# whwu95/MVFNet

Measured on AMD Instinct MI355X. Metric: clips/sec (fwd+bwd) MVFNet-R50 8x8 224^2, higher is better.
Workload: dtype bf16; 1 GPU; MVFNet-ResNet50 8x8, 32 clips/GPU of 8x3x224x224, bf16, train step: fwd (batch-stat BN) + loss + bwd + clip + SGD-nesterov; all through the HIP C ABI (stem + 16 bottlenecks + MVF + TSN head); clips_per_gpu=32, frames_per_clip=8, parallelism=dp1: replicas, one flat gradient all-reduce per step

## Files before the change

### include/mvfnet_hip.h

```cpp
#ifndef MVFNET_HIP_H
#define MVFNET_HIP_H

#include <stddef.h>
#include <stdint.h>

#ifdef __cplusplus
extern "C" {
#endif

#define MVF_ABI_VERSION 2

enum { MVF_OK = 0, MVF_EINVAL = -1, MVF_ESHAPE = -2, MVF_EWS = -3, MVF_EHIP = -4, MVF_EUNSUPPORTED = -5 };
enum { MVF_F32 = 0, MVF_BF16 = 1 };
enum { MVF_NCHW = 0, MVF_NHWC = 1 };
enum { MVF_VIEW_T = 1, MVF_VIEW_H = 2, MVF_VIEW_W = 4 };

int mvf_abi_version(void);
const char* mvf_last_error(void);

typedef struct {
    int32_t nt, c, h, w;
    int32_t n_segment;
    int32_t cs;
    int32_t mode;
// ... 6 lines not shown
                  const float* bn_scale, const float* bn_shift, void* stream);

int mvf_fwd_infer_slice(const mvf_desc_t* d, const void* x, void* out_slice,
                        const float* w_t, const float* w_h, const float* w_w,
                        const float* bn_scale, const float* bn_shift, void* stream);

size_t mvf_fwd_train_workspace_bytes(const mvf_desc_t* d);
int mvf_fwd_train(const mvf_desc_t* d, const void* x, void* out,
                  const float* w_t, const float* w_h, const float* w_w,
                  const float* gamma, const float* beta, float eps, float momentum,
                  float* running_mean, float* running_var, float* save_mean, float* save_invstd,
                  void* ws, size_t ws_bytes, void* stream);

size_t mvf_bwd_workspace_bytes(const mvf_desc_t* d);
int mvf_bwd(const mvf_desc_t* d, const void* g, const void* x,
            const float* w_t, const float* w_h, const float* w_w,
            const float* gamma, const float* beta, const float* mean, const float* invstd, int training,
            void* dx, float* dw_t, float* dw_h, float* dw_w, float* dgamma, float* dbeta,
            void* ws, size_t ws_bytes, void* stream);


typedef struct {
    int32_t n, h, w;
    int32_t cin, cout;
    int32_t kh, kw, stride, pad;
    int32_t ho, wo;
    int32_t x_pix_stride;
    int32_t dtype;
    int32_t relu;
    int32_t split_c;
    int32_t x2_pix_stride;
    int32_t in_dil;
    int32_t res_c0;
    int32_t x_c0;
} mvf_conv_desc_t;

int mvf_conv2d_nhwc_fwd(const mvf_conv_desc_t* d, const void* x, const void* x2, const void* w_packed,
                        const float* bias, const void* residual, void* y, void* stream);
size_t mvf_conv2d_workspace_bytes(const mvf_conv_desc_t* d);
int mvf_conv2d_nhwc_fwd_ws(const mvf_conv_desc_t* d, const void* x, const void* x2, const void* w_packed,
                           const float* bias, const void* residual, void* y, void* ws, size_t ws_bytes, void* stream);
int mvf_conv2d_nhwc_fwd_mvf(const mvf_conv_desc_t* d, const void* x, const void* w_packed, const float* bias, const float* mvf_coef,
                            int cs, int n_segment, int act, void* y, void* ws, size_t ws_bytes, void* stream);
int mvf_conv2d_nhwc_fwd_bnapply(const mvf_conv_desc_t* d, const void* x, const void* x2, const void* w_packed, const float* bn_scale,
                                const float* bn_shift, const void* residual, const float* res_scale, const float* res_shift, void* out,
                                unsigned char* sign_bits, void* ws, size_t ws_bytes, void* stream);
int mvf_conv2d_nhwc_fwd_bnbwd_sums(const mvf_conv_desc_t* d, const void* x, const void* x2, const void* w_packed, const void* g,
                                   const unsigned char* sign_bits, const float* bn_mean, const float* bn_invstd, float* sums_part, void* ws,
                                   size_t ws_bytes, void* stream);
int mvf_conv2d_nhwc_fwd_bnbwd_apply(const mvf_conv_desc_t* d, const void* x, const void* x2, const void* w_packed, const void* g,
                                    const unsigned char* sign_bits, const float* bn_gamma, const float* bn_mean, const float* bn_invstd,
                                    const float* dgamma, const float* dbeta, void* dz, void* ws, size_t ws_bytes, void* stream);
int mvf_conv2d_nhwc_fwd_resmask(const mvf_conv_desc_t* d, const void* x, const void* x2, const void* w_packed,
                                const float* bias, const void* residual, const unsigned char* res_sign_bits, void* y,
                                void* ws, size_t ws_bytes, void* stream);
int mvf_conv2d_nhwc_fwd_resmask_gate(const mvf_conv_desc_t* d, const void* x, const void* x2, const void* w_packed, const float* bias,
                                     const void* residual, const unsigned char* res_sign_bits, const unsigned char* out_gate_bits, void* y,
                                     void* ws, size_t ws_bytes, void* stream);
int mvf_conv2d_nhwc_fwd_resmask_gate_colsums(const mvf_conv_desc_t* d, const void* x, const void* x2, const void* w_packed, const void* residual,
                                             const unsigned char* res_sign_bits, const unsigned char* out_gate_bits, void* y, float* sums_part, void* ws,
                                             size_t ws_bytes, void* stream);
int mvf_conv2d_nhwc_dgrad_bnsums(const mvf_conv_desc_t* d, const void* dz, const void* w_packed_dgrad, void* y, const void* bn_z,
                                 const float* bn_mean, const float* bn_invstd, const float* bn_scale, const float* bn_shift,
                                 float* sums_part, void* ws, size_t ws_bytes, void* stream);
int mvf_bn_bwd_finalize(const float* sums_part, int nblk, int c, float* dgamma, float* dbeta, void* stream);
int mvf_conv2d_stats_rows(const mvf_conv_desc_t* d);
int mvf_conv2d_nhwc_fwd_stats(const mvf_conv_desc_t* d, const void* x, const void* x2, const void* w_packed, void* y,
                              float* stats_part, const float* stats_shift, void* ws, size_t ws_bytes, void* stream);

enum {
    MVF_CONV_FAM_NONE = 0,
    MVF_CONV_FAM_REG = 1,
    MVF_CONV_FAM_X3 = 2,
    MVF_CONV_FAM_LDS_DMA = 3,
    MVF_CONV_FAM_T256_2B = 4,
    MVF_CONV_FAM_T256_P4 = 5,
    MVF_CONV_FAM_DBUF = 6,
    MVF_CONV_FAM_DBUF_PF2 = 7,
    MVF_CONV_FAM_STREAMK = 8,
    MVF_CONV_FAM_GENERIC = 9,
    MVF_CONV_FAM_MVF_LOADER = 10,
    MVF_CONV_FAM_STEM_DIRECT = 11,
    MVF_CONV_FAM_PW_SUMS = 12,
    MVF_CONV_FAM_C3X3_C64 = 13
};
typedef struct {
    int32_t family;
    int32_t epi_asked;
    int32_t epi_run;
    int32_t pointwise;
    int32_t buffers;
    int32_t tile_m, tile_n;
    int32_t dtype;
    int32_t k_chunks;
    int32_t half_k;
    int32_t launches;
} mvf_conv_launch_info_t;
int mvf_conv2d_last_launch(mvf_conv_launch_info_t* out);

int mvf_pack_conv_weight(const float* w_oihw, int cout, int cin, int kh, int kw, int kw_pad, int cin_pad,
                         const float* scale, void* w_packed, int dtype, void* stream);
int mvf_bn_fold(const float* gamma, const float* beta, const float* mean, const float* var, float eps, int c,
                float* scale, float* shift, void* stream);

int mvf_stem_prep(const float* x_nchw, int n, int c, int h, int w, int pad, int wp, void* out, int dtype, void* stream);

int mvf_frames_prep_u8(const unsigned char* frames_hwc, int n, int hs, int ws, const int* window, int h, int w,
                       const float* mean3, const float* std3, int to_rgb, int div_255, int pad, int wp, void* out_stem,
                       float* out_nchw, int dtype, void* stream);
int mvf_frames_resample_u8(const unsigned char* frames_hwc, int n, int hs, int ws, const int* rows, int h, int w,
                           const float* mean3, const float* std3, int to_rgb, int div_255, int pad, int wp, void* out_stem,
                           float* out_nchw, int dtype, void* stream);
int mvf_frames_resample_color_u8(const unsigned char* frames_hwc, int n, int hs, int ws, const int* rows, const float* color, int h, int w,
                                 const float* mean3, const float* std3, int to_rgb, int div_255, int pad, int wp, void* out_stem,
                                 float* out_nchw, int dtype, void* stream);
int mvf_frames_gather_resample_u8(const unsigned char* frames_hwc, int n_src, int hs, int ws, const int* src_index, int n_out, const int* rows,
                                  const float* color, int h, int w, const float* mean3, const float* std3, int to_rgb, int div_255, int pad,
                                  int wp, void* out_stem, float* out_nchw, int dtype, void* stream);
int mvf_frames_yuv420_gather_resample_u8(const unsigned char* frames, int n_src, int hs, int ws, int pitch, int layout, int standard, int order,
                                         const int* src_index, int n_out, const int* rows, const float* color, int h, int w, const float* mean3,
                                         const float* std3, int to_rgb, int div_255, int pad, int wp, void* out_stem, float* out_nchw, int dtype,
                                         void* stream);
int mvf_frames_addressed_resample_u8(const unsigned char* frames, long long frames_bytes, int format, int standard, int order,
                                     int n_out, const int* rows, const int* addr, const float* color, int h, int w,
                                     const float* mean3, const float* std3, int to_rgb, int div_255, int pad, int wp,
                                     void* out_stem, float* out_nchw, int dtype, void* stream);

int mvf_maxpool3x3s2_nhwc(const void* x, int n, int h, int w, int c, void* y, int dtype, void* stream);

int mvf_head_pool_fc(const void* feat, int clips, int t, int hw, int c, const float* fc_w, const float* fc_b,
                     int classes, float* pooled_ws, float* scores, int dtype, void* stream);
int mvf_average_clip(const float* scores, int clips, int classes, int kind, float* out, void* stream);
int mvf_average_clip_sigmoid(const float* scores, int clips, int classes, float* out, void* stream);

int mvf_conv2d_nhwc_dgrad_bnsums_split(const mvf_conv_desc_t* d, const void* x, const void* x2, const void* w_packed, const float* bias, void* y,
                                       const void* bn_z, const float* bn_mean, const float* bn_invstd, const float* bn_scale, const float* bn_shift,
                                       float* sums_part, void* ws, size_t ws_bytes, void* stream);
int mvf_bn_bwd_dzfree_prep(const void* w_packed_dgrad, int c, int k, const float* gamma, const float* mean, const float* invstd, const float* dgamma,
                           const float* dbeta, long m, void* w_out, float* bias_out, int dtype, void* stream);
int mvf_bn_bwd_dzfree_wgrad(float* dw, const void* w_packed, const float* gram, const float* a_mean, const float* gamma, const float* mean,
                            const float* invstd, const float* dgamma, const float* dbeta, long m, int c, int k, int dtype, void* stream);
int mvf_bn_bwd_dzfree_sums(const float* q, const void* w_packed, int c, int k, const float* mean, const float* invstd, const float* part_lo, int rows_lo,
                           int c_split, const float* part_hi, int rows_hi, float* dgamma, float* dbeta, int dtype, void* stream);
size_t mvf_bn_workspace_bytes(long m, int c);
int mvf_bn_train_stats(const void* z, long m, int c, const float* gamma, const float* beta, float eps, float momentum,
                       float* running_mean, float* running_var, float* save_mean, float* save_invstd, float* scale,
                       float* shift, void* ws, size_t ws_bytes, int dtype, void* stream);
int mvf_bn_train_finalize(const float* part, int nblk, long m, int c, const float* gamma, const float* beta, float eps,
                          float momentum, float* running_mean, float* running_var, float* save_mean, float* save_invstd,
                          float* scale, float* shift, void* stream);
int mvf_bn_train_stats_gram(const float* gram, const float* a_mean, const void* w_packed, long m, int c, int k, const float* gamma, const float* beta,
                            float eps, float momentum, float* running_mean, float* running_var, float* save_mean, float* save_invstd, float* scale,
                            float* shift, int dtype, void* stream);
int mvf_bn_apply_colmeans(const void* z, long m, int c, const float* scale, const float* shift, int act, void* out, float* mean_out, void* ws,
                          size_t ws_bytes, int dtype, void* stream);
int mvf_bn_apply(const void* z, long m, int c, const float* scale, const float* shift, const void* residual,
                 const float* rscale, const float* rshift, int act, void* out, int dtype, void* stream);
int mvf_bn_bwd_reduce(const void* g, int g_pitch, const void* z, const void* ymask, long m, int c, const float* mean,
                      const float* invstd, const float* scale, const float* shift, int mask_mode, void* gm_out,
                      float* dgamma, float* dbeta, void* ws, size_t ws_bytes, int dtype, void* stream);
int mvf_bn_bwd_apply(const void* g, int g_pitch, const void* z, long m, int c, const float* gamma, const float* mean,
                     const float* invstd, const float* scale, const float* shift, const float* dgamma,
                     const float* dbeta, int mask_mode, void* dz, int dtype, void* stream);
int mvf_bn_apply_bits(const void* z, long m, int c, const float* scale, const float* shift, const void* residual,
                      const float* rscale, const float* rshift, int relu, void* out, unsigned char* sign_bits, int dtype,
                      void* stream);
int mvf_bn_apply_bits_rowscale(const void* z, long m, int c, const float* scale, const float* shift, const void* residual, const float* rscale,
                               const float* rshift, const float* row_scale, int rows_per_image, int act, void* out, unsigned char* sign_bits, int dtype,
                               void* stream);
int mvf_gate_rowscale(const void* g, int g_pitch, const unsigned char* sign_bits, const float* row_scale, int rows_per_image, long m, int c, void* gm_out,
                      int dtype, void* stream);
int mvf_bn_bwd_apply_masked(const void* g, int g_pitch, const void* z, const void* ymask, long m, int c, const float* gamma,
                            const float* mean, const float* invstd, const float* scale, const float* shift,
                            const float* dgamma, const float* dbeta, int mask_mode, void* dz, int dtype, void* stream);
int mvf_bn_bwd_pair(const void* g, int g_pitch, const void* z_a, const void* z_b, const unsigned char* sign_bits, long m, int c,
                    const float* gamma_a, const float* mean_a, const float* invstd_a, float* dgamma_a, float* dbeta_a,
                    const float* gamma_b, const float* mean_b, const float* invstd_b, float* dgamma_b, float* dbeta_b,
                    void* dz_a, void* dz_b, void* ws, size_t ws_bytes, int dtype, void* stream);
int mvf_bn_bwd_wgrad_splits(long m, int c, int k, int nbn, int mask_mode);
size_t mvf_bn_bwd_wgrad_slab_bytes(long m, int c, int k, int nbn, int mask_mode);
int mvf_bn_bwd_apply_wgrad(const void* g, int g_pitch, const void* z, const void* ymask, long m, int c, const float* gamma, const float* mean,
                           const float* invstd, const float* scale, const float* shift, const float* dgamma, const float* dbeta, int mask_mode,
                           void* dz, const void* x, int x_pitch, int k, float* slabs, size_t slab_bytes, int dtype, void* stream);
int mvf_bn_bwd_pair_wgrad(const void* g, int g_pitch, const void* z_a, const void* z_b, const unsigned char* sign_bits, long m, int c,
                          const float* gamma_a, const float* mean_a, const float* invstd_a, float* dgamma_a, float* dbeta_a,
                          const float* gamma_b, const float* mean_b, const float* invstd_b, float* dgamma_b, float* dbeta_b,
                          void* dz_a, void* dz_b, const void* x_a, int xa_pitch, const void* x_b, int xb_pitch, int k,
                          float* slabs_a, float* slabs_b, size_t slab_bytes, void* ws, size_t ws_bytes, int dtype, void* stream);
int mvf_conv1x1_bwd_fused_splits(long m, int c, int k);
int mvf_conv1x1_bwd_fused(const void* a_in, int a_pitch, const void* w_packed, const void* g, int g_pitch, const unsigned char* sign_bits, long m, int c,
                          int k, const float* gamma, const float* mean, const float* invstd, const float* dgamma, const float* dbeta, const void* z_in,
                          const float* in_mean, const float* in_invstd, const float* in_scale, const float* in_shift, void* dx, float* sums_part,
                          int sums_rows, float* slabs, size_t slab_bytes, int dtype, void* stream);
int mvf_conv1x1_bnbwd_sums_pair(const void* a_in, int a_pitch, const void* w_a, const void* x_in, int x_pitch, const void* w_b, const void* g, int g_pitch,
                                const unsigned char* sign_bits, long m, int c, int k, const float* mean_a, const float* invstd_a, const float* mean_b,
                                const float* invstd_b, float* part_a, float* part_b, int rows, int dtype, void* stream);
int mvf_wgrad_slab_reduce(const float* slabs, int nsplit, int cout, int k, float* dw_oihw, void* stream);
int mvf_maxpool_bn_relu_fwd(const void* z, int n, int h, int w, int c, const float* scale, const float* shift, void* y,
                            unsigned char* argmax, int dtype, void* stream);
int mvf_maxpool_bn_relu_bwd(const unsigned char* argmax, const void* g, int n, int h, int w, int c, void* ga, int dtype,
                            void* stream);
int mvf_maxpool_bwd_sums_rows(int n, int h);
int mvf_maxpool_bn_relu_bwd_apply(const unsigned char* argmax, const void* g, int n, int h, int w, int c, const void* z, const float* gamma,
                                  const float* mean, const float* invstd, const float* scale, const float* shift, const float* dgamma,
                                  const float* dbeta, void* dz, int dtype, void* stream);
int mvf_maxpool_bn_relu_bwd_sums(const unsigned char* argmax, const void* g, int n, int h, int w, int c, void* ga, const void* z, const float* mean,
                                 const float* invstd, const float* scale, const float* shift, float* sums_part, int dtype, void* stream);
enum {
    MVF_BN_ENTRY_NONE = 0,
    MVF_BN_ENTRY_TRAIN_STATS = 1, MVF_BN_ENTRY_TRAIN_FINALIZE = 2,
    MVF_BN_ENTRY_APPLY = 3,
    MVF_BN_ENTRY_APPLY_COLMEANS = 4,
    MVF_BN_ENTRY_BWD_REDUCE = 5, MVF_BN_ENTRY_BWD_FINALIZE = 6,
    MVF_BN_ENTRY_BWD_APPLY = 7,
    MVF_BN_ENTRY_BWD_PAIR = 8, MVF_BN_ENTRY_BWD_PAIR_WGRAD = 9,
    MVF_BN_ENTRY_POOL_FWD = 10, MVF_BN_ENTRY_POOL_BWD = 11, MVF_BN_ENTRY_POOL_BWD_SUMS = 12, MVF_BN_ENTRY_POOL_BWD_APPLY = 13
};
enum {
    MVF_BN_FIN_NONE = 0,
    MVF_BN_FIN_ROW_MAJOR = 1,
    MVF_BN_FIN_CM_WORKGROUP = 2,
    MVF_BN_FIN_CM_WAVE = 3
};
enum {
    MVF_POOL_FORM_NONE = 0,
    MVF_POOL_FORM_ELEMENT = 1,
    MVF_POOL_FORM_ROWS = 2,
    MVF_POOL_FORM_BLOCK = 3,
    MVF_POOL_FORM_ROWS_SUMS = 4,
    MVF_POOL_FORM_ROWS_APPLY = 5
};
typedef struct {
    int32_t entry;
    int32_t dtype;
    int32_t vn;
    int32_t cqb, rows, gx, gy;
    int32_t mask_mode;
    int32_t specialised;
    int32_t finalize;
    int32_t part_rows;
    int32_t pool;
    int32_t launches;
} mvf_bn_launch_info_t;
int mvf_bn_last_launch(mvf_bn_launch_info_t* out);
int mvf_head_train_fwd(const void* feat, int clips, int t, int hw, int c, const float* fc_w, const float* fc_b, int classes,
                       const long long* labels, const float* drop_mask ,
                       float* pooled, float* scores, float* dscores, float* loss_part, float* loss, int dtype, void* stream);
int mvf_ce_loss(const float* scores, const long long* labels, int clips, int classes, float* dscores, float* loss_part, float* loss,
                void* stream);
int mvf_head_train_bwd(const float* dscores, const float* pooled, const float* fc_w, const float* drop_mask, int clips, int t,
                       int hw, int c, int classes, float* dfc_w, float* dfc_b, float* dpool_ws , void* dfeat, int dtype,
                       void* stream);
int mvf_stem_blend(const void* xp, int clips, int t, int hp, int wp, int pad, const int* rows, const float* wts, void* out, int dtype, void* stream);
int mvf_soft_targets(const long long* labels, const int* rows, const float* wts, int clips, int classes, float eps, float* targets, void* stream);
int mvf_ce_loss_soft(const float* scores, const float* targets, int clips, int classes, float* dscores, float* loss_part, float* loss, void* stream);
int mvf_head_train_fwd_soft(const void* feat, int clips, int t, int hw, int c, const float* fc_w, const float* fc_b, int classes,
                            const float* targets, const float* drop_mask ,
                            float* pooled, float* scores, float* dscores, float* loss_part, float* loss, int dtype, void* stream);
int mvf_bce_loss(const float* scores, const float* targets, int clips, int classes, const float* pos_weight ,
                 float target_threshold , int sum_classes, float* dscores , float* loss_part, float* loss, void* stream);
int mvf_head_train_fwd_bce(const void* feat, int clips, int t, int hw, int c, const float* fc_w, const float* fc_b, int classes,
                           const float* targets, const float* drop_mask ,
                           const float* pos_weight , float target_threshold , int sum_classes,
                           float* pooled, float* scores, float* dscores, float* loss_part, float* loss, int dtype, void* stream);
typedef struct mvf_focal_params {
    float gamma_pos, gamma_neg, margin, alpha, target_threshold;
    int sum_classes, reserved[2];
} mvf_focal_params_t;
int mvf_focal_loss(const float* scores, const float* targets, int clips, int classes, const float* class_weight ,
                   const mvf_focal_params_t* prm, float* dscores , float* loss_part, float* loss, void* stream);
int mvf_head_train_fwd_focal(const void* feat, int clips, int t, int hw, int c, const float* fc_w, const float* fc_b, int classes,
                             const float* targets, const float* drop_mask ,
                             const float* class_weight , const mvf_focal_params_t* prm,
                             float* pooled, float* scores, float* dscores, float* loss_part, float* loss, int dtype, void* stream);
int mvf_distill_loss(const float* scores, const float* teacher_scores, int clips, int classes, float temperature, float alpha,
                     float* dscores , float* loss_part , float* loss , float* terms ,
                     void* stream);
#define MVF_TRN_MAX_FRAMES 16
#define MVF_TRN_KSPLIT_MAX 8
typedef struct mvf_trn_scale {
    const float *w1, *b1, *w2, *b2;
    float *dw1, *db1, *dw2, *db2;
} mvf_trn_scale_t;
enum { MVF_TRN_ENTRY_NONE = 0, MVF_TRN_ENTRY_FWD = 1, MVF_TRN_ENTRY_BWD = 2 };
typedef struct mvf_trn_launch_info {
    int32_t entry;
    int32_t dtype;
    int32_t rows, n_scales;
    int32_t launches;
} mvf_trn_launch_info_t;
int mvf_trn_head_fwd(const void* feat, int clips, int t, int hw, int c, const float* fc_w, const float* fc_b, int fdim, const mvf_trn_scale_t* scales,
                     int n_scales, int hidden, int classes, const int* table, int rows, const float* drop_mask , float* pooled,
                     float* f, float* h, float* hpart , float* scores, int dtype, void* stream);
int mvf_trn_head_bwd(const float* dscores, const float* pooled, const float* f, const float* h, const float* fc_w, const mvf_trn_scale_t* scales, int n_scales,
                     int hidden, int classes, const int* table, int rows, const float* drop_mask , int clips, int t, int hw, int c,
                     int fdim, float* dfc_w, float* dfc_b, float* dh , float* df , float* dpool ,
                     void* dfeat, int dtype, void* stream);
int mvf_trn_head_last_launch(mvf_trn_launch_info_t* out);
int mvf_stem_erase(void* xp, int planes, int hp, int wp, int pad, const int* boxes, int max_boxes, const float* fill, const unsigned int* key, int dtype,
                   void* stream);
#define MVF_RANDAUG_WS_PER_FRAME (3 * 256 + 16)
int mvf_frames_randaug_u8(const unsigned char* frames_hwc, int n, int hs, int ws, int t, int order, const int* sizes, const int* table, int layers,
                          unsigned stats_layers, unsigned char* out, unsigned char* tmp, void* workspace, long long workspace_bytes, void* stream);
size_t mvf_conv2d_wgrad_workspace_bytes(const mvf_conv_desc_t* d);
int mvf_conv2d_nhwc_wgrad(const mvf_conv_desc_t* d, const void* dz, const void* x, const void* x2, int kw_real,
                          int cin_real, int kw_packed, int cin_packed, float* dw_oihw, void* ws, size_t ws_bytes,
                          void* stream);
int mvf_conv2d_nhwc_wgrad_wgs(const mvf_conv_desc_t* d, const void* dz, const void* x, const void* x2, int kw_real,
                              int cin_real, int kw_packed, int cin_packed, float* dw_oihw, void* ws, size_t ws_bytes, int wgs, void* stream);
enum {
    MVF_WGRAD_FAM_NONE = 0,
    MVF_WGRAD_FAM_F32_REG = 1,
    MVF_WGRAD_FAM_F32_DMA = 2,
    MVF_WGRAD_FAM_X3 = 3,
    MVF_WGRAD_FAM_BF16_WIDEN = 4,
    MVF_WGRAD_FAM_BF16_REG = 5,
    MVF_WGRAD_FAM_BF16_DMA2 = 6,
    MVF_WGRAD_FAM_BF16_PIPE = 7,
    MVF_WGRAD_FAM_T256_2B = 8,
    MVF_WGRAD_FAM_T256_P4 = 9,
    MVF_WGRAD_FAM_C3X3_C64 = 10,
    MVF_WGRAD_FAM_STEM = 11
};
typedef struct {
    int32_t family;
    int32_t stages;
    int32_t tile_co, tile_k;
    int32_t dtype;
    int32_t nsplit;
    int32_t rows_per_split;
    int32_t xcd_rr;
    int32_t split_operand;
    int32_t gram;
    int32_t wgs_target;
    int32_t launches;
} mvf_wgrad_launch_info_t;
int mvf_conv2d_wgrad_last_launch(mvf_wgrad_launch_info_t* out);
typedef struct {
    const float* w;
    void* out;
    int cout, cin, kh, kw, kw_pad, cin_pad;
    int kind, first_block;
} mvf_pack_job_t;
int mvf_pack_conv_weights_batched(const mvf_pack_job_t* jobs_dev, int njobs, int total_blocks, int dtype, void* stream);

int mvf_pack_conv_weight_dgrad(const float* w_oihw, int cout, int cin, int kh, int kw, void* w_packed, int dtype,
                               void* stream);
int mvf_nhwc_stencil(const mvf_desc_t* d, const void* x, int x_c, void* out, int out_c, const float* w_t,
                     const float* w_h, const float* w_w, const float* scale, const float* shift, int flip,
                     const void* addend, int addend_c, const unsigned char* addend_sign_bits, void* stream);
int mvf_nhwc_stencil_gate(const mvf_desc_t* d, const void* x, int x_c, void* out, int out_c, const float* w_t,
                          const float* w_h, const float* w_w, const float* scale, const float* shift, int flip,
                          const void* addend, int addend_c, const unsigned char* addend_sign_bits,
                          const unsigned char* out_gate_bits, void* stream);
int mvf_nhwc_stencil_gate_colsums(const mvf_desc_t* d, const void* x, int x_c, void* out, int out_c, const float* w_t, const float* w_h,
                                  const float* w_w, int flip, const void* addend, int addend_c, const unsigned char* addend_sign_bits,
                                  const unsigned char* out_gate_bits, float* sums_part, void* stream);
int mvf_nhwc_stencil_stats_rows(const mvf_desc_t* d, int x_c, int out_c);
int mvf_nhwc_stencil_tile_plan(const mvf_desc_t* d, int x_c, int out_c, int* rows_per_band, int* chan_per_wg);
int mvf_nhwc_stencil_stats(const mvf_desc_t* d, const void* x, int x_c, void* out, int out_c, const float* w_t, const float* w_h,
                           const float* w_w, float* stats_part, const float* stats_shift, void* stream);
size_t mvf_nhwc_tapgrad_workspace_bytes(const mvf_desc_t* d);
int mvf_nhwc_tapgrad(const mvf_desc_t* d, const void* x, int x_c, const void* dy, int dy_c, float* dw_t, float* dw_h,
                     float* dw_w, void* ws, size_t ws_bytes, void* stream);
enum {
    MVF_STENCIL_KERNEL_NONE = 0,
    MVF_STENCIL_KERNEL_WALK1 = 1,
    MVF_STENCIL_KERNEL_WALK4 = 2,
    MVF_STENCIL_KERNEL_CHUNKED = 3,
    MVF_STENCIL_KERNEL_LDS = 4
};
enum {
    MVF_STENCIL_FLIP = 1, MVF_STENCIL_HSWISH = 2, MVF_STENCIL_ADDEND = 4, MVF_STENCIL_ADDEND_BITS = 8, MVF_STENCIL_OUT_GATE = 16,
    MVF_STENCIL_STATS = 32,
    MVF_STENCIL_TAIL_COPY = 64
};
typedef struct {
    int32_t kernel;
    int32_t dtype;
    int32_t frames_per_chunk;
    int32_t rows_per_band, chan_per_wg;
    int32_t bands;
    int32_t pixels_per_wg;
    int32_t grid_x, grid_y;
    int32_t partial_rows;
    int32_t flags;
    int32_t launches;
} mvf_stencil_launch_info_t;
int mvf_nhwc_stencil_last_launch(mvf_stencil_launch_info_t* out);
enum {
    MVF_TAPGRAD_KERNEL_NONE = 0,
    MVF_TAPGRAD_KERNEL_ROWS = 1,
    MVF_TAPGRAD_KERNEL_BANDS = 2
};
typedef struct {
    int32_t kernel;
    int32_t dtype;
    int32_t nblk;
    int32_t rows_per_blk;
    int32_t cgp;
    int32_t grid_y;
    int32_t launches;
} mvf_tapgrad_launch_info_t;
int mvf_nhwc_tapgrad_last_launch(mvf_tapgrad_launch_info_t* out);
size_t mvf_sgd_workspace_bytes(long n);
int mvf_sgd_nesterov_step(float* params, const float* grads, float* momentum_buf, long n, float grad_scale, float max_norm,
                          float lr, float momentum, float weight_decay, int first_step, float* norm_out, void* ws,
                          size_t ws_bytes, void* stream);
typedef struct mvf_sgd_segment {
    long long first;
    float lr_mult, decay_mult;
} mvf_sgd_segment_t;
int mvf_sgd_step_segments(float* params, const float* grads, float* momentum_buf, long n, float grad_scale, float max_norm, float lr,
                          float momentum, float weight_decay, int first_step, int nesterov, const mvf_sgd_segment_t* segments, int nseg,
                          float* norm_out, void* ws, size_t ws_bytes, void* stream);
int mvf_grad_accumulate(float* acc, const float* g, long n, int first, void* stream);
int mvf_sgd_nesterov_step_ema(float* params, const float* grads, float* momentum_buf, long n, float grad_scale, float max_norm, float lr, float momentum,
                              float weight_decay, int first_step, float* ema, float ema_momentum, float* norm_out, void* ws, size_t ws_bytes, void* stream);
int mvf_sgd_step_segments_ema(float* params, const float* grads, float* momentum_buf, long n, float grad_scale, float max_norm, float lr, float momentum,
                              float weight_decay, int first_step, int nesterov, const mvf_sgd_segment_t* segments, int nseg, float* ema, float ema_momentum,
                              float* norm_out, void* ws, size_t ws_bytes, void* stream);
int mvf_ema_update(float* ema, const float* params, long n, float momentum, void* stream);
int mvf_ema_swap(float* a, float* b, long n, void* stream);
typedef struct mvf_stat_segment {
    float* ptr;
    long first;
} mvf_stat_segment_t;
int mvf_bn_stats_accumulate(const mvf_stat_segment_t* seg, int nseg, long n, double* acc, void* stream);
int mvf_bn_stats_finalize(const mvf_stat_segment_t* seg, int nseg, long n, const double* acc, long count, float* dst_flat_or_null, void* stream);
int mvf_bn_stats_exchange(const mvf_stat_segment_t* seg, int nseg, long n, float* flat, int mode, void* stream);
int mvf_sgd_step_guarded(float* params, const float* grads, float* momentum_buf, long n, float grad_scale, float max_norm, float lr, float momentum,
                         float weight_decay, int first_step, int nesterov, const mvf_sgd_segment_t* segments, int nseg, float* ema, float ema_momentum,
                         int* guard, float* norm_out, void* ws, size_t ws_bytes, void* stream);
int mvf_bn_stats_snapshot(const mvf_stat_segment_t* seg, int nseg, long n, float* flat, const long long* counters, long ncount, long long* counters_copy,
                          void* stream);
int mvf_bn_stats_restore(const mvf_stat_segment_t* seg, int nseg, long n, const float* flat, long long* counters, long ncount,
                         const long long* counters_copy, const int* guard, void* stream);
typedef struct mvf_adamw_hyper {
    double lr, beta1, beta2, eps, weight_decay;
    int decoupled;
} mvf_adamw_hyper_t;
size_t mvf_adamw_workspace_bytes(long n);
int mvf_adamw_step(float* params, const float* grads, float* exp_avg, float* exp_avg_sq, long n, float grad_scale, float max_norm,
                   const mvf_adamw_hyper_t* hyper, const mvf_sgd_segment_t* segments, int nseg, float* ema, float ema_momentum, int* guard,
                   long long* applied_steps, float* norm_out, void* ws, size_t ws_bytes, void* stream);
typedef struct mvf_lamb_hyper {
    double lr, beta1, beta2, eps, weight_decay;
    int trust_clip, always_adapt;
} mvf_lamb_hyper_t;
size_t mvf_lamb_workspace_bytes(long n, int nseg);
int mvf_lamb_step(float* params, const float* grads, float* exp_avg, float* exp_avg_sq, long n, float grad_scale, float max_norm,
                  const mvf_lamb_hyper_t* hyper, const mvf_sgd_segment_t* segments, int nseg, float* ema, float ema_momentum, int* guard,
                  long long* applied_steps, float* norm_out, float* ratio_out, void* ws, size_t ws_bytes, void* stream);
enum { MVF_METRICS_ROWS = 0, MVF_METRICS_BAD_LABEL = 1, MVF_METRICS_NAN_ROWS = 2, MVF_METRICS_HITS = 8, MVF_METRICS_MAX_K = 8, MVF_METRICS_CONFUSION = 16 };
size_t mvf_metrics_state_words(int classes, int with_confusion);
int mvf_metrics_update(const float* scores, int rows, int classes, const long long* labels, const int* ks, int nk, long long* state, int with_confusion,
                       int* rank_out, int* pred_out, void* stream);
enum { MVF_MULTILABEL_SLOTS = 0, MVF_MULTILABEL_NAN_ROWS = 1, MVF_MULTILABEL_OVERFLOW = 2, MVF_MULTILABEL_SEEN = 3, MVF_MULTILABEL_STATE_WORDS = 8 };
int mvf_multilabel_record(const float* scores, const unsigned char* labels, int rows, int classes, float* rec_scores, unsigned char* rec_labels, long capacity,
                          long long* state, void* stream);
int mvf_multilabel_ap(const float* rec_scores, const unsigned char* rec_labels, long capacity, int classes, const long long* state, int* tp, int* nn, double* ap,
                      long long* positives, void* stream);
int mvf_multilabel_sample_ap(const float* rec_scores, const unsigned char* rec_labels, long capacity, int classes, const long long* state, double* sample_ap,
                             int* sample_positives, void* stream);
int mvf_multilabel_prf(const float* rec_scores, const unsigned char* rec_labels, long capacity, int classes, const long long* state, float threshold,
                       const float* thresholds , long long* counts , void* stream);
int mvf_multilabel_best_f1(const float* rec_scores, const int* tp, const int* nn, const long long* positives, long capacity, int classes,
                           const long long* state, int* best_tp, int* best_n, float* best_threshold, void* stream);
typedef struct mvf_flat_stats {
    double sumsq;
    double absmax;
    long long n_nan;
    long long n_inf;
} mvf_flat_stats_t;
size_t mvf_flat_stats_workspace_bytes(long n, int nseg);
int mvf_flat_segment_stats(const float* x, const float* y_or_null, long n, const long long* first, int nseg, mvf_flat_stats_t* out, const int* guard_or_null,
                           long long* step_out_or_null, void* ws, size_t ws_bytes, void* stream);
int mvf_bn_stats_nonfinite(const mvf_stat_segment_t* seg, int nseg, long n, long long* counts, const int* guard_or_null, void* stream);

enum { MVF_PLAN_CALL = 0, MVF_PLAN_RECORD = 1, MVF_PLAN_WAIT = 2 };
typedef struct mvf_plan_op {
    int kind, n_int, n_flt, reserved;
    void* fn;
    long long word0, float0;
} mvf_plan_op_t;
int mvf_plan_run(const mvf_plan_op_t* ops, int n_ops, const unsigned long long* words, const float* floats, int* failed_op);

#ifdef __cplusplus
}
#endif
// ... 2 lines not shown
```

### mvfnet_amd/_lib.py

```python
import ctypes as C
import os

import torch

_HERE = os.path.dirname(os.path.abspath(__file__))
LIB_PATH = os.environ.get("MVF_LIB_PATH") or os.path.join(_HERE, "libmvfnet_hip.so")

MVF_F32, MVF_BF16 = 0, 1
MVF_NCHW, MVF_NHWC = 0, 1
VIEW_T, VIEW_H, VIEW_W = 1, 2, 4
MODE_BITS = {"T": 1, "TH": 3, "THW": 7}
METRICS_ROWS, METRICS_BAD_LABEL, METRICS_NAN_ROWS, METRICS_HITS, METRICS_MAX_K, METRICS_CONFUSION = 0, 1, 2, 8, 8, 16
MULTILABEL_SLOTS, MULTILABEL_NAN_ROWS, MULTILABEL_OVERFLOW, MULTILABEL_SEEN, MULTILABEL_STATE_WORDS = 0, 1, 2, 3, 8
ERRNAMES = {-1: "MVF_EINVAL", -2: "MVF_ESHAPE", -3: "MVF_EWS", -4: "MVF_EHIP", -5: "MVF_EUNSUPPORTED"}


class MvfDesc(C.Structure):
    _fields_ = [("nt", C.c_int32), ("c", C.c_int32), ("h", C.c_int32), ("w", C.c_int32), ("n_segment", C.c_int32),
                ("cs", C.c_int32), ("mode", C.c_int32), ("layout", C.c_int32), ("dtype", C.c_int32)]


class ConvDesc(C.Structure):
    _fields_ = [("n", C.c_int32), ("h", C.c_int32), ("w", C.c_int32), ("cin", C.c_int32), ("cout", C.c_int32),
                ("kh", C.c_int32), ("kw", C.c_int32), ("stride", C.c_int32), ("pad", C.c_int32),
# ... 71 lines not shown


class FocalParams(C.Structure):
    _fields_ = [("gamma_pos", C.c_float), ("gamma_neg", C.c_float), ("margin", C.c_float), ("alpha", C.c_float), ("target_threshold", C.c_float),
                ("sum_classes", C.c_int32), ("reserved", C.c_int32 * 2)]


TRN_MAX_FRAMES, TRN_KSPLIT_MAX = 16, 8


class TrnScale(C.Structure):
    _fields_ = [("w1", C.c_void_p), ("b1", C.c_void_p), ("w2", C.c_void_p), ("b2", C.c_void_p),
                ("dw1", C.c_void_p), ("db1", C.c_void_p), ("dw2", C.c_void_p), ("db2", C.c_void_p)]


class TrnLaunchInfo(C.Structure):
    _fields_ = [("entry", C.c_int32), ("dtype", C.c_int32), ("rows", C.c_int32), ("n_scales", C.c_int32), ("launches", C.c_int32)]


class LambHyper(C.Structure):
    _fields_ = [("lr", C.c_double), ("beta1", C.c_double), ("beta2", C.c_double), ("eps", C.c_double), ("weight_decay", C.c_double), ("trust_clip", C.c_int32),
                ("always_adapt", C.c_int32)]


class StatSegment(C.Structure):
    _fields_ = [("ptr", C.c_void_p), ("first", C.c_long)]


QUERIES = frozenset((
    "mvf_abi_version", "mvf_last_error",
    "mvf_fwd_train_workspace_bytes", "mvf_bwd_workspace_bytes", "mvf_conv2d_workspace_bytes", "mvf_conv2d_wgrad_workspace_bytes", "mvf_bn_workspace_bytes",
    "mvf_bn_bwd_wgrad_slab_bytes", "mvf_nhwc_tapgrad_workspace_bytes", "mvf_sgd_workspace_bytes", "mvf_adamw_workspace_bytes", "mvf_lamb_workspace_bytes",
    "mvf_flat_stats_workspace_bytes", "mvf_metrics_state_words",
    "mvf_conv2d_stats_rows", "mvf_nhwc_stencil_stats_rows", "mvf_maxpool_bwd_sums_rows",
    "mvf_bn_bwd_wgrad_splits", "mvf_conv1x1_bwd_fused_splits", "mvf_nhwc_stencil_tile_plan",
    "mvf_conv2d_last_launch", "mvf_conv2d_wgrad_last_launch", "mvf_bn_last_launch", "mvf_nhwc_stencil_last_launch", "mvf_nhwc_tapgrad_last_launch",
    "mvf_trn_head_last_launch",
))


def _load():
    if not os.path.exists(LIB_PATH):
        raise ImportError(
            "mvfnet_amd: %s not found. Build it with `python -m mvfnet_amd.build` (needs hipcc, "
            "--offload-arch=gfx950). There is no CPU or PyTorch fallback for the hot path." % LIB_PATH)
    lib = C.CDLL(LIB_PATH)
    vp, fp, sz, i32, f32 = C.c_void_p, C.c_void_p, C.c_size_t, C.c_int, C.c_float
    dp = C.POINTER(MvfDesc)
    lib.mvf_abi_version.restype = i32
    lib.mvf_abi_version.argtypes = []
    lib.mvf_last_error.restype = C.c_char_p
    lib.mvf_last_error.argtypes = []
    lib.mvf_fwd_infer.restype = i32
    lib.mvf_fwd_infer.argtypes = [dp, vp, vp, fp, fp, fp, fp, fp, vp]
    lib.mvf_fwd_train_workspace_bytes.restype = sz
    lib.mvf_fwd_train_workspace_bytes.argtypes = [dp]
    lib.mvf_fwd_train.restype = i32
    lib.mvf_fwd_train.argtypes = [dp, vp, vp, fp, fp, fp, fp, fp, f32, f32, fp, fp, fp, fp, vp, sz, vp]
    lib.mvf_bwd_workspace_bytes.restype = sz
    lib.mvf_bwd_workspace_bytes.argtypes = [dp]
    lib.mvf_bwd.restype = i32
    lib.mvf_bwd.argtypes = [dp, vp, vp, fp, fp, fp, fp, fp, fp, fp, i32, vp, fp, fp, fp, fp, fp, vp, sz, vp]
    lib.mvf_fwd_infer_slice.restype = i32
    lib.mvf_fwd_infer_slice.argtypes = [dp, vp, vp, fp, fp, fp, fp, fp, vp]
    cp = C.POINTER(ConvDesc)
    lib.mvf_conv2d_nhwc_fwd.restype = i32
    lib.mvf_conv2d_nhwc_fwd.argtypes = [cp, vp, vp, vp, fp, vp, vp, vp]
    lib.mvf_conv2d_workspace_bytes.restype = sz
    lib.mvf_conv2d_workspace_bytes.argtypes = [cp]
    lib.mvf_conv2d_nhwc_fwd_ws.restype = i32
    lib.mvf_conv2d_nhwc_fwd_ws.argtypes = [cp, vp, vp, vp, fp, vp, vp, vp, sz, vp]
    lib.mvf_conv2d_nhwc_dgrad_bnsums.restype = i32
    lib.mvf_conv2d_nhwc_dgrad_bnsums.argtypes = [cp, vp, vp, vp, vp, fp, fp, fp, fp, fp, vp, sz, vp]
    lib.mvf_bn_bwd_finalize.restype = i32
    lib.mvf_bn_bwd_finalize.argtypes = [fp, i32, i32, fp, fp, vp]
    lib.mvf_conv2d_nhwc_fwd_bnapply.restype = i32
    lib.mvf_conv2d_nhwc_fwd_bnapply.argtypes = [cp, vp, vp, vp, fp, fp, vp, fp, fp, vp, vp, vp, sz, vp]
    lib.mvf_conv2d_nhwc_fwd_bnbwd_sums.restype = i32
    lib.mvf_conv2d_nhwc_fwd_bnbwd_sums.argtypes = [cp, vp, vp, vp, vp, vp, fp, fp, fp, vp, sz, vp]
    lib.mvf_conv2d_nhwc_fwd_bnbwd_apply.restype = i32
    lib.mvf_conv2d_nhwc_fwd_bnbwd_apply.argtypes = [cp, vp, vp, vp, vp, vp, fp, fp, fp, fp, fp, vp, vp, sz, vp]
    lib.mvf_conv2d_nhwc_fwd_resmask.restype = i32
    lib.mvf_conv2d_nhwc_fwd_resmask.argtypes = [cp, vp, vp, vp, fp, vp, vp, vp, vp, sz, vp]
    i64_ = C.c_long
    lib.mvf_conv2d_nhwc_fwd_resmask_gate.restype = i32
    lib.mvf_conv2d_nhwc_fwd_resmask_gate.argtypes = [cp, vp, vp, vp, fp, vp, vp, vp, vp, vp, sz, vp]
    lib.mvf_conv2d_nhwc_fwd_resmask_gate_colsums.restype = i32
    lib.mvf_conv2d_nhwc_fwd_resmask_gate_colsums.argtypes = [cp, vp, vp, vp, vp, vp, vp, vp, fp, vp, sz, vp]
    lib.mvf_nhwc_stencil_gate_colsums.restype = i32
    lib.mvf_nhwc_stencil_gate_colsums.argtypes = [dp, vp, i32, vp, i32, fp, fp, fp, i32, vp, i32, vp, vp, fp, vp]
    lib.mvf_conv2d_nhwc_dgrad_bnsums_split.restype = i32
    lib.mvf_conv2d_nhwc_dgrad_bnsums_split.argtypes = [cp, vp, vp, vp, fp, vp, vp, fp, fp, fp, fp, fp, vp, sz, vp]
    lib.mvf_bn_bwd_dzfree_prep.restype = i32
    lib.mvf_bn_bwd_dzfree_prep.argtypes = [vp, i32, i32, fp, fp, fp, fp, fp, i64_, vp, fp, i32, vp]
    lib.mvf_bn_bwd_dzfree_wgrad.restype = i32
    lib.mvf_bn_bwd_dzfree_wgrad.argtypes = [fp, vp, fp, fp, fp, fp, fp, fp, fp, i64_, i32, i32, i32, vp]
    lib.mvf_bn_bwd_dzfree_sums.restype = i32
    lib.mvf_bn_bwd_dzfree_sums.argtypes = [fp, vp, i32, i32, fp, fp, fp, i32, i32, fp, i32, fp, fp, i32, vp]
    lib.mvf_nhwc_stencil_stats_rows.restype = i32
    lib.mvf_nhwc_stencil_stats_rows.argtypes = [dp, i32, i32]
    lib.mvf_nhwc_stencil_tile_plan.restype = i32
    lib.mvf_nhwc_stencil_tile_plan.argtypes = [dp, i32, i32, C.POINTER(C.c_int), C.POINTER(C.c_int)]
    lib.mvf_nhwc_stencil_stats.restype = i32
    lib.mvf_nhwc_stencil_stats.argtypes = [dp, vp, i32, vp, i32, fp, fp, fp, fp, fp, vp]
    lib.mvf_nhwc_stencil_gate.restype = i32
    lib.mvf_nhwc_stencil_gate.argtypes = [dp, vp, i32, vp, i32, fp, fp, fp, fp, fp, i32, vp, i32, vp, vp, vp]
    lib.mvf_conv2d_stats_rows.restype = i32
    lib.mvf_conv2d_stats_rows.argtypes = [cp]
    lib.mvf_conv2d_nhwc_fwd_stats.restype = i32
    lib.mvf_conv2d_nhwc_fwd_stats.argtypes = [cp, vp, vp, vp, vp, fp, fp, vp, sz, vp]
    lib.mvf_conv2d_last_launch.restype = i32
    lib.mvf_conv2d_last_launch.argtypes = [C.POINTER(ConvLaunchInfo)]
    lib.mvf_pack_conv_weight.restype = i32
    lib.mvf_pack_conv_weight.argtypes = [fp, i32, i32, i32, i32, i32, i32, fp, vp, i32, vp]
    lib.mvf_pack_conv_weights_batched.restype = i32
    lib.mvf_pack_conv_weights_batched.argtypes = [vp, i32, i32, i32, vp]
    lib.mvf_bn_fold.restype = i32
    lib.mvf_bn_fold.argtypes = [fp, fp, fp, fp, f32, i32, fp, fp, vp]
    lib.mvf_stem_prep.restype = i32
    lib.mvf_stem_prep.argtypes = [fp, i32, i32, i32, i32, i32, i32, vp, i32, vp]
    lib.mvf_frames_prep_u8.restype = i32
    lib.mvf_frames_prep_u8.argtypes = [vp, i32, i32, i32, vp, i32, i32, C.POINTER(C.c_float), C.POINTER(C.c_float),
                                       i32, i32, i32, i32, vp, vp, i32, vp]
    lib.mvf_frames_resample_u8.restype = i32
    lib.mvf_frames_resample_u8.argtypes = [vp, i32, i32, i32, vp, i32, i32, C.POINTER(C.c_float), C.POINTER(C.c_float),
                                           i32, i32, i32, i32, vp, vp, i32, vp]
    lib.mvf_frames_resample_color_u8.restype = i32
    lib.mvf_frames_resample_color_u8.argtypes = [vp, i32, i32, i32, vp, vp, i32, i32, C.POINTER(C.c_float), C.POINTER(C.c_float),
                                                 i32, i32, i32, i32, vp, vp, i32, vp]
    lib.mvf_frames_gather_resample_u8.restype = i32
    lib.mvf_frames_gather_resample_u8.argtypes = [vp, i32, i32, i32, vp, i32, vp, vp, i32, i32, C.POINTER(C.c_float), C.POINTER(C.c_float),
                                                  i32, i32, i32, i32, vp, vp, i32, vp]
    lib.mvf_frames_yuv420_gather_resample_u8.restype = i32
    lib.mvf_frames_yuv420_gather_resample_u8.argtypes = [vp, i32, i32, i32, i32, i32, i32, i32, vp, i32, vp, vp, i32, i32, C.POINTER(C.c_float),
                                                         C.POINTER(C.c_float), i32, i32, i32, i32, vp, vp, i32, vp]
    lib.mvf_frames_addressed_resample_u8.restype = i32
    lib.mvf_frames_addressed_resample_u8.argtypes = [vp, C.c_longlong, i32, i32, i32, i32, vp, vp, vp, i32, i32, C.POINTER(C.c_float), C.POINTER(C.c_float),
                                                     i32, i32, i32, i32, vp, vp, i32, vp]
    lib.mvf_maxpool3x3s2_nhwc.restype = i32
    lib.mvf_maxpool3x3s2_nhwc.argtypes = [vp, i32, i32, i32, i32, vp, i32, vp]
    lib.mvf_head_pool_fc.restype = i32
    lib.mvf_head_pool_fc.argtypes = [vp, i32, i32, i32, i32, fp, fp, i32, fp, fp, i32, vp]
    lib.mvf_average_clip.restype = i32
    lib.mvf_average_clip.argtypes = [fp, i32, i32, i32, fp, vp]
    i64, ll = C.c_long, C.c_void_p
    lib.mvf_bn_workspace_bytes.restype = sz
    lib.mvf_bn_workspace_bytes.argtypes = [i64, i32]
    lib.mvf_bn_train_stats.restype = i32
    lib.mvf_bn_train_stats.argtypes = [vp, i64, i32, fp, fp, f32, f32, fp, fp, fp, fp, fp, fp, vp, sz, i32, vp]
    lib.mvf_bn_train_finalize.restype = i32
    lib.mvf_bn_train_finalize.argtypes = [fp, i32, i64, i32, fp, fp, f32, f32, fp, fp, fp, fp, fp, fp, vp]
    lib.mvf_bn_train_stats_gram.restype = i32
    lib.mvf_bn_train_stats_gram.argtypes = [fp, fp, vp, i64, i32, i32, fp, fp, f32, f32, fp, fp, fp, fp, fp, fp, i32, vp]
    lib.mvf_bn_apply_colmeans.restype = i32
    lib.mvf_bn_apply_colmeans.argtypes = [vp, i64, i32, fp, fp, i32, vp, fp, vp, sz, i32, vp]
    lib.mvf_bn_apply.restype = i32
    lib.mvf_bn_apply.argtypes = [vp, i64, i32, fp, fp, vp, fp, fp, i32, vp, i32, vp]
    lib.mvf_bn_apply_bits.restype = i32
    lib.mvf_bn_apply_bits.argtypes = [vp, i64, i32, fp, fp, vp, fp, fp, i32, vp, vp, i32, vp]
    lib.mvf_bn_apply_bits_rowscale.restype = i32
    lib.mvf_bn_apply_bits_rowscale.argtypes = [vp, i64, i32, fp, fp, vp, fp, fp, fp, i32, i32, vp, vp, i32, vp]
    lib.mvf_gate_rowscale.restype = i32
    lib.mvf_gate_rowscale.argtypes = [vp, i32, vp, fp, i32, i64, i32, vp, i32, vp]
    lib.mvf_bn_bwd_apply_masked.restype = i32
    lib.mvf_bn_bwd_apply_masked.argtypes = [vp, i32, vp, vp, i64, i32, fp, fp, fp, fp, fp, fp, fp, i32, vp, i32, vp]
    lib.mvf_bn_bwd_reduce.restype = i32
    lib.mvf_bn_bwd_reduce.argtypes = [vp, i32, vp, vp, i64, i32, fp, fp, fp, fp, i32, vp, fp, fp, vp, sz, i32, vp]
    lib.mvf_bn_bwd_apply.restype = i32
    lib.mvf_bn_bwd_apply.argtypes = [vp, i32, vp, i64, i32, fp, fp, fp, fp, fp, fp, fp, i32, vp, i32, vp]
    lib.mvf_maxpool_bn_relu_fwd.restype = i32
    lib.mvf_maxpool_bn_relu_fwd.argtypes = [vp, i32, i32, i32, i32, fp, fp, vp, vp, i32, vp]
    lib.mvf_maxpool_bn_relu_bwd.restype = i32
    lib.mvf_maxpool_bn_relu_bwd.argtypes = [vp, vp, i32, i32, i32, i32, vp, i32, vp]
    lib.mvf_maxpool_bwd_sums_rows.restype = i32
    lib.mvf_maxpool_bwd_sums_rows.argtypes = [i32, i32]
    lib.mvf_maxpool_bn_relu_bwd_apply.restype = i32
    lib.mvf_maxpool_bn_relu_bwd_apply.argtypes = [vp, vp, i32, i32, i32, i32, vp, fp, fp, fp, fp, fp, fp, fp, vp, i32, vp]
    lib.mvf_maxpool_bn_relu_bwd_sums.restype = i32
    lib.mvf_maxpool_bn_relu_bwd_sums.argtypes = [vp, vp, i32, i32, i32, i32, vp, vp, fp, fp, fp, fp, fp, i32, vp]
    lib.mvf_bn_last_launch.restype = i32
    lib.mvf_bn_last_launch.argtypes = [C.POINTER(BnLaunchInfo)]
    lib.mvf_head_train_fwd.restype = i32
    lib.mvf_head_train_fwd.argtypes = [vp, i32, i32, i32, i32, fp, fp, i32, ll, fp, fp, fp, fp, fp, fp, i32, vp]
    lib.mvf_conv2d_nhwc_fwd_mvf.restype = i32
    lib.mvf_conv2d_nhwc_fwd_mvf.argtypes = [cp, vp, vp, fp, fp, i32, i32, i32, vp, vp, sz, vp]
    lib.mvf_bn_bwd_pair.restype = i32
    lib.mvf_bn_bwd_pair.argtypes = [vp, i32, vp, vp, vp, i64, i32, fp, fp, fp, fp, fp, fp, fp, fp, fp, fp, vp, vp, vp, sz, i32, vp]
    lib.mvf_bn_bwd_wgrad_splits.restype = i32
    lib.mvf_bn_bwd_wgrad_splits.argtypes = [i64, i32, i32, i32, i32]
    lib.mvf_bn_bwd_wgrad_slab_bytes.restype = sz
    lib.mvf_bn_bwd_wgrad_slab_bytes.argtypes = [i64, i32, i32, i32, i32]
    lib.mvf_bn_bwd_apply_wgrad.restype = i32
    lib.mvf_bn_bwd_apply_wgrad.argtypes = [vp, i32, vp, vp, i64, i32, fp, fp, fp, fp, fp, fp, fp, i32, vp, vp, i32, i32, fp, sz, i32, vp]
    lib.mvf_bn_bwd_pair_wgrad.restype = i32
    lib.mvf_bn_bwd_pair_wgrad.argtypes = [vp, i32, vp, vp, vp, i64, i32, fp, fp, fp, fp, fp, fp, fp, fp, fp, fp, vp, vp, vp, i32, vp, i32, i32,
                                          fp, fp, sz, vp, sz, i32, vp]
    lib.mvf_conv1x1_bwd_fused_splits.restype = i32
    lib.mvf_conv1x1_bwd_fused_splits.argtypes = [i64, i32, i32]
    lib.mvf_conv1x1_bwd_fused.restype = i32
    lib.mvf_conv1x1_bwd_fused.argtypes = [vp, i32, vp, vp, i32, vp, i64, i32, i32, fp, fp, fp, fp, fp, vp, fp, fp, fp, fp, vp, fp, i32, fp, sz, i32, vp]
    lib.mvf_conv1x1_bnbwd_sums_pair.restype = i32
    lib.mvf_conv1x1_bnbwd_sums_pair.argtypes = [vp, i32, vp, vp, i32, vp, vp, i32, vp, i64, i32, i32, fp, fp, fp, fp, fp, fp, i32, i32, vp]
    lib.mvf_wgrad_slab_reduce.restype = i32
    lib.mvf_wgrad_slab_reduce.argtypes = [fp, i32, i32, i32, fp, vp]
    lib.mvf_ce_loss.restype = i32
    lib.mvf_ce_loss.argtypes = [fp, ll, i32, i32, fp, fp, fp, vp]
    lib.mvf_stem_blend.restype = i32
    lib.mvf_stem_blend.argtypes = [vp, i32, i32, i32, i32, i32, vp, fp, vp, i32, vp]
    lib.mvf_stem_erase.restype = i32
    lib.mvf_stem_erase.argtypes = [vp, i32, i32, i32, i32, vp, i32, fp, vp, i32, vp]
    lib.mvf_frames_randaug_u8.restype = i32
    lib.mvf_frames_randaug_u8.argtypes = [vp, i32, i32, i32, i32, i32, vp, vp, i32, C.c_uint, vp, vp, vp, C.c_longlong, vp]
    lib.mvf_soft_targets.restype = i32
    lib.mvf_soft_targets.argtypes = [ll, vp, fp, i32, i32, f32, fp, vp]
    lib.mvf_ce_loss_soft.restype = i32
    lib.mvf_ce_loss_soft.argtypes = [fp, fp, i32, i32, fp, fp, fp, vp]
    lib.mvf_head_train_fwd_soft.restype = i32
    lib.mvf_head_train_fwd_soft.argtypes = [vp, i32, i32, i32, i32, fp, fp, i32, fp, fp, fp, fp, fp, fp, fp, i32, vp]
    lib.mvf_distill_loss.restype = i32
    lib.mvf_distill_loss.argtypes = [fp, fp, i32, i32, f32, f32, fp, fp, fp, fp, vp]
    lib.mvf_bce_loss.restype = i32
    lib.mvf_bce_loss.argtypes = [fp, fp, i32, i32, fp, f32, i32, fp, fp, fp, vp]
    lib.mvf_head_train_fwd_bce.restype = i32
    lib.mvf_head_train_fwd_bce.argtypes = [vp, i32, i32, i32, i32, fp, fp, i32, fp, fp, fp, f32, i32, fp, fp, fp, fp, fp, i32, vp]
    lib.mvf_focal_loss.restype = i32
    lib.mvf_focal_loss.argtypes = [fp, fp, i32, i32, fp, C.POINTER(FocalParams), fp, fp, fp, vp]
    lib.mvf_head_train_fwd_focal.restype = i32
    lib.mvf_head_train_fwd_focal.argtypes = [vp, i32, i32, i32, i32, fp, fp, i32, fp, fp, fp, C.POINTER(FocalParams), fp, fp, fp, fp, fp, i32, vp]
    lib.mvf_trn_head_fwd.restype = i32
    lib.mvf_trn_head_fwd.argtypes = [vp, i32, i32, i32, i32, fp, fp, i32, C.POINTER(TrnScale), i32, i32, i32, vp, i32, fp, fp, fp, fp, fp, fp, i32, vp]
    lib.mvf_trn_head_bwd.restype = i32
    lib.mvf_trn_head_bwd.argtypes = [fp, fp, fp, fp, fp, C.POINTER(TrnScale), i32, i32, i32, vp, i32, fp, i32, i32, i32, i32, i32, fp, fp, fp, fp, fp, vp, i32, vp]
    lib.mvf_trn_head_last_launch.restype = i32
    lib.mvf_trn_head_last_launch.argtypes = [C.POINTER(TrnLaunchInfo)]
    lib.mvf_average_clip_sigmoid.restype = i32
    lib.mvf_average_clip_sigmoid.argtypes = [fp, i32, i32, fp, vp]
    lib.mvf_multilabel_record.restype = i32
    lib.mvf_multilabel_record.argtypes = [fp, vp, i32, i32, fp, vp, C.c_long, ll, vp]
    lib.mvf_multilabel_ap.restype = i32
    lib.mvf_multilabel_ap.argtypes = [fp, vp, C.c_long, i32, ll, vp, vp, vp, ll, vp]
    lib.mvf_multilabel_sample_ap.restype = i32
    lib.mvf_multilabel_sample_ap.argtypes = [fp, vp, C.c_long, i32, ll, vp, vp, vp]
    lib.mvf_multilabel_prf.restype = i32
    lib.mvf_multilabel_prf.argtypes = [fp, vp, C.c_long, i32, ll, f32, fp, ll, vp]
    lib.mvf_multilabel_best_f1.restype = i32
    lib.mvf_multilabel_best_f1.argtypes = [fp, vp, vp, ll, C.c_long, i32, ll, vp, vp, fp, vp]
    lib.mvf_head_train_bwd.restype = i32
    lib.mvf_head_train_bwd.argtypes = [fp, fp, fp, fp, i32, i32, i32, i32, i32, fp, fp, fp, vp, i32, vp]
    lib.mvf_conv2d_wgrad_workspace_bytes.restype = sz
    lib.mvf_conv2d_wgrad_workspace_bytes.argtypes = [cp]
    lib.mvf_conv2d_nhwc_wgrad.restype = i32
    lib.mvf_conv2d_nhwc_wgrad.argtypes = [cp, vp, vp, vp, i32, i32, i32, i32, fp, vp, sz, vp]
    lib.mvf_conv2d_nhwc_wgrad_wgs.restype = i32
    lib.mvf_conv2d_nhwc_wgrad_wgs.argtypes = [cp, vp, vp, vp, i32, i32, i32, i32, fp, vp, sz, i32, vp]
    lib.mvf_conv2d_wgrad_last_launch.restype = i32
    lib.mvf_conv2d_wgrad_last_launch.argtypes = [C.POINTER(WgradLaunchInfo)]
    lib.mvf_pack_conv_weight_dgrad.restype = i32
    lib.mvf_pack_conv_weight_dgrad.argtypes = [fp, i32, i32, i32, i32, vp, i32, vp]
    lib.mvf_nhwc_stencil.restype = i32
    lib.mvf_nhwc_stencil.argtypes = [dp, vp, i32, vp, i32, fp, fp, fp, fp, fp, i32, vp, i32, vp, vp]
    lib.mvf_nhwc_tapgrad_workspace_bytes.restype = sz
    lib.mvf_nhwc_tapgrad_workspace_bytes.argtypes = [dp]
    lib.mvf_nhwc_tapgrad.restype = i32
    lib.mvf_nhwc_tapgrad.argtypes = [dp, vp, i32, vp, i32, fp, fp, fp, vp, sz, vp]
    lib.mvf_nhwc_stencil_last_launch.restype = i32
    lib.mvf_nhwc_stencil_last_launch.argtypes = [C.POINTER(StencilLaunchInfo)]
    lib.mvf_nhwc_tapgrad_last_launch.restype = i32
    lib.mvf_nhwc_tapgrad_last_launch.argtypes = [C.POINTER(TapgradLaunchInfo)]
    lib.mvf_sgd_workspace_bytes.restype = sz
    lib.mvf_sgd_workspace_bytes.argtypes = [i64]
    lib.mvf_sgd_nesterov_step.restype = i32
    lib.mvf_sgd_nesterov_step.argtypes = [fp, fp, fp, i64, f32, f32, f32, f32, f32, i32, fp, vp, sz, vp]
    lib.mvf_sgd_step_segments.restype = i32
    lib.mvf_sgd_step_segments.argtypes = [fp, fp, fp, i64, f32, f32, f32, f32, f32, i32, i32, vp, i32, fp, vp, sz, vp]
    lib.mvf_grad_accumulate.restype = i32
    lib.mvf_grad_accumulate.argtypes = [fp, fp, i64, i32, vp]
    lib.mvf_sgd_nesterov_step_ema.restype = i32
    lib.mvf_sgd_nesterov_step_ema.argtypes = [fp, fp, fp, i64, f32, f32, f32, f32, f32, i32, fp, f32, fp, vp, sz, vp]
    lib.mvf_sgd_step_segments_ema.restype = i32
    lib.mvf_sgd_step_segments_ema.argtypes = [fp, fp, fp, i64, f32, f32, f32, f32, f32, i32, i32, vp, i32, fp, f32, fp, vp, sz, vp]
    lib.mvf_ema_update.restype = i32
    lib.mvf_ema_update.argtypes = [fp, fp, i64, f32, vp]
    lib.mvf_ema_swap.restype = i32
    lib.mvf_ema_swap.argtypes = [fp, fp, i64, vp]
    lib.mvf_bn_stats_accumulate.restype = i32
    lib.mvf_bn_stats_accumulate.argtypes = [vp, i32, i64, vp, vp]
    lib.mvf_bn_stats_finalize.restype = i32
    lib.mvf_bn_stats_finalize.argtypes = [vp, i32, i64, vp, i64, fp, vp]
    lib.mvf_bn_stats_exchange.restype = i32
    lib.mvf_bn_stats_exchange.argtypes = [vp, i32, i64, fp, i32, vp]
    lib.mvf_sgd_step_guarded.restype = i32
    lib.mvf_sgd_step_guarded.argtypes = [fp, fp, fp, i64, f32, f32, f32, f32, f32, i32, i32, vp, i32, fp, f32, vp, fp, vp, sz, vp]
    lib.mvf_bn_stats_snapshot.restype = i32
    lib.mvf_bn_stats_snapshot.argtypes = [vp, i32, i64, fp, vp, i64, vp, vp]
    lib.mvf_bn_stats_restore.restype = i32
    lib.mvf_bn_stats_restore.argtypes = [vp, i32, i64, fp, vp, i64, vp, vp, vp]
    lib.mvf_adamw_workspace_bytes.restype = sz
    lib.mvf_adamw_workspace_bytes.argtypes = [i64]
    lib.mvf_adamw_step.restype = i32
    lib.mvf_adamw_step.argtypes = [fp, fp, fp, fp, i64, f32, f32, C.POINTER(AdamwHyper), vp, i32, fp, f32, vp, vp, fp, vp, sz, vp]
    lib.mvf_lamb_workspace_bytes.restype = sz
    lib.mvf_lamb_workspace_bytes.argtypes = [i64, i32]
    lib.mvf_lamb_step.restype = i32
    lib.mvf_lamb_step.argtypes = [fp, fp, fp, fp, i64, f32, f32, C.POINTER(LambHyper), vp, i32, fp, f32, vp, vp, fp, fp, vp, sz, vp]
    lib.mvf_metrics_state_words.restype = sz
    lib.mvf_metrics_state_words.argtypes = [i32, i32]
    lib.mvf_metrics_update.restype = i32
    lib.mvf_metrics_update.argtypes = [fp, i32, i32, ll, vp, i32, ll, i32, vp, vp, vp]
    lib.mvf_flat_stats_workspace_bytes.restype = sz
    lib.mvf_flat_stats_workspace_bytes.argtypes = [i64, i32]
    lib.mvf_flat_segment_stats.restype = i32
    lib.mvf_flat_segment_stats.argtypes = [fp, fp, i64, vp, i32, vp, vp, vp, vp, sz, vp]
    lib.mvf_bn_stats_nonfinite.restype = i32
    lib.mvf_bn_stats_nonfinite.argtypes = [vp, i32, i64, vp, vp, vp]
    lib.mvf_plan_run.restype = i32
    lib.mvf_plan_run.argtypes = [C.POINTER(PlanOp), i32, C.POINTER(C.c_ulonglong), C.POINTER(C.c_float), C.POINTER(C.c_int)]
    missing = [n for n in declared_symbols() if hasattr(lib, n) and getattr(lib, n).argtypes is None]
    if missing:
        raise ImportError("mvfnet_amd._lib: no argtypes declared for %s" % missing)
    return lib


def check(rc, what=""):
    if rc != 0:
        msg = lib.mvf_last_error().decode("utf-8", "replace")
        raise RuntimeError("%s failed: %s (%s)" % (what or "libmvfnet_hip", ERRNAMES.get(rc, rc), msg))


def declared_symbols():
    import re
    hdr = os.path.join(os.path.dirname(_HERE), "include", "mvfnet_hip.h")
    txt = open(hdr).read()
    txt = re.sub(r"/\*.*?\*/", "", txt, flags=re.S)
    return sorted(set(re.findall(r"\b((?:mvf|mvfnet)_[a-z0-9_]+)\s*\(", txt)))


lib = _load()
```

### mvfnet_amd/csrc/bn_dzfree.hip

```cpp
#include "common.h"

namespace {

typedef float f32x16 __attribute__((ext_vector_type(16)));
typedef short bf16x8 __attribute__((ext_vector_type(8)));

struct PrepArgs {
    const uint16_t* wd;
    const float *gamma, *mean, *invstd, *dgamma, *dbeta;
    uint16_t* bd;
    float* bias;
    int C, K;
    float inv_m;
    int g_wgs, s_wgs;
};

__device__ __forceinline__ float bf16lo(unsigned u) { return __uint_as_float(u << 16); }
__device__ __forceinline__ float bf16hi(unsigned u) { return __uint_as_float(u & 0xffff0000u); }

__global__ __launch_bounds__(256) void dzfree_prep_kernel(PrepArgs p) {
    extern __shared__ __attribute__((aligned(16))) float coef[];
    const int C = p.C, K = p.K, tid = threadIdx.x;
    float* ca = coef;
    float* ce = coef + C;
// ... 98 lines not shown
    const int kb = K / 32, blk = blockIdx.x * 4 + wave;
    if (blk >= (C / 32) * kb) return;
    const int c0 = (blk / kb) * 32, k0 = (blk % kb) * 32;
    const int row = lane & 31, half = lane >> 5;
    const uint16_t* pw = w + (long)(c0 + row) * K + half * 8;
    const float* pg = gram + (long)(k0 + row) * K + half * 8;
    f32x16 acc;
#pragma unroll
    for (int r = 0; r < 16; ++r) acc[r] = 0.f;
    constexpr int U = 4;
    for (int j = 0; j < K; j += 16 * U) {
        uint4 vw[U];
        float4 g0[U], g1[U];
#pragma unroll
        for (int u = 0; u < U; ++u) {
            vw[u] = *reinterpret_cast<const uint4*>(pw + j + 16 * u);
            g0[u] = *reinterpret_cast<const float4*>(pg + j + 16 * u);
            g1[u] = *reinterpret_cast<const float4*>(pg + j + 16 * u + 4);
        }
#pragma unroll
        for (int u = 0; u < U; ++u) {
            uint4 hi, lo;
            hi.x = pack_bf16x2(g0[u].x, g0[u].y); hi.y = pack_bf16x2(g0[u].z, g0[u].w);
            hi.z = pack_bf16x2(g1[u].x, g1[u].y); hi.w = pack_bf16x2(g1[u].z, g1[u].w);
            lo.x = pack_bf16x2(g0[u].x - bf16lo(hi.x), g0[u].y - bf16hi(hi.x)); lo.y = pack_bf16x2(g0[u].z - bf16lo(hi.y), g0[u].w - bf16hi(hi.y));
            lo.z = pack_bf16x2(g1[u].x - bf16lo(hi.z), g1[u].y - bf16hi(hi.z)); lo.w = pack_bf16x2(g1[u].z - bf16lo(hi.w), g1[u].w - bf16hi(hi.w));
            bf16x8 fw, fh, fl;
            __builtin_memcpy(&fw, &vw[u], 16);
            __builtin_memcpy(&fh, &hi, 16);
            __builtin_memcpy(&fl, &lo, 16);
            acc = __builtin_amdgcn_mfma_f32_32x32x16_bf16(fw, fh, acc, 0, 0, 0);
            acc = __builtin_amdgcn_mfma_f32_32x32x16_bf16(fw, fl, acc, 0, 0, 0);
        }
    }
    const float inv_m = 1.0f / m_f;
    const int k = k0 + row;
    const float sa = a_mean[k] * m_f;
#pragma unroll
    for (int r = 0; r < 16; ++r) {
        const int c = c0 + 8 * (r >> 2) + 4 * half + (r & 3);
        const float rs = invstd[c], a = gamma[c] * rs, d0 = dbeta[c] * inv_m, kx = rs * dgamma[c] * inv_m;
        const long i = (long)c * K + k;
        dw[i] = a * (dw[i] - d0 * sa - kx * (acc[r] - mean[c] * sa));
    }
}

__global__ __launch_bounds__(256) void dzfree_sums_kernel(const float* q, const uint16_t* w, int C, int K, const float* mean,
                                                          const float* invstd, const float* part_lo, int rows_lo, int c_split, const float* part_hi, int rows_hi,
                                                          float* dgamma, float* dbeta) {
    const int lane = threadIdx.x & 63, c = blockIdx.x * 4 + (threadIdx.x >> 6);
    if (c >= C) return;
    const bool lo = c < c_split;
    const int rows = lo ? rows_lo : rows_hi;
    const float2* p = reinterpret_cast<const float2*>(lo ? part_lo : part_hi) + (long)c * rows;
    float s1 = 0.f, dot = 0.f;
    for (int r = lane; r < rows; r += 64) s1 += p[r].x;
    const uint16_t* pw = w + (long)c * K;
    const float* pq = q + (long)c * K;
    for (int k = lane * 4; k < K; k += 256) {
        const uint2 wv = *reinterpret_cast<const uint2*>(pw + k);
        const float4 qv = *reinterpret_cast<const float4*>(pq + k);
        dot += bf16lo(wv.x) * qv.x + bf16hi(wv.x) * qv.y + bf16lo(wv.y) * qv.z + bf16hi(wv.y) * qv.w;
    }
#pragma unroll
    for (int o = 32; o > 0; o >>= 1) {
        s1 += __shfl_xor(s1, o, 64);
        dot += __shfl_xor(dot, o, 64);
    }
    if (lane == 0) {
        dbeta[c] = s1;
        dgamma[c] = invstd[c] * (dot - mean[c] * s1);
    }
}

struct GramStatsArgs {
    const float* gram; const float* a_mean; const uint16_t* w; const float* gamma; const float* beta;
    float* running_mean; float* running_var; float* save_mean; float* save_invstd; float* scale; float* shift;
    int C, K; float inv_m, eps, momentum, unbias;
};
__global__ __launch_bounds__(256) void gram_stats_kernel(GramStatsArgs p) {
    const int lane = threadIdx.x & 63, wave = threadIdx.x >> 6, K = p.K;
    const int blk = blockIdx.x * 4 + wave;
    if (blk >= p.C / 32) return;
    const int c0 = blk * 32, row = lane & 31, half = lane >> 5;
    const uint16_t* pw = p.w + (long)(c0 + row) * K + half * 8;
    float qacc[16], macc[16];
#pragma unroll
    for (int r = 0; r < 16; ++r) qacc[r] = macc[r] = 0.f;
    for (int kb = 0; kb < K / 32; ++kb) {
        const int k = kb * 32 + row;
        const float* pg = p.gram + (long)k * K + half * 8;
        const float* pa = p.a_mean + half * 8;
        const float ak = p.a_mean[k];
        f32x16 acc;
#pragma unroll
        for (int r = 0; r < 16; ++r) acc[r] = 0.f;
        for (int j = 0; j < K; j += 16) {
            const uint4 vw = *reinterpret_cast<const uint4*>(pw + j);
            const float4 g0 = *reinterpret_cast<const float4*>(pg + j), g1 = *reinterpret_cast<const float4*>(pg + j + 4);
            const float4 a0 = *reinterpret_cast<const float4*>(pa + j), a1 = *reinterpret_cast<const float4*>(pa + j + 4);
            float gc[8] = {g0.x * p.inv_m - ak * a0.x, g0.y * p.inv_m - ak * a0.y, g0.z * p.inv_m - ak * a0.z, g0.w * p.inv_m - ak * a0.w,
                           g1.x * p.inv_m - ak * a1.x, g1.y * p.inv_m - ak * a1.y, g1.z * p.inv_m - ak * a1.z, g1.w * p.inv_m - ak * a1.w};
            unsigned hi[4], mid[4], lo[4];
#pragma unroll
            for (int q = 0; q < 4; ++q) {
                const float x0 = gc[2 * q], x1 = gc[2 * q + 1];
                hi[q] = pack_bf16x2(x0, x1);
                const float r0 = x0 - bf16lo(hi[q]), r1 = x1 - bf16hi(hi[q]);
                mid[q] = pack_bf16x2(r0, r1);
                lo[q] = pack_bf16x2(r0 - bf16lo(mid[q]), r1 - bf16hi(mid[q]));
            }
            bf16x8 fw, fh, fm, fl;
            __builtin_memcpy(&fw, &vw, 16);
            __builtin_memcpy(&fh, hi, 16);
            __builtin_memcpy(&fm, mid, 16);
            __builtin_memcpy(&fl, lo, 16);
            acc = __builtin_amdgcn_mfma_f32_32x32x16_bf16(fw, fh, acc, 0, 0, 0);
            acc = __builtin_amdgcn_mfma_f32_32x32x16_bf16(fw, fm, acc, 0, 0, 0);
            acc = __builtin_amdgcn_mfma_f32_32x32x16_bf16(fw, fl, acc, 0, 0, 0);
        }
#pragma unroll
        for (int r = 0; r < 16; ++r) {
            const int c = c0 + 8 * (r >> 2) + 4 * half + (r & 3);
            const float wv = __uint_as_float((unsigned)p.w[(long)c * K + k] << 16);
            qacc[r] += acc[r] * wv;
            macc[r] += wv * ak;
        }
    }
#pragma unroll
    for (int r = 0; r < 16; ++r) {
#pragma unroll
        for (int o = 1; o < 32; o <<= 1) {
            qacc[r] += __shfl_xor(qacc[r], o, 64);
            macc[r] += __shfl_xor(macc[r], o, 64);
        }
    }
    if (row == 0) {
#pragma unroll
        for (int r = 0; r < 16; ++r) {
            const int c = c0 + 8 * (r >> 2) + 4 * half + (r & 3);
            const float mean = macc[r], var = fmaxf(qacc[r], 0.f);
            const float invstd = 1.0f / sqrtf(var + p.eps);
            p.save_mean[c] = mean;
            p.save_invstd[c] = invstd;
            const float s = p.gamma[c] * invstd;
            p.scale[c] = s;
            p.shift[c] = p.beta[c] - mean * s;
            if (p.running_mean) p.running_mean[c] = (1.f - p.momentum) * p.running_mean[c] + p.momentum * mean;
            if (p.running_var) p.running_var[c] = (1.f - p.momentum) * p.running_var[c] + p.momentum * (var * p.unbias);
        }
    }
}

constexpr long GRAM_F64_MAX_ROWS = 16;
__global__ __launch_bounds__(256) void gram_stats_f64_kernel(GramStatsArgs p, double inv_m, double unbias) {
    const int lane = threadIdx.x & 63, c = blockIdx.x * 4 + (threadIdx.x >> 6), K = p.K;
    if (c >= p.C) return;
    const uint16_t* pw = p.w + (long)c * K;
    double q = 0.0, mu = 0.0;
    for (int k = lane; k < K; k += 64) {
        const double wk = (double)__uint_as_float((unsigned)pw[k] << 16), ak = (double)p.a_mean[k];
        const float* pg = p.gram + (long)k * K;
        double t = 0.0;
        for (int j = 0; j < K; ++j) t += (double)__uint_as_float((unsigned)pw[j] << 16) * ((double)pg[j] * inv_m - ak * (double)p.a_mean[j]);
        q += wk * t;
        mu += wk * ak;
    }
#pragma unroll
    for (int o = 32; o > 0; o >>= 1) {
        q += __shfl_xor(q, o, 64);
        mu += __shfl_xor(mu, o, 64);
    }
    if (lane == 0) {
        const double var = q > 0.0 ? q : 0.0;
        const float mean = (float)mu, invstd = (float)(1.0 / sqrt(var + (double)p.eps));
        p.save_mean[c] = mean;
        p.save_invstd[c] = invstd;
        const float s = p.gamma[c] * invstd;
        p.scale[c] = s;
        p.shift[c] = p.beta[c] - mean * s;
        if (p.running_mean) p.running_mean[c] = (1.f - p.momentum) * p.running_mean[c] + p.momentum * mean;
        if (p.running_var) p.running_var[c] = (1.f - p.momentum) * p.running_var[c] + p.momentum * (float)(var * unbias);
    }
}

}

extern "C" {

int mvf_bn_train_stats_gram(const float* gram, const float* a_mean, const void* w_packed, long m, int c, int k, const float* gamma, const float* beta, float eps,
                            float momentum, float* running_mean, float* running_var, float* save_mean, float* save_invstd, float* scale, float* shift,
                            int dtype, void* stream) {
    MVF_REQUIRE(gram && a_mean && w_packed && gamma && beta && save_mean && save_invstd && scale && shift && m > 0, MVF_EINVAL, "bn_train_stats_gram: NULL argument");
    MVF_REQUIRE(dtype == MVF_BF16, MVF_EUNSUPPORTED, "bn_train_stats_gram: bf16 storage only");
    MVF_REQUIRE(c > 0 && k > 0 && c % 32 == 0 && k % 32 == 0, MVF_ESHAPE, "bn_train_stats_gram: c=%d and k=%d must be multiples of 32", c, k);
    MVF_REQUIRE(((uintptr_t)gram | (uintptr_t)a_mean | (uintptr_t)w_packed) % 16 == 0, MVF_EINVAL, "bn_train_stats_gram: operands must be 16-byte aligned");
    GramStatsArgs p = {gram, a_mean, (const uint16_t*)w_packed, gamma, beta, running_mean, running_var, save_mean, save_invstd, scale, shift,
                       c, k, 1.0f / (float)m, eps, momentum, (float)((double)m / (double)(m > 1 ? m - 1 : 1))};
    if (m <= GRAM_F64_MAX_ROWS)
        hipLaunchKernelGGL(gram_stats_f64_kernel, dim3((c + 3) / 4), dim3(256), 0, (hipStream_t)stream, p, 1.0 / (double)m, (double)m / (double)(m > 1 ? m - 1 : 1));
    else
        hipLaunchKernelGGL(gram_stats_kernel, dim3((c / 32 + 3) / 4), dim3(256), 0, (hipStream_t)stream, p);
    MVF_LAUNCH_CHECK();
    return MVF_OK;
}

int mvf_bn_bwd_dzfree_sums(const float* q, const void* w_packed, int c, int k, const float* mean, const float* invstd,
                           const float* part_lo, int rows_lo, int c_split, const float* part_hi, int rows_hi, float* dgamma, float* dbeta, int dtype, void* stream) {
    MVF_REQUIRE(q && w_packed && mean && invstd && dgamma && dbeta, MVF_EINVAL, "bn_bwd_dzfree_sums: NULL argument");
    MVF_REQUIRE(dtype == MVF_BF16, MVF_EUNSUPPORTED, "bn_bwd_dzfree_sums: bf16 storage only");
    MVF_REQUIRE(c > 0 && k > 0 && k % 4 == 0 && c_split >= 0 && c_split <= c, MVF_ESHAPE, "bn_bwd_dzfree_sums: c=%d, k=%d (a multiple of 4), 0 <= c_split=%d <= c", c, k, c_split);
    MVF_REQUIRE((c_split == 0 || (part_lo && rows_lo > 0)) && (c_split == c || (part_hi && rows_hi > 0)), MVF_EINVAL, "bn_bwd_dzfree_sums: a channel range without partial sums");
    MVF_REQUIRE(((uintptr_t)q % 16 == 0) && ((uintptr_t)w_packed % 8 == 0), MVF_EINVAL, "bn_bwd_dzfree_sums: q must be 16-byte, w_packed 8-byte aligned");
    hipLaunchKernelGGL(dzfree_sums_kernel, dim3((c + 3) / 4), dim3(256), 0, (hipStream_t)stream, q, (const uint16_t*)w_packed, c, k, mean, invstd, part_lo, rows_lo,
                       c_split, part_hi, rows_hi, dgamma, dbeta);
    MVF_LAUNCH_CHECK();
    return MVF_OK;
}

int mvf_bn_bwd_dzfree_prep(const void* w_packed_dgrad, int c, int k, const float* gamma, const float* mean, const float* invstd, const float* dgamma,
                           const float* dbeta, long m, void* w_out, float* bias_out, int dtype, void* stream) {
    MVF_REQUIRE(w_packed_dgrad && gamma && mean && invstd && dgamma && dbeta && w_out && bias_out && m > 0, MVF_EINVAL, "bn_bwd_dzfree_prep: NULL argument");
    MVF_REQUIRE(dtype == MVF_BF16, MVF_EUNSUPPORTED, "bn_bwd_dzfree_prep: bf16 storage only");
    MVF_REQUIRE(c > 0 && k > 0 && c % 64 == 0 && k % 32 == 0 && c <= 4096, MVF_ESHAPE, "bn_bwd_dzfree_prep: c=%d must be a multiple of 64 (<= 4096), k=%d a multiple of 32", c, k);
    MVF_REQUIRE(((uintptr_t)w_packed_dgrad | (uintptr_t)w_out) % 16 == 0, MVF_EINVAL, "bn_bwd_dzfree_prep: operands must be 16-byte aligned");
    PrepArgs p = {};
    p.wd = (const uint16_t*)w_packed_dgrad; p.gamma = gamma; p.mean = mean; p.invstd = invstd; p.dgamma = dgamma; p.dbeta = dbeta;
    p.bd = (uint16_t*)w_out; p.bias = bias_out; p.C = c; p.K = k; p.inv_m = 1.0f / (float)m;
    MVF_REQUIRE(c % 256 == 0, MVF_ESHAPE, "bn_bwd_dzfree_prep: c=%d must be a multiple of 256 (four waves x 64-channel trips)", c);
    const int kb = k / 32;
    p.g_wgs = kb * kb;
    p.s_wgs = (int)(((long)k * (c / 8) + 255) / 256);
    const int b_wgs = (k + 3) / 4;
    const size_t lds = (size_t)3 * c * sizeof(float) + 4 * 16 * 64 * sizeof(float);
    hipLaunchKernelGGL(dzfree_prep_kernel, dim3(p.g_wgs + p.s_wgs + b_wgs), dim3(256), lds, (hipStream_t)stream, p);
    MVF_LAUNCH_CHECK();
    return MVF_OK;
}

int mvf_bn_bwd_dzfree_wgrad(float* dw, const void* w_packed, const float* gram, const float* a_mean, const float* gamma, const float* mean,
                            const float* invstd, const float* dgamma, const float* dbeta, long m, int c, int k, int dtype, void* stream) {
    MVF_REQUIRE(dw && w_packed && gram && a_mean && gamma && mean && invstd && dgamma && dbeta && m > 0, MVF_EINVAL, "bn_bwd_dzfree_wgrad: NULL argument");
    MVF_REQUIRE(dtype == MVF_BF16, MVF_EUNSUPPORTED, "bn_bwd_dzfree_wgrad: bf16 storage only");
    MVF_REQUIRE(c > 0 && c % 32 == 0 && k > 0 && k % 64 == 0, MVF_ESHAPE, "bn_bwd_dzfree_wgrad: c=%d must be a multiple of 32, k=%d of 64", c, k);
    MVF_REQUIRE(((uintptr_t)w_packed | (uintptr_t)gram) % 16 == 0, MVF_EINVAL, "bn_bwd_dzfree_wgrad: w_packed / gram must be 16-byte aligned");
    const int blocks = (c / 32) * (k / 32);
    hipLaunchKernelGGL(dzfree_wgrad_fix_kernel, dim3((blocks + 3) / 4), dim3(256), 0, (hipStream_t)stream, dw, (const uint16_t*)w_packed, gram, a_mean, gamma, mean,
                       invstd, dgamma, dbeta, c, k, (float)m);
    MVF_LAUNCH_CHECK();
    return MVF_OK;
}

}
```

### mvfnet_amd/csrc/wgrad_nhwc.hip

```cpp
#include <algorithm>

#include <stdlib.h>

#include "common.h"

namespace {

constexpr int kThreads = 256;
constexpr int BMR = 32;
typedef float f32x16 __attribute__((ext_vector_type(16)));

struct WgArgs {
    const void* dz;
    const void* x;
    const void* x2;
    float* part;
    int N, H, W, Cin, Cout, KH, KW, stride, pad, Ho, Wo, xps, split_c, x2ps;
    int M, K, rows_per_split, tiles_k;
    int tiles, nsplit;
    unsigned fd_hw_mul, fd_hw_shr, fd_w_mul, fd_w_shr;
    int xcd_rr;
    int abl;
};

// ... 362 lines not shown
        __syncthreads();
    }
    if (c < nchunks) compute(0);
    float* out = a.part + (long)wg_split * a.Cout * a.K;
#pragma unroll
    for (int j = 0; j < TN; ++j) {
        const int col = k0 + (wn * TN + j) * 32 + lc;
        if (col >= a.K) continue;
#pragma unroll
        for (int i = 0; i < TM; ++i)
#pragma unroll
            for (int r = 0; r < 16; ++r) {
                const int row = co0 + (wm * TM + i) * 32 + (r & 3) + 8 * (r >> 2) + 4 * lr;
                if (row < a.Cout) out[(long)row * a.K + col] = acc[i][j][r];
            }
    }
}

template <int N>
__device__ __forceinline__ void wg_wait_vmcnt() {
    static_assert(N >= 0 && N < 64, "vmcnt is a 6-bit field");
    asm volatile("s_waitcnt vmcnt(%0)" ::"n"(N) : "memory");
}
template <int TM, int TN, int NS>
__global__ __launch_bounds__(256) void wgrad_bf16_pipe_kernel(WgArgs a) {
    constexpr int kThreads = 256;
    constexpr int BCO = 2 * TM * 32, BK = 2 * TN * 32;
    constexpr int PA = BCO * 2, PB = BK * 2;
    constexpr int UA = BCO / 8, UB = BK / 8;
    constexpr int NA = BMR16 * UA / kThreads, NB = BMR16 * UB / kThreads;
    constexpr int IPC = NA + NB;
    static_assert(NS >= 3 && (NS - 2) * IPC < 64, "ring depth");
    extern __shared__ __attribute__((aligned(16))) char smem16[];
    char* Ds = smem16;
    char* Xs = smem16 + NS * BMR16 * PA;
    int wg_tile, wg_split;
    if (!wg_map(a.tiles, a.nsplit, wg_tile, wg_split, a.xcd_rr)) return;
    const int tile_k = wg_tile % a.tiles_k, tile_co = wg_tile / a.tiles_k;
    const int co0 = tile_co * BCO, k0 = tile_k * BK;
    const int tid = threadIdx.x, lane = tid & 63, wave = tid >> 6;
    const int wm = wave >> 1, wn = wave & 1;
    const int ra0 = tid / UA, rb0 = tid / UB;
    const int qa = (tid % UA) ^ swz16<UA>(ra0);
    const int qb = (tid % UB) ^ swz16<UB>(rb0);
    const bool co_ok = co0 + qa * 8 < a.Cout;
    const int kcol = k0 + qb * 8;
    const bool k_ok = kcol < a.K;
    const int tap = k_ok ? kcol / a.Cin : 0;
    const int ci = k_ok ? kcol - tap * a.Cin : 0;
    const int kh = tap / a.KW, kw = tap - kh * a.KW;
    const bf16_t* dzp = reinterpret_cast<const bf16_t*>(a.dz);
    const int m_begin = wg_split * a.rows_per_split;
    const int m_end = min(a.M, m_begin + a.rows_per_split);
    const int nchunks = (m_end - m_begin + BMR16 - 1) / BMR16;
    constexpr unsigned kOOB = 0x80000000u;
    const int hw_o = a.Ho * a.Wo;
    const i32x4 gs_dz = rsrc_words(dzp + (long)m_begin * a.Cout, (unsigned)min((long)(m_end - m_begin) * a.Cout * 2, 0x7ffffff0L));
    const bool x2u = a.split_c > 0 && (k0 % a.Cin) < a.split_c;
    const int ps = x2u ? a.x2ps : a.xps;
    const i32x4 gs_x = rsrc_words(x2u ? a.x2 : a.x, (unsigned)min((long)a.N * a.H * a.W * ps * 2, 0x7ffffff0L));
    const unsigned lds_d0 = (unsigned)__builtin_amdgcn_readfirstlane((int)(unsigned)(size_t)(__attribute__((address_space(3))) char*)Ds + (wave * 64 / UA) * PA);
    const unsigned lds_x0 = (unsigned)__builtin_amdgcn_readfirstlane((int)(unsigned)(size_t)(__attribute__((address_space(3))) char*)Xs + (wave * 64 / UB) * PB);
    const unsigned dz_col = (unsigned)(qa * 8 + co0) * 2u;
    const unsigned x_tap = (unsigned)((kh * a.W + kw) * ps + ci) * 2u;
    auto dma_chunk = [&](int c, int buf) {
        const int mc = m_begin + c * BMR16;
#pragma unroll
        for (int i = 0; i < NA; ++i) {
            const int r = c * BMR16 + ra0 + (kThreads / UA) * i;
            const unsigned off = co_ok ? (unsigned)(r * a.Cout) * 2u + dz_col : kOOB;
            glds16(gs_dz, lds_d0 + (unsigned)((buf * BMR16 + (kThreads / UA) * i) * PA), off);
        }
#pragma unroll
        for (int i = 0; i < NB; ++i) {
            const int m = mc + rb0 + (kThreads / UB) * i;
            const int img = wg_fd_div(m, a.fd_hw_mul, a.fd_hw_shr), rem = m - img * hw_o;
            const int oh = wg_fd_div(rem, a.fd_w_mul, a.fd_w_shr), ow = rem - oh * a.Wo;
            const int ih0 = oh * a.stride - a.pad, iw0 = ow * a.stride - a.pad;
            const bool ok = m < m_end && k_ok && (unsigned)(ih0 + kh) < (unsigned)a.H && (unsigned)(iw0 + kw) < (unsigned)a.W;
            const unsigned off = ok ? (unsigned)(((img * a.H + ih0) * a.W + iw0) * ps) * 2u + x_tap : kOOB;
            glds16(gs_x, lds_x0 + (unsigned)((buf * BMR16 + (kThreads / UB) * i) * PB), off);
        }
    };
    const int tg = lane >> 4, ti = lane & 15;
    const int trow = (ti >> 2) + 8 * (tg >> 1);
    const int tunit = 2 * (tg & 1) + ((ti & 3) >> 1), thalf = ti & 1;
    int offA[TM], offB[TN];
#pragma unroll
    for (int i = 0; i < TM; ++i) offA[i] = trow * PA + ((((wm * TM + i) * 4 + tunit) ^ swz16<UA>(trow)) * 16) + thalf * 8;
#pragma unroll
    for (int j = 0; j < TN; ++j) offB[j] = trow * PB + ((((wn * TN + j) * 4 + tunit) ^ swz16<UB>(trow)) * 16) + thalf * 8;
    auto gather = [&](const char* p, int pitch) {
        typedef short v4s __attribute__((ext_vector_type(4)));
        typedef __attribute__((address_space(3))) v4s* lds_v4s;
        const v4s lo = __builtin_amdgcn_ds_read_tr16_b64_v4i16((lds_v4s)(p));
        const v4s hi = __builtin_amdgcn_ds_read_tr16_b64_v4i16((lds_v4s)(p + 4 * pitch));
        bf16x8_t v;
        v[0] = lo[0]; v[1] = lo[1]; v[2] = lo[2]; v[3] = lo[3];
        v[4] = hi[0]; v[5] = hi[1]; v[6] = hi[2]; v[7] = hi[3];
        return v;
    };
    f32x16 acc[TM][TN];
#pragma unroll
    for (int i = 0; i < TM; ++i)
#pragma unroll
        for (int j = 0; j < TN; ++j)
#pragma unroll
            for (int r = 0; r < 16; ++r) acc[i][j][r] = 0.f;
    auto compute = [&](int buf) {
#pragma unroll
        for (int ks = 0; ks < BMR16 / 16; ++ks) {
            const int r0 = buf * BMR16 + ks * 16;
            bf16x8_t fa[TM], fb[TN];
#pragma unroll
            for (int i = 0; i < TM; ++i) fa[i] = gather(Ds + r0 * PA + offA[i], PA);
#pragma unroll
            for (int j = 0; j < TN; ++j) fb[j] = gather(Xs + r0 * PB + offB[j], PB);
#pragma unroll
            for (int i = 0; i < TM; ++i)
#pragma unroll
                for (int j = 0; j < TN; ++j) acc[i][j] = __builtin_amdgcn_mfma_f32_32x32x16_bf16(fa[i], fb[j], acc[i][j], 0, 0, 0);
        }
    };
#pragma unroll
    for (int s_ = 0; s_ < NS - 1; ++s_) dma_chunk(s_, s_);
    for (int cc = 0; cc < nchunks; cc += NS) {
#pragma unroll
        for (int s_ = 0; s_ < NS; ++s_) {
            if (cc + s_ < nchunks) {
                wg_wait_vmcnt<(NS - 2) * IPC>();
                __builtin_amdgcn_s_barrier();
                dma_chunk(cc + s_ + NS - 1, (s_ + NS - 1) % NS);
                compute(s_);
            }
        }
    }
    asm volatile("s_waitcnt vmcnt(0)" ::: "memory");
    float* outp = a.part + (long)wg_split * a.Cout * a.K;
    const int lr = lane >> 5, lc = lane & 31;
#pragma unroll
    for (int j = 0; j < TN; ++j) {
        const int col = k0 + (wn * TN + j) * 32 + lc;
        if (col >= a.K) continue;
#pragma unroll
        for (int i = 0; i < TM; ++i)
#pragma unroll
            for (int r = 0; r < 16; ++r) {
                const int row = co0 + (wm * TM + i) * 32 + (r & 3) + 8 * (r >> 2) + 4 * lr;
                if (row < a.Cout) outp[(long)row * a.K + col] = acc[i][j][r];
            }
    }
}

constexpr int BMRX = 32;
template <int TM, int TN>
__global__ __launch_bounds__(256, 3) void wgrad_x3_kernel(WgArgs a) {
    constexpr int kThreads = 256;
    constexpr int BCO = 2 * TM * 32, BK = 2 * TN * 32;
    constexpr int PA = BCO * 2, PB = BK * 2;
    constexpr int UA = BCO / 8, UB = BK / 8;
    constexpr int QA = BCO / 4, QB = BK / 4;
    constexpr int NA = BMRX * QA / kThreads, NB = BMRX * QB / kThreads;
    __shared__ __attribute__((aligned(16))) char Ds[3 * BMRX * PA];
    __shared__ __attribute__((aligned(16))) char Xs[3 * BMRX * PB];
    int wg_tile, wg_split;
    if (!wg_map(a.tiles, a.nsplit, wg_tile, wg_split, a.xcd_rr)) return;
    const int tile_k = wg_tile % a.tiles_k, tile_co = wg_tile / a.tiles_k;
    const int co0 = tile_co * BCO, k0 = tile_k * BK;
    const int tid = threadIdx.x, lane = tid & 63, wave = tid >> 6;
    const int wm = wave >> 1, wn = wave & 1;
    const int qa = tid % QA, ra0 = tid / QA, qb = tid % QB, rb0 = tid / QB;
    const int co = co0 + qa * 4;
    const bool co_ok = co < a.Cout;
    const int kcol = k0 + qb * 4;
    const bool k_ok = kcol < a.K;
    const int tap = k_ok ? kcol / a.Cin : 0;
    const int ci = k_ok ? kcol - tap * a.Cin : 0;
    const int kh = tap / a.KW, kw = tap - kh * a.KW;
    const bool from2 = a.split_c > 0 && ci < a.split_c;
    const float* xb = reinterpret_cast<const float*>(from2 ? a.x2 : a.x);
    const float* dzp = reinterpret_cast<const float*>(a.dz);
    const int ps = from2 ? a.x2ps : a.xps;

    const int m_begin = wg_split * a.rows_per_split;
    const int m_end = min(a.M, m_begin + a.rows_per_split);
    const int nchunks = (m_end - m_begin + BMRX - 1) / BMRX;

    typedef unsigned u32x4 __attribute__((ext_vector_type(4)));
    constexpr unsigned kOOB = 0x80000000u;
    const int hw_o = a.Ho * a.Wo;
    const __amdgpu_buffer_rsrc_t rs_dz = __builtin_amdgcn_make_buffer_rsrc(
        (void*)(dzp + (long)m_begin * a.Cout), 0, (unsigned)min((long)(m_end - m_begin) * a.Cout * 4, 0x7ffffff0L), 0x00020000);
    uint4 sd[NA], sx[NB];
    unsigned okx = 0u;
    auto load_chunk = [&](int c) {
#pragma unroll
        for (int i = 0; i < NA; ++i) {
            const int r = c * BMRX + ra0 + (kThreads / QA) * i;
            const unsigned off = co_ok ? (unsigned)(r * a.Cout + co) * 4u : kOOB;
            const u32x4 v = __builtin_amdgcn_raw_buffer_load_b128(rs_dz, off, 0, 0);
            sd[i] = make_uint4(v.x, v.y, v.z, v.w);
        }
        okx = 0u;
#pragma unroll
        for (int i = 0; i < NB; ++i) {
            const int m = m_begin + c * BMRX + rb0 + (kThreads / QB) * i;
            const int img = wg_fd_div(m, a.fd_hw_mul, a.fd_hw_shr), rem = m - img * hw_o;
            const int oh = wg_fd_div(rem, a.fd_w_mul, a.fd_w_shr), ow = rem - oh * a.Wo;
            const int ih = oh * a.stride - a.pad + kh, iw = ow * a.stride - a.pad + kw;
            const bool ok = m < m_end && k_ok && (unsigned)ih < (unsigned)a.H && (unsigned)iw < (unsigned)a.W;
            const long off = ok ? ((long)((img * a.H + ih) * a.W + iw) * ps + ci) : 0L;
            sx[i] = *reinterpret_cast<const uint4*>(xb + off);
            okx |= ok ? (1u << i) : 0u;
        }
    };
    auto split3 = [&](const uint4& v, uint2 (&pl)[3]) {
        float r[4] = {__uint_as_float(v.x), __uint_as_float(v.y), __uint_as_float(v.z), __uint_as_float(v.w)};
#pragma unroll
        for (int p = 0; p < 3; ++p) {
            const unsigned lo2 = pack_bf16x2(r[0], r[1]), hi2 = pack_bf16x2(r[2], r[3]);
            pl[p] = make_uint2(lo2, hi2);
            if (p < 2) {
                auto sub1 = [](float x, float y) { float d; asm("v_sub_f32 %0, %1, %2" : "=v"(d) : "v"(x), "v"(y)); return d; };
                r[0] = sub1(r[0], __uint_as_float(lo2 << 16)); r[1] = sub1(r[1], __uint_as_float(lo2 & 0xffff0000u));
                r[2] = sub1(r[2], __uint_as_float(hi2 << 16)); r[3] = sub1(r[3], __uint_as_float(hi2 & 0xffff0000u));
            }
        }
    };
    auto store_chunk = [&]() {
#pragma unroll
        for (int i = 0; i < NA; ++i) {
            const int row = ra0 + (kThreads / QA) * i;
            uint2 pl[3];
            split3(sd[i], pl);
            char* d = Ds + row * PA + ((((qa >> 1) ^ swz16<UA>(row)) << 4) | ((qa & 1) << 3));
#pragma unroll
            for (int p = 0; p < 3; ++p) *reinterpret_cast<uint2*>(d + p * BMRX * PA) = pl[p];
        }
#pragma unroll
        for (int i = 0; i < NB; ++i) {
            const int row = rb0 + (kThreads / QB) * i;
            const bool ok = (okx >> i) & 1u;
            const uint4 v = sx[i];
            uint2 pl[3];
            split3(make_uint4(ok ? v.x : 0u, ok ? v.y : 0u, ok ? v.z : 0u, ok ? v.w : 0u), pl);
            char* d = Xs + row * PB + ((((qb >> 1) ^ swz16<UB>(row)) << 4) | ((qb & 1) << 3));
#pragma unroll
            for (int p = 0; p < 3; ++p) *reinterpret_cast<uint2*>(d + p * BMRX * PB) = pl[p];
        }
    };
    const int tg = lane >> 4, ti = lane & 15;
    const int trow = (ti >> 2) + 8 * (tg >> 1);
    const int tunit = 2 * (tg & 1) + ((ti & 3) >> 1), thalf = ti & 1;
    int offA[TM], offB[TN];
#pragma unroll
    for (int i = 0; i < TM; ++i) offA[i] = trow * PA + ((((wm * TM + i) * 4 + tunit) ^ swz16<UA>(trow)) * 16) + thalf * 8;
#pragma unroll
    for (int j = 0; j < TN; ++j) offB[j] = trow * PB + ((((wn * TN + j) * 4 + tunit) ^ swz16<UB>(trow)) * 16) + thalf * 8;
    auto gather = [&](const char* p, int pitch) {
        typedef short v4s __attribute__((ext_vector_type(4)));
        typedef __attribute__((address_space(3))) v4s* lds_v4s;
        const v4s lo = __builtin_amdgcn_ds_read_tr16_b64_v4i16((lds_v4s)(p));
        const v4s hi = __builtin_amdgcn_ds_read_tr16_b64_v4i16((lds_v4s)(p + 4 * pitch));
        bf16x8_t v;
        v[0] = lo[0]; v[1] = lo[1]; v[2] = lo[2]; v[3] = lo[3];
        v[4] = hi[0]; v[5] = hi[1]; v[6] = hi[2]; v[7] = hi[3];
        return v;
    };

    f32x16 acc[TM][TN];
#pragma unroll
    for (int i = 0; i < TM; ++i)
#pragma unroll
        for (int j = 0; j < TN; ++j)
#pragma unroll
            for (int r = 0; r < 16; ++r) acc[i][j][r] = 0.f;

    auto compute = [&]() {
#pragma unroll
        for (int ks = 0; ks < BMRX / 16; ++ks) {
            bf16x8_t fa[3][TM], fb[3][TN];
#pragma unroll
            for (int p = 0; p < 3; ++p) {
#pragma unroll
                for (int i = 0; i < TM; ++i) fa[p][i] = gather(Ds + (p * BMRX + ks * 16) * PA + offA[i], PA);
#pragma unroll
                for (int j = 0; j < TN; ++j) fb[p][j] = gather(Xs + (p * BMRX + ks * 16) * PB + offB[j], PB);
            }
            constexpr int PA_[6] = {0, 2, 1, 0, 1, 0}, PB_[6] = {2, 0, 1, 1, 0, 0};
#pragma unroll
            for (int t = 0; t < 6; ++t)
#pragma unroll
                for (int i = 0; i < TM; ++i)
#pragma unroll
                    for (int j = 0; j < TN; ++j)
                        acc[i][j] = __builtin_amdgcn_mfma_f32_32x32x16_bf16(fa[PA_[t]][i], fb[PB_[t]][j], acc[i][j], 0, 0, 0);
        }
    };
    load_chunk(0);
    for (int c = 0; c < nchunks; ++c) {
        store_chunk();
        __syncthreads();
        load_chunk(c + 1);
        compute();
        __syncthreads();
    }
// ... 166 lines not shown
        asm volatile("s_waitcnt lgkmcnt(0)" ::: "memory");
        MVF_PIN2(acc[0][0], acc[0][1]); MVF_PIN2(acc[1][0], acc[1][1]);
        MVF_WG_PRIO(1);
#pragma unroll
        for (int ks = 0; ks < 4; ++ks) {
            acc[0][0] = __builtin_amdgcn_mfma_f32_32x32x16_bf16(fd0[ks], fx[0][ks], acc[0][0], 0, 0, 0);
            __builtin_amdgcn_sched_barrier(0); x_step(4 * ks + 0, c + 2); __builtin_amdgcn_sched_barrier(0);
            acc[0][1] = __builtin_amdgcn_mfma_f32_32x32x16_bf16(fd0[ks], fx[1][ks], acc[0][1], 0, 0, 0);
            __builtin_amdgcn_sched_barrier(0); x_step(4 * ks + 1, c + 2); __builtin_amdgcn_sched_barrier(0);
            acc[1][0] = __builtin_amdgcn_mfma_f32_32x32x16_bf16(d1[ks], fx[0][ks], acc[1][0], 0, 0, 0);
            __builtin_amdgcn_sched_barrier(0); x_step(4 * ks + 2, c + 2); __builtin_amdgcn_sched_barrier(0);
            acc[1][1] = __builtin_amdgcn_mfma_f32_32x32x16_bf16(d1[ks], fx[1][ks], acc[1][1], 0, 0, 0);
            __builtin_amdgcn_sched_barrier(0); x_step(4 * ks + 3, c + 2); __builtin_amdgcn_sched_barrier(0);
        }
        MVF_WG_PRIO(0);
        MVF_PIN2(acc[0][0], acc[0][1]); MVF_PIN2(acc[1][0], acc[1][1]);
        __builtin_amdgcn_s_barrier();
    };
    auto phase_y = [&](int c, int buf, bf16x8_t (&d1)[4], bf16x8_t (&d1n)[4]) {
        fetch_x(buf, 2, fx[0]);
        fetch_x(buf, 3, fx[1]);
        __builtin_amdgcn_sched_barrier(0);
        fetch_dz(buf ^ 1, 1, d1n);
        __builtin_amdgcn_sched_barrier(0);
        stage_dz(1, buf, c + 2);
        stage_x(0, buf);
        asm volatile("s_waitcnt vmcnt(6) lgkmcnt(8)" ::: "memory");
        __builtin_amdgcn_s_barrier();
        asm volatile("s_waitcnt lgkmcnt(0)" ::: "memory");
        MVF_PIN2(acc[0][2], acc[0][3]); MVF_PIN2(acc[1][2], acc[1][3]);
        MVF_WG_PRIO(1);
#pragma unroll
        for (int ks = 0; ks < 4; ++ks) {
            acc[0][2] = __builtin_amdgcn_mfma_f32_32x32x16_bf16(fd0[ks], fx[0][ks], acc[0][2], 0, 0, 0);
            acc[0][3] = __builtin_amdgcn_mfma_f32_32x32x16_bf16(fd0[ks], fx[1][ks], acc[0][3], 0, 0, 0);
            acc[1][2] = __builtin_amdgcn_mfma_f32_32x32x16_bf16(d1[ks], fx[0][ks], acc[1][2], 0, 0, 0);
            acc[1][3] = __builtin_amdgcn_mfma_f32_32x32x16_bf16(d1[ks], fx[1][ks], acc[1][3], 0, 0, 0);
        }
        MVF_WG_PRIO(0);
        MVF_PIN2(acc[0][2], acc[0][3]); MVF_PIN2(acc[1][2], acc[1][3]);
        __builtin_amdgcn_s_barrier();
    };
#ifdef MVF_WGRAD_ABLATE
    const int nloop = (a.abl & 1) ? 0 : nchunks;
#else
    const int nloop = nchunks;
#endif
    for (int c = 0; c < nloop; c += 2) {
        phase_x(c, 0, fd1a);
        phase_y(c, 0, fd1a, fd1b);
        if (c + 1 < nchunks) {
            phase_x(c + 1, 1, fd1b);
            phase_y(c + 1, 1, fd1b, fd1a);
        }
    }
    if (grp == 0) __builtin_amdgcn_s_barrier();
    asm volatile("s_waitcnt vmcnt(0)" ::: "memory");
#undef MVF_PIN2
#ifdef MVF_WGRAD_ABLATE
    if (a.abl & 2) {
        if (acc[0][0][0] == 123.456f) a.part[0] = acc[1][3][5];
        return;
    }
#endif
    float* outp = a.part + (long)wg_split * a.Cout * a.K;
    const int lr = lane >> 5, lc = lane & 31;
#pragma unroll
    for (int j = 0; j < 4; ++j) {
        const int col = k0 + (j >> 1) * 128 + wn * 64 + (j & 1) * 32 + lc;
        if (col >= a.K) continue;
#pragma unroll
        for (int i = 0; i < 2; ++i)
#pragma unroll
            for (int r = 0; r < 16; ++r) {
                const int row = co0 + i * 128 + wm * 32 + (r & 3) + 8 * (r >> 2) + 4 * lr;
                if (row < a.Cout) outp[(long)row * a.K + col] = acc[i][j][r];
            }
    }
}

template <int TM, int TN>
int launch_wgrad_bf16(const WgArgs& a, int tiles, int nsplit, hipStream_t st, int& fam, int& stages) {
    constexpr int BCO = 2 * TM * 32, BK = 2 * TN * 32;
    const size_t lds = (size_t)2 * BMR16 * (BCO * 2 + BK * 2);
    static const int dma_env = mvf_policy_int("wgrad_dma", 1);
    const bool dma = dma_env && (a.split_c == 0 || (dma_env != 3 && a.split_c % BK == 0 && a.Cin % BK == 0)) &&
                     (long)a.N * a.H * a.W * std::max(a.xps, a.x2ps) * 2 < 0x7ffffff0L && (dma_env == 2 || (a.K >= 128 && a.Cin >= 32));
    static const int stages_env = mvf_policy_int("wgrad_stages", 3);
    if (dma && stages_env >= 3) {
        const size_t lds_p = (size_t)(stages_env >= 4 ? 4 : 3) * BMR16 * (BCO * 2 + BK * 2);
        auto k3 = wgrad_bf16_pipe_kernel<TM, TN, 3>;
        auto k4 = wgrad_bf16_pipe_kernel<TM, TN, 4>;
        static bool attr_p = false;
        if (!attr_p) {
            MVF_HIP_OK(hipFuncSetAttribute((const void*)k3, hipFuncAttributeMaxDynamicSharedMemorySize, (int)(3 * BMR16 * (BCO * 2 + BK * 2))));
            MVF_HIP_OK(hipFuncSetAttribute((const void*)k4, hipFuncAttributeMaxDynamicSharedMemorySize, (int)(4 * BMR16 * (BCO * 2 + BK * 2))));
            attr_p = true;
        }
        if (stages_env >= 4) hipLaunchKernelGGL(k4, dim3(nsplit * tiles), dim3(kThreads), lds_p, st, a);
        else hipLaunchKernelGGL(k3, dim3(nsplit * tiles), dim3(kThreads), lds_p, st, a);
        MVF_LAUNCH_CHECK();
        fam = MVF_WGRAD_FAM_BF16_PIPE; stages = stages_env >= 4 ? 4 : 3;
        return MVF_OK;
    }
    if (dma) {
        auto kd = wgrad_bf16_kernel<TM, TN, true>;
        static bool attr_d = false;
        if (!attr_d) {
            MVF_HIP_OK(hipFuncSetAttribute((const void*)kd, hipFuncAttributeMaxDynamicSharedMemorySize, (int)lds));
            attr_d = true;
        }
        hipLaunchKernelGGL(kd, dim3(nsplit * tiles), dim3(kThreads), lds, st, a);
        MVF_LAUNCH_CHECK();
        fam = MVF_WGRAD_FAM_BF16_DMA2; stages = 2;
        return MVF_OK;
    }
    auto kern = wgrad_bf16_kernel<TM, TN>;
    static bool attr_done = false;
    if (!attr_done) {
        MVF_HIP_OK(hipFuncSetAttribute((const void*)kern, hipFuncAttributeMaxDynamicSharedMemorySize, (int)lds));
        attr_done = true;
    }
    hipLaunchKernelGGL(kern, dim3(nsplit * tiles), dim3(kThreads), lds, st, a);
    MVF_LAUNCH_CHECK();
    fam = MVF_WGRAD_FAM_BF16_REG; stages = 0;
    return MVF_OK;
}

int launch_wgrad_bf16_big(const WgArgs& a, int tiles, int nsplit, hipStream_t st, int& fam, int& stages) {
    stages = 2;
    constexpr size_t lds = (size_t)2 * BMR16 * (256 * 2 + 256 * 2);
    auto kd = wgrad_bf16_kernel<2, 4, true, 4>;
    auto kp = wgrad_bf16_p4_kernel;
    static bool attr_d = false;
    if (!attr_d) {
        MVF_HIP_OK(hipFuncSetAttribute((const void*)kd, hipFuncAttributeMaxDynamicSharedMemorySize, (int)lds));
        MVF_HIP_OK(hipFuncSetAttribute((const void*)kp, hipFuncAttributeMaxDynamicSharedMemorySize, (int)lds));
        attr_d = true;
    }
    static const int p4_on = mvf_policy_int("wgrad_p4", 1);
    if (p4_on && a.Cin % 64 == 0) {
        hipLaunchKernelGGL(kp, dim3(nsplit * tiles), dim3(512), lds, st, a);
        MVF_LAUNCH_CHECK();
        fam = MVF_WGRAD_FAM_T256_P4;
        return MVF_OK;
    }
    hipLaunchKernelGGL(kd, dim3(nsplit * tiles), dim3(512), lds, st, a);
    MVF_LAUNCH_CHECK();
    fam = MVF_WGRAD_FAM_T256_2B;
    return MVF_OK;
}

__global__ __launch_bounds__(256) void wgrad_reduce1_kernel(const float* part, int nsplit, int cout, int cin, int kh, int kw, int kwp, int cinp,
                                    float* dw) {
    __shared__ float red[4][64];
    const long K = (long)kh * kwp * cinp;
    const long total = (long)cout * K;
    const int e = threadIdx.x & 63, sl = threadIdx.x >> 6;
    const long i = (long)blockIdx.x * 64 + e;
    float s0 = 0.f, s1 = 0.f, s2 = 0.f, s3 = 0.f;
    if (i < total) {
        int k = sl;
        for (; k + 12 < nsplit; k += 16) {
            s0 += part[(long)k * total + i];
            s1 += part[(long)(k + 4) * total + i];
            s2 += part[(long)(k + 8) * total + i];
            s3 += part[(long)(k + 12) * total + i];
        }
        for (; k < nsplit; k += 4) s0 += part[(long)k * total + i];
    }
    red[sl][e] = (s0 + s1) + (s2 + s3);
    __syncthreads();
    if (sl == 0 && i < total) {
        long t = i;
        const int ci = (int)(t % cinp); t /= cinp;
        const int x = (int)(t % kwp); t /= kwp;
        const int y = (int)(t % kh);
        const int co = (int)(t / kh);
        if (ci < cin && x < kw) dw[(((long)co * cin + ci) * kh + y) * kw + x] = (red[0][e] + red[1][e]) + (red[2][e] + red[3][e]);
    }
}
int launch_wgrad_reduce(const float* part, int nsplit, int cout, int cin, int kh, int kw, int kwp, int cinp, float* dw, hipStream_t st) {
    const long total = (long)cout * kh * kwp * cinp;
    hipLaunchKernelGGL(wgrad_reduce1_kernel, dim3((int)((total + 63) / 64)), dim3(256), 0, st, part, nsplit, cout, cin, kh, kw, kwp, cinp, dw);
    MVF_LAUNCH_CHECK();
    return MVF_OK;
}

template <typename ET>
__global__ void pack_dgrad_weight_kernel(const float* w, int cout, int cin, int kh, int kw, ET* out) {
    const long total = (long)cin * kh * kw * cout;
    for (long i = (long)blockIdx.x * blockDim.x + threadIdx.x; i < total; i += (long)gridDim.x * blockDim.x) {
        long t = i;
        const int co = (int)(t % cout); t /= cout;
        const int x = (int)(t % kw); t /= kw;
        const int y = (int)(t % kh);
        const int ci = (int)(t / kh);
        stf(out + i, w[(((long)co * cin + ci) * kh + (kh - 1 - y)) * kw + (kw - 1 - x)]);
    }
}

constexpr int kPackT = 32, kPackTapsMax = 9;
template <typename ET>
__global__ __launch_bounds__(256) void pack_batched_kernel(const mvf_pack_job_t* jobs, int njobs) {
    __shared__ float tile[kPackT * (kPackT * kPackTapsMax + 1)];
    int lo = 0, hi = njobs - 1;
    while (lo < hi) {
        const int mid = (lo + hi + 1) >> 1;
        if (jobs[mid].first_block <= (int)blockIdx.x) lo = mid; else hi = mid - 1;
    }
    const mvf_pack_job_t j = jobs[lo];
    const float* w = j.w;
    ET* out = reinterpret_cast<ET*>(j.out);
    if (j.kind >= 2) {
        const int taps = j.kh * j.kw, run = kPackT * taps, pitch = run + 1;
        const int b = (int)blockIdx.x - j.first_block, tiles_ci = j.cin / kPackT;
        const int co0 = (b / tiles_ci) * kPackT, ci0 = (b % tiles_ci) * kPackT;
        for (int e = threadIdx.x; e < kPackT * run; e += 256) {
            const int r = e / run, q = e - r * run;
            tile[r * pitch + q] = w[((long)(co0 + r) * j.cin + ci0) * taps + q];
        }
        __syncthreads();
        const int l = threadIdx.x & 31, g = threadIdx.x >> 5;
        if (j.kind == 2) {
            for (int p = g; p < kPackT * taps; p += 8) {
                const int r = p / taps, t = p - r * taps;
                stf(out + ((long)(co0 + r) * taps + t) * j.cin + ci0 + l, tile[r * pitch + l * taps + t]);
            }
        } else {
            for (int p = g; p < kPackT * taps; p += 8) {
                const int c = p / taps, t = p - c * taps;
                stf(out + ((long)(ci0 + c) * taps + t) * j.cout + co0 + l, tile[l * pitch + c * taps + (taps - 1 - t)]);
            }
        }
        return;
    }
    const long base = (long)((int)blockIdx.x - j.first_block) * 2048;
    const long total = j.kind == 0 ? (long)j.cout * j.kh * j.kw_pad * j.cin_pad : (long)j.cin * j.kh * j.kw * j.cout;
#pragma unroll
    for (int u = 0; u < 8; ++u) {
        const long i = base + u * 256 + threadIdx.x;
        if (i >= total) break;
        long t = i;
        float v = 0.f;
        if (j.kind == 0) {
            const int ci = (int)(t % j.cin_pad); t /= j.cin_pad;
            const int x = (int)(t % j.kw_pad); t /= j.kw_pad;
            const int yk = (int)(t % j.kh);
            const int co = (int)(t / j.kh);
            if (ci < j.cin && x < j.kw) v = w[(((long)co * j.cin + ci) * j.kh + yk) * j.kw + x];
        } else {
            const int co = (int)(t % j.cout); t /= j.cout;
            const int x = (int)(t % j.kw); t /= j.kw;
            const int y = (int)(t % j.kh);
            const int ci = (int)(t / j.kh);
            v = w[(((long)co * j.cin + ci) * j.kh + (j.kh - 1 - y)) * j.kw + (j.kw - 1 - x)];
        }
        stf(out + i, v);
    }
}

int plan_split(int M, int tiles, int target_override = 0, int* target_used = nullptr) {
    static const int target_env = std::max(64, mvf_policy_int("wgrad_wgs", 1024));
    const int target = target_override > 0 ? target_override : target_env;
    if (target_used) *target_used = target;
    int want = std::max(1, target / std::max(tiles, 1));
    int rows = std::max((M + want - 1) / want, 256);
    rows = (rows + 63) / 64 * 64;
    return rows;
}

struct WgTile { int bco, bk; };
WgTile pick_tile(int cout, int K) {
    if (cout <= 64) return {64, 128};
    if (K <= 64) return {128, 64};
    return {128, 128};
}

}

namespace mvf_internal {
int wgrad_slab_reduce_launch(const float* part, int nsplit, int cout, int k, float* dw_oihw, hipStream_t st) {
    return launch_wgrad_reduce(part, nsplit, cout, k, 1, 1, 1, k, dw_oihw, st);
}
}

extern "C" {

static bool wg_big_shape(const mvf_conv_desc_t* d) {
    static const int big_env = mvf_policy_int("wgrad_big", 1);
    const long K = (long)d->kh * d->kw * d->cin;
    if (big_env >= 2 && (d->kh != 1 || d->kw != 1)) return false;
    if (big_env >= 3 && d->cout < 512) return false;
    return big_env && d->dtype == MVF_BF16 && d->cout % 256 == 0 && K % 256 == 0 && d->cin % 8 == 0 && d->x_pix_stride % 4 == 0 &&
           (d->split_c == 0 || (d->split_c % 256 == 0 && d->cin % 256 == 0));
}
static int wg_big_rows(const mvf_conv_desc_t* d, int wgs_override = 0, int* target_used = nullptr) {
    const int M = d->n * d->ho * d->wo, K = d->kh * d->kw * d->cin;
    static const int big_wgs = std::max(32, mvf_policy_int("wgrad_big_wgs", 128));
    return plan_split(M, (d->cout / 256) * (K / 256), wgs_override > 0 ? wgs_override : big_wgs, target_used);
}

static bool wg_direct3x3(const mvf_conv_desc_t* d) {
    return d->dtype == MVF_BF16 && d->cin == 64 && d->cout == 64 && d->kh == 3 && d->kw == 3 && d->stride == 1 && d->pad == 1 && d->split_c == 0 &&
           d->ho == d->h && d->wo == d->w && mvf_internal::wgrad3x3_c64_ok(d->n, d->h, d->w, d->x_pix_stride);
}

static bool wg_direct_stem(const mvf_conv_desc_t* d) {
    return d->dtype == MVF_BF16 && d->cin == 32 && d->cout == 64 && d->kh == 7 && d->kw == 1 && d->stride == 2 && d->pad == 0 && d->split_c == 0 &&
           d->x_pix_stride == 4 && mvf_internal::wgrad_stem_ok(d->n, d->h, d->w, d->ho, d->wo);
}

size_t mvf_conv2d_wgrad_workspace_bytes(const mvf_conv_desc_t* d) {
    if (!d || d->cout <= 0 || d->cin <= 0) return 0;
    const int M = d->n * d->ho * d->wo, K = d->kh * d->kw * d->cin;
    const WgTile t = pick_tile(d->cout, K);
    const int tiles = ((d->cout + t.bco - 1) / t.bco) * ((K + t.bk - 1) / t.bk);
    const int rows = plan_split(M, tiles);
    int nsplit = (M + rows - 1) / rows;
    if (wg_big_shape(d)) nsplit = std::max(nsplit, (M + wg_big_rows(d) - 1) / wg_big_rows(d));
    if (wg_direct3x3(d)) nsplit = std::max(nsplit, mvf_internal::wgrad3x3_c64_wgs(d->n, d->h));
    if (wg_direct_stem(d)) nsplit = std::max(nsplit, mvf_internal::wgrad_stem_wgs(d->n, d->ho));
    return align_up((size_t)nsplit * d->cout * K * sizeof(float), 256);
}

}
static int wgrad_impl(const mvf_conv_desc_t* d, const void* dz, const void* x, const void* x2, int kw_real, int cin_real,
                      int kw_packed, int cin_packed, float* dw_oihw, void* ws, size_t ws_bytes, void* stream, int wgs_target) {
    t_last_wgrad = mvf_wgrad_launch_info_t{};
    MVF_REQUIRE(d && dz && x && dw_oihw, MVF_EINVAL, "wgrad: NULL argument");
    MVF_REQUIRE(d->dtype == MVF_F32 || d->dtype == MVF_BF16, MVF_EINVAL, "wgrad: bad dtype");
    MVF_REQUIRE(d->cin % 4 == 0 && d->cout % 4 == 0 && d->x_pix_stride > 0, MVF_ESHAPE, "wgrad: cin/cout must be multiples of 4");
    MVF_REQUIRE(kw_packed * cin_packed == d->kw * d->cin && kw_real <= kw_packed && cin_real <= cin_packed, MVF_EINVAL, "wgrad: packed extents inconsistent");
    MVF_REQUIRE(ws && ws_bytes >= mvf_conv2d_wgrad_workspace_bytes(d), MVF_EWS, "wgrad: workspace too small");
    if (d->split_c) MVF_REQUIRE(x2 && d->kh == 1 && d->kw == 1 && d->split_c % 4 == 0, MVF_EINVAL, "wgrad: bad split_c");
    hipStream_t st0 = (hipStream_t)stream;
    if (wg_direct3x3(d) && kw_real == 3 && cin_real == 64 && kw_packed == 3 && cin_packed == 64 && ((uintptr_t)dz | (uintptr_t)x) % 16 == 0) {
        Wgrad3x3C64Args w = {dz, x, (float*)ws, d->n, d->h, d->w, d->x_pix_stride, mvf_internal::wgrad3x3_c64_wgs(d->n, d->h)};
        const int rc = mvf_internal::wgrad3x3_c64_launch(w, st0);
        if (rc != MVF_OK) return rc;
        t_last_wgrad = mvf_wgrad_launch_info_t{MVF_WGRAD_FAM_C3X3_C64, 0, 64, 576, MVF_BF16, w.nwg, 0, 0, 0, 0, 0, 1};
        const int rr = launch_wgrad_reduce((const float*)ws, w.nwg, 64, 64, 3, 3, 3, 64, dw_oihw, st0);
        if (rr == MVF_OK) t_last_wgrad.launches = 2;
        return rr;
    }
    if (wg_direct_stem(d) && kw_real == 7 && cin_real == 3 && kw_packed == 8 && cin_packed == 4 && ((uintptr_t)dz | (uintptr_t)x) % 16 == 0) {
        WgradStemArgs w = {dz, x, (float*)ws, d->n, d->h, d->w, d->ho, d->wo, mvf_internal::wgrad_stem_wgs(d->n, d->ho)};
        const int rc = mvf_internal::wgrad_stem_launch(w, st0);
        if (rc != MVF_OK) return rc;
        t_last_wgrad = mvf_wgrad_launch_info_t{MVF_WGRAD_FAM_STEM, 0, 64, 224, MVF_BF16, w.nwg, 0, 0, 0, 0, 0, 1};
        const int rr = launch_wgrad_reduce((const float*)ws, w.nwg, 64, 3, 7, 7, 8, 4, dw_oihw, st0);
        if (rr == MVF_OK) t_last_wgrad.launches = 2;
        return rr;
    }
    WgArgs a = {};
    a.dz = dz; a.x = x; a.x2 = x2; a.part = (float*)ws;
    a.N = d->n; a.H = d->h; a.W = d->w; a.Cin = d->cin; a.Cout = d->cout; a.KH = d->kh; a.KW = d->kw;
    a.stride = d->stride; a.pad = d->pad; a.Ho = d->ho; a.Wo = d->wo; a.xps = d->x_pix_stride;
    a.split_c = d->split_c; a.x2ps = d->x2_pix_stride;
    a.M = d->n * d->ho * d->wo; a.K = d->kh * d->kw * d->cin;
    WgTile t = pick_tile(d->cout, a.K);
    static const int gram_env = std::max(8, mvf_policy_int("gram_wgs", 32));
    const bool gram = wgs_target <= 0 && dz == x && !x2 && d->kh == 1 && d->kw == 1 && d->cin == d->cout;
    const int gram_wgs = wgs_target > 0 ? wgs_target : gram ? gram_env : 0;
    bool big = wg_big_shape(d) && wgs_target <= 0 && ((uintptr_t)dz | (uintptr_t)x | (uintptr_t)(x2 ? x2 : x)) % 16 == 0 &&
               (long)a.N * a.H * a.W * std::max(a.xps, a.x2ps) * 2 < 0x7ffffff0L;
    if (big) {
        const int rows = wg_big_rows(d, gram_wgs);
        big = rows >= 4 * 64 && ((long)rows + 6 * 64) * d->cout * 2 < 0x7ffffff0L;
        if (big) t = WgTile{256, 256};
    }
    a.tiles_k = (a.K + t.bk - 1) / t.bk;
    const int tiles = ((d->cout + t.bco - 1) / t.bco) * a.tiles_k;
    static const int x3_env = (mvf_policy_int("f32_x3", 1) != 0) && (mvf_policy_int("wgrad_x3", 1) != 0);
    bool x3 = d->dtype == MVF_F32 && x3_env && d->cin % 4 == 0 && d->cout % 4 == 0 && d->x_pix_stride % 4 == 0 && d->split_c % 4 == 0 &&
              (d->x2_pix_stride % 4 == 0 || !d->split_c) && ((uintptr_t)dz | (uintptr_t)x | (uintptr_t)(x2 ? x2 : x)) % 16 == 0;
    static const bool wgs_forced = mvf_policy_has("wgrad_wgs");
    const int bf16_wgs = (d->dtype == MVF_BF16 && !wgs_forced) ? 256 : 0;
    int target_used = 0;
    a.rows_per_split = big ? wg_big_rows(d, gram_wgs, &target_used) : plan_split(a.M, tiles, gram_wgs ? gram_wgs : (x3 && !wgs_forced ? 768 : bf16_wgs), &target_used);
    if (wgs_target > 0) {
        const long fit = std::max<long>(1, (long)(mvf_conv2d_wgrad_workspace_bytes(d) / ((size_t)d->cout * a.K * sizeof(float))));
        if ((a.M + a.rows_per_split - 1) / a.rows_per_split > fit) a.rows_per_split = std::max(a.rows_per_split, (int)(((a.M + fit - 1) / fit + 63) / 64 * 64));
    }
    x3 = x3 && ((long)a.rows_per_split + 64) * d->cout * 4 < 0x7ffffff0L;
    if (d->dtype == MVF_F32 && !x3 && !wgs_forced && !gram_wgs) a.rows_per_split = plan_split(a.M, tiles, 0, &target_used);
    const int nsplit = (a.M + a.rows_per_split - 1) / a.rows_per_split;
    MVF_REQUIRE(ws_bytes >= (size_t)nsplit * d->cout * a.K * sizeof(float), MVF_EWS, "wgrad: workspace too small for %d slabs", nsplit);
    a.tiles = tiles;
    a.nsplit = nsplit;
    a.xcd_rr = nsplit % 8 == 0;
#ifdef MVF_WGRAD_ABLATE
    a.abl = mvf_policy_int("wgrad_abl", 0);
#endif
    wg_fd_make((unsigned)(a.Ho * a.Wo), a.fd_hw_mul, a.fd_hw_shr);
    wg_fd_make((unsigned)a.Wo, a.fd_w_mul, a.fd_w_shr);
    hipStream_t st = (hipStream_t)stream;
    static const int dma32_env = mvf_policy_int("wgrad_dma_f32", 1);
    const bool dma32 = d->dtype == MVF_F32 && dma32_env && d->cin % 4 == 0 && d->cout % 4 == 0 && d->x_pix_stride % 4 == 0 &&
                       (a.split_c == 0 || (a.split_c % t.bk == 0 && a.Cin % t.bk == 0)) &&
                       ((uintptr_t)dz | (uintptr_t)x | (uintptr_t)(x2 ? x2 : x)) % 16 == 0 &&
                       (long)a.N * a.H * a.W * std::max(a.xps, a.x2ps) * 4 < 0x7ffffff0L && ((long)a.rows_per_split + 64) * d->cout * 4 < 0x7ffffff0L;
    int fam = MVF_WGRAD_FAM_NONE, stages = 0;
    if (x3) {
        fam = MVF_WGRAD_FAM_X3;
        if (t.bco == 64) hipLaunchKernelGGL((wgrad_x3_kernel<1, 2>), dim3(nsplit * tiles), dim3(256), 0, st, a);
        else if (t.bk == 64) hipLaunchKernelGGL((wgrad_x3_kernel<2, 1>), dim3(nsplit * tiles), dim3(256), 0, st, a);
        else hipLaunchKernelGGL((wgrad_x3_kernel<2, 2>), dim3(nsplit * tiles), dim3(256), 0, st, a);
    } else if (dma32) {
        fam = MVF_WGRAD_FAM_F32_DMA; stages = 2;
        if (t.bco == 64) hipLaunchKernelGGL((wgrad_kernel<float, 1, 2, true>), dim3(nsplit * tiles), dim3(kThreads), 0, st, a);
        else if (t.bk == 64) hipLaunchKernelGGL((wgrad_kernel<float, 2, 1, true>), dim3(nsplit * tiles), dim3(kThreads), 0, st, a);
        else hipLaunchKernelGGL((wgrad_kernel<float, 2, 2, true>), dim3(nsplit * tiles), dim3(kThreads), 0, st, a);
    } else if (d->dtype == MVF_F32) {
        fam = MVF_WGRAD_FAM_F32_REG;
        if (t.bco == 64) hipLaunchKernelGGL((wgrad_kernel<float, 1, 2>), dim3(nsplit * tiles), dim3(kThreads), 0, st, a);
        else if (t.bk == 64) hipLaunchKernelGGL((wgrad_kernel<float, 2, 1>), dim3(nsplit * tiles), dim3(kThreads), 0, st, a);
        else hipLaunchKernelGGL((wgrad_kernel<float, 2, 2>), dim3(nsplit * tiles), dim3(kThreads), 0, st, a);
    } else if (d->cin % 8 == 0 && d->cout % 8 == 0 && d->x_pix_stride % 4 == 0 && (d->split_c % 8) == 0 &&
               ((uintptr_t)dz | (uintptr_t)x | (uintptr_t)(x2 ? x2 : x)) % 16 == 0 &&
               ((long)a.rows_per_split + 6 * 64) * d->cout * 2 < 0x7ffffff0L) {
        int rc;
        if (big) rc = launch_wgrad_bf16_big(a, tiles, nsplit, st, fam, stages);
        else if (t.bco == 64) rc = launch_wgrad_bf16<1, 2>(a, tiles, nsplit, st, fam, stages);
        else if (t.bk == 64) rc = launch_wgrad_bf16<2, 1>(a, tiles, nsplit, st, fam, stages);
        else rc = launch_wgrad_bf16<2, 2>(a, tiles, nsplit, st, fam, stages);
        if (rc) return rc;
    } else {
        fam = MVF_WGRAD_FAM_BF16_WIDEN;
        if (t.bco == 64) hipLaunchKernelGGL((wgrad_kernel<bf16_t, 1, 2>), dim3(nsplit * tiles), dim3(kThreads), 0, st, a);
        else if (t.bk == 64) hipLaunchKernelGGL((wgrad_kernel<bf16_t, 2, 1>), dim3(nsplit * tiles), dim3(kThreads), 0, st, a);
        else hipLaunchKernelGGL((wgrad_kernel<bf16_t, 2, 2>), dim3(nsplit * tiles), dim3(kThreads), 0, st, a);
    }
    MVF_LAUNCH_CHECK();
    t_last_wgrad = mvf_wgrad_launch_info_t{fam, stages, t.bco, t.bk, d->dtype, nsplit, a.rows_per_split, a.xcd_rr, a.split_c > 0 ? 1 : 0, gram ? 1 : 0, target_used, 1};
    const int kh_p = d->kh * d->kw * d->cin / (kw_packed * cin_packed);
    const int rr = launch_wgrad_reduce(a.part, nsplit, d->cout, cin_real, kh_p, kw_real, kw_packed, cin_packed, dw_oihw, st);
    if (rr == MVF_OK) t_last_wgrad.launches = 2;
    return rr;
}
extern "C" {

int mvf_conv2d_nhwc_wgrad(const mvf_conv_desc_t* d, const void* dz, const void* x, const void* x2, int kw_real, int cin_real,
                          int kw_packed, int cin_packed, float* dw_oihw, void* ws, size_t ws_bytes, void* stream) {
    return wgrad_impl(d, dz, x, x2, kw_real, cin_real, kw_packed, cin_packed, dw_oihw, ws, ws_bytes, stream, 0);
}

int mvf_conv2d_nhwc_wgrad_wgs(const mvf_conv_desc_t* d, const void* dz, const void* x, const void* x2, int kw_real, int cin_real,
                              int kw_packed, int cin_packed, float* dw_oihw, void* ws, size_t ws_bytes, int wgs, void* stream) {
    t_last_wgrad = mvf_wgrad_launch_info_t{};
    MVF_REQUIRE(wgs >= 8 && wgs <= 4096, MVF_EINVAL, "wgrad_wgs: wgs=%d outside 8 .. 4096", wgs);
    return wgrad_impl(d, dz, x, x2, kw_real, cin_real, kw_packed, cin_packed, dw_oihw, ws, ws_bytes, stream, wgs);
}

int mvf_conv2d_wgrad_last_launch(mvf_wgrad_launch_info_t* out) {
    MVF_REQUIRE(out, MVF_EINVAL, "conv2d_wgrad_last_launch: NULL argument");
    *out = t_last_wgrad;
    return MVF_OK;
}

int mvf_pack_conv_weights_batched(const mvf_pack_job_t* jobs_dev, int njobs, int total_blocks, int dtype, void* stream) {
    MVF_REQUIRE(jobs_dev && njobs > 0 && total_blocks > 0 && (dtype == MVF_F32 || dtype == MVF_BF16), MVF_EINVAL, "pack_conv_weights_batched: bad argument");
    if (dtype == MVF_F32)
        hipLaunchKernelGGL(pack_batched_kernel<float>, dim3(total_blocks), dim3(256), 0, (hipStream_t)stream, jobs_dev, njobs);
    else
        hipLaunchKernelGGL(pack_batched_kernel<bf16_t>, dim3(total_blocks), dim3(256), 0, (hipStream_t)stream, jobs_dev, njobs);
    MVF_LAUNCH_CHECK();
    return MVF_OK;
}

int mvf_pack_conv_weight_dgrad(const float* w_oihw, int cout, int cin, int kh, int kw, void* w_packed, int dtype, void* stream) {
    MVF_REQUIRE(w_oihw && w_packed && cout > 0 && cin > 0 && kh > 0 && kw > 0, MVF_EINVAL, "pack_conv_weight_dgrad: bad argument");
    const long total = (long)cout * cin * kh * kw;
    const int blocks = (int)std::min<long>((total + 255) / 256, 4096);
    if (dtype == MVF_F32)
        hipLaunchKernelGGL(pack_dgrad_weight_kernel<float>, dim3(blocks), dim3(256), 0, (hipStream_t)stream, w_oihw, cout, cin, kh, kw, (float*)w_packed);
    else
        hipLaunchKernelGGL(pack_dgrad_weight_kernel<bf16_t>, dim3(blocks), dim3(256), 0, (hipStream_t)stream, w_oihw, cout, cin, kh, kw, (bf16_t*)w_packed);
    MVF_LAUNCH_CHECK();
    return MVF_OK;
}

}
```

### mvfnet_amd/train_engine.py

```python
import ctypes as C
import os

import torch

from . import _lib
from ._lib import ConvDesc, MvfDesc, check
from .heads import loss_calls

F32 = _lib.MVF_F32

_ConvDescT, _MvfDescT = ConvDesc, MvfDesc
_DESC_CACHE = {}


def ConvDesc(*a):
    d = _DESC_CACHE.get(a)
    if d is None:
        d = _DESC_CACHE[a] = _ConvDescT(*a)
    return d


def MvfDesc(*a):
    k = ("mvf",) + a
    d = _DESC_CACHE.get(k)
# ... 306 lines not shown
            check(self.eng.lib.mvf_bn_bwd_finalize(_p(part), 2 * ns, self.cout, _p(bn.dgamma), _p(bn.dbeta), _st()), "mvf_bn_bwd_finalize")
        elif not sums_done:
            part = self.eng.buf((id(self), "bwpart"), (rows, self.cout, 2), torch.float32)
            self.launch_bwd_sums(d, a_in, g, bits, bn, part, ws)
            check(self.eng.lib.mvf_bn_bwd_finalize(_p(part), rows, self.cout, _p(bn.dgamma), _p(bn.dbeta), _st()), "mvf_bn_bwd_finalize")
        dx = self.eng.buf((id(self), "dx"), (m, self.cin))
        spart = self.eng.buf((id(self), "bnsums_fused"), (self.cin, 2 * ns, 2), torch.float32) if bn_in is not None else None
        slabs = self.eng.buf((id(self), "wslab"), (ns * self.cout * self.cin,), torch.float32)
        self.launch_bwd_fused(m, a_in, g, bits, bn, bn_in, z_in, dx, spart, ns, slabs, pitch)
        if bn_in is not None:
            check(self.eng.lib.mvf_bn_bwd_finalize(_p(spart), 2 * ns, self.cin, _p(bn_in.dgamma), _p(bn_in.dbeta), _st()), "bn bwd finalize")
        self.slab_reduce(slabs, ns, self.eng)
        return dx

    def launch_bwd_sums1(self, m, a_in, a_pitch, g, bits, bn, part, ns):
        check(self.eng.lib.mvf_conv1x1_bnbwd_sums_pair(_p(a_in), a_pitch, _p(self.wp), None, 0, None, _p(g), self.cout, _p(bits), m, self.cout, self.cin, _p(bn.mean),
                                              _p(bn.invstd), None, None, _p(part), None, 2 * ns, self.eng.dt, _st()), "bn backward sums (one branch)")

    def launch_bwd_fused(self, m, a_in, g, bits, bn, bn_in, z_in, dx, spart, ns, slabs, a_pitch=None):
        i = bn_in
        check(self.eng.lib.mvf_conv1x1_bwd_fused(_p(a_in), a_pitch or self.cin, _p(self.wp), _p(g), self.cout, _p(bits), m, self.cout, self.cin, _p(bn.gamma), _p(bn.mean),
                                        _p(bn.invstd), _p(bn.dgamma), _p(bn.dbeta), _p(z_in) if i is not None else None, _p(i.mean) if i else None,
                                        _p(i.invstd) if i else None, _p(i.scale) if i else None, _p(i.shift) if i else None,
                                        _p(dx), _p(spart), 2 * ns, _p(slabs), slabs.numel() * 4, self.eng.dt, _st()), "conv1x1 backward fused")

    def launch_bwd_sums(self, d, a_in, g, bits, bn, part, ws):
        check(self.eng.lib.mvf_conv2d_nhwc_fwd_bnbwd_sums(C.byref(d), _p(a_in), None, _p(self.wp), _p(g), _p(bits), _p(bn.mean), _p(bn.invstd), _p(part),
                                                 _p(ws), ws.numel(), _st()), "conv + bn backward sums")

    def launch_bwd_apply(self, d, a_in, g, bits, bn, dz, ws):
        check(self.eng.lib.mvf_conv2d_nhwc_fwd_bnbwd_apply(C.byref(d), _p(a_in), None, _p(self.wp), _p(g), _p(bits), _p(bn.gamma), _p(bn.mean), _p(bn.invstd),
                                                  _p(bn.dgamma), _p(bn.dbeta), _p(dz), _p(ws), ws.numel(), _st()), "conv + bn backward apply")

    def launch_fwd_apply(self, d, x, bn, residual, rbn, out, bits, ws):
        check(self.eng.lib.mvf_conv2d_nhwc_fwd_bnapply(C.byref(d), _p(x), None, _p(self.wp), _p(bn.scale), _p(bn.shift), _p(residual),
                                              _p(rbn.scale if rbn else None), _p(rbn.shift if rbn else None), _p(out), _p(bits),
                                              _p(ws), ws.numel(), _st()), "conv fwd + bn apply")

    def launch_fwd(self, d, x, x2, z, ws, part, shift):
        if part is None:
            check(self.eng.lib.mvf_conv2d_nhwc_fwd_ws(C.byref(d), _p(x), _p(x2), _p(self.wp), None, None, _p(z), _p(ws), ws.numel(), _st()), "conv fwd")
        else:
            check(self.eng.lib.mvf_conv2d_nhwc_fwd_stats(C.byref(d), _p(x), _p(x2), _p(self.wp), _p(z), _p(part), _p(shift), _p(ws), ws.numel(), _st()),
                  "conv fwd+stats")

    def wgrad(self, dz, x, n, h, w, ho, wo, eng, x_pitch=None, x2=None, split_c=0, on_main=False):
        d = self.desc(n, h, w, ho, wo, x_pitch or self.cin, split_c)
        kwr, cinr, kwp, cinp = (self.kw, self.cin, 8, 4) if self.stem else (self.kw, self.cin, self.kw, self.cin)
        nbytes = self.eng.lib.mvf_conv2d_wgrad_workspace_bytes(C.byref(d))
        side = None if on_main else eng.side_stream()
        if side is None:
            ws = eng.workspace(nbytes)
            check(self.eng.lib.mvf_conv2d_nhwc_wgrad(C.byref(d), _p(dz), _p(x), _p(x2), kwr, cinr, kwp, cinp, _p(self.dw), _p(ws), ws.numel(), _st()), "conv wgrad")
            return
        ws = eng.workspace(nbytes, side=True)

        def launch():
            check(self.eng.lib.mvf_conv2d_nhwc_wgrad(C.byref(d), _p(dz), _p(x), _p(x2), kwr, cinr, kwp, cinp, _p(self.dw), _p(ws), ws.numel(), _st()), "conv wgrad")
        eng.on_side(launch)

    def fuses_wgrad(self, eng, m, c, mask_mode, nbn=1):
        return (eng.tdtype == torch.bfloat16 and self.kh == 1 and self.kw == 1 and self.stride == 1 and not self.stem and c == self.cout and
                self.eng.lib.mvf_bn_bwd_wgrad_splits(m, c, self.cin, nbn, mask_mode) > 0)

    def slab_reduce(self, slabs, ns, eng):
        def launch():
            check(self.eng.lib.mvf_wgrad_slab_reduce(_p(slabs), ns, self.cout, self.cin, _p(self.dw), _st()), "wgrad slab reduce")
        if eng.side_stream() is None:
            launch()
        else:
            eng.on_side(launch)

    def dgrad_bnsums(self, dz, n, ho, wo, h, w, bn, z):
        d = ConvDesc(n, ho, wo, self.cout, self.cin, self.kh, self.kw, 1, self.kh - 1 - self.pad, h, w, self.cout, self.eng.dt, 0, 0, 0,
                     self.stride if self.stride > 1 else 0, 0)
        dx = self.eng.buf((id(self), "dx"), (n * h * w, self.cin))
        ws = _conv_ws(dz.device)
        rows = _stats_rows(d)
        part = self.eng.buf((id(self), "bnsums"), (rows, self.cin, 2), torch.float32)
        self.launch_dgrad_bnsums(d, dz, dx, z, bn, part, ws)
        check(self.eng.lib.mvf_bn_bwd_finalize(_p(part), rows, self.cin, _p(bn.dgamma), _p(bn.dbeta), _st()), "bn bwd finalize")
        return dx

    def launch_dgrad_bnsums(self, d, dz, dx, z, bn, part, ws):
        check(self.eng.lib.mvf_conv2d_nhwc_dgrad_bnsums(C.byref(d), _p(dz), _p(self.wd), _p(dx), _p(z), _p(bn.mean), _p(bn.invstd), _p(bn.scale), _p(bn.shift),
                                               _p(part), _p(ws), ws.numel(), _st()), "conv dgrad+bn sums")

    def dgrad(self, dz, n, ho, wo, h, w, residual=None, res_c0=0, res_bits=None, out_gate=None, gsum=None):
        d = ConvDesc(n, ho, wo, self.cout, self.cin, self.kh, self.kw, 1, self.kh - 1 - self.pad, h, w, self.cout, self.eng.dt, 0, 0, 0,
                     self.stride if self.stride > 1 else 0, res_c0)
        dx = self.eng.buf((id(self), "dx"), (n * h * w, self.cin))
        ws = _conv_ws(dz.device)
        if out_gate is not None and gsum is not None:
            bn = gsum["bn"]
            rows = _stats_rows(d)
            part = self.eng.buf((id(bn), "gsum_conv"), (self.cin, rows, 2), torch.float32)
            check(self.eng.lib.mvf_conv2d_nhwc_fwd_resmask_gate_colsums(C.byref(d), _p(dz), None, _p(self.wd), _p(residual), _p(res_bits), _p(out_gate), _p(dx), _p(part), _p(ws),
                                                               ws.numel(), _st()), "conv dgrad (gated output + column sums)")
            bn._s1 = [None, 0, res_c0, part, rows]
        elif out_gate is not None:
            check(self.eng.lib.mvf_conv2d_nhwc_fwd_resmask_gate(C.byref(d), _p(dz), None, _p(self.wd), None, _p(residual), _p(res_bits), _p(out_gate), _p(dx), _p(ws),
                                                       ws.numel(), _st()), "conv dgrad (gated output)")
        else:
            check(self.eng.lib.mvf_conv2d_nhwc_fwd_resmask(C.byref(d), _p(dz), None, _p(self.wd), None, _p(residual), _p(res_bits), _p(dx), _p(ws), ws.numel(),
                                                  _st()), "conv dgrad")
        return dx

    def dzfree_ok(self, m):
        return (self.eng.tdtype == torch.bfloat16 and self.kh == 1 and self.kw == 1 and self.stride == 1 and not self.stem and
                self.cout % 256 == 0 and self.cin % 64 == 0 and self.cout <= 4096 and m * (self.cout + self.cin) * 2 < 0x7ffffff0)

    def dzfree_dgrad(self, gm, a_in, bn, n, h, w, bn_in, z_in, frozen_zero=None):
        eng = self.eng
        c, k, m = self.cout, self.cin, n * h * w
        bd = eng.buf((id(self), "dzfree_w"), (k, c + k))
        bias = eng.buf((id(self), "dzfree_b"), (k,), torch.float32)
        sg, sb = (frozen_zero, frozen_zero) if frozen_zero is not None else (bn.dgamma, bn.dbeta)
        check(self.eng.lib.mvf_bn_bwd_dzfree_prep(_p(self.wd), c, k, _p(bn.gamma), _p(bn.mean), _p(bn.invstd), _p(sg), _p(sb), m, _p(bd), _p(bias), eng.dt, _st()),
              "bn backward without dz: operands")
        d = ConvDesc(n, h, w, c + k, k, 1, 1, 1, 0, h, w, k, eng.dt, 0, c, c, 0, 0, c)
        dx = eng.buf((id(self), "dx"), (m, k))
        ws = _conv_ws(gm.device)
        rows = _stats_rows(d)
        part = eng.buf((id(self), "bnsums"), (rows, k, 2), torch.float32)
        self.launch_dzfree_dgrad(d, a_in, gm, bd, bias, dx, z_in, bn_in, part, ws)
        check(self.eng.lib.mvf_bn_bwd_finalize(_p(part), rows, k, _p(bn_in.dgamma), _p(bn_in.dbeta), _st()), "bn bwd finalize")
        return dx

    def launch_dzfree_dgrad(self, d, a_in, gm, bd, bias, dx, z_in, bn_in, part, ws):
        check(self.eng.lib.mvf_conv2d_nhwc_dgrad_bnsums_split(C.byref(d), _p(a_in), _p(gm), _p(bd), _p(bias), _p(dx), _p(z_in), _p(bn_in.mean), _p(bn_in.invstd),
                                                     _p(bn_in.scale), _p(bn_in.shift), _p(part), _p(ws), ws.numel(), _st()), "conv dgrad on [gm | a] + bn sums")

    def dzfree_q_sums(self, gm, a_in, bn, n, h, w, eng):
        c, k = self.cout, self.cin
        d = self.desc(n, h, w, h, w, k, 0)
        ws = eng.workspace(self.eng.lib.mvf_conv2d_wgrad_workspace_bytes(C.byref(d)))
        self.launch_q(d, gm, a_in, ws, eng.dzfree_q_wgs)
        lo, rows_lo, c_split, hi, rows_hi = bn._s1
        assert c_split == 0 or lo is not None, "the MVF slice's column sums are missing"
        check(self.eng.lib.mvf_bn_bwd_dzfree_sums(_p(self.dw), _p(self.wp), c, k, _p(bn.mean), _p(bn.invstd), _p(lo), rows_lo, c_split, _p(hi), rows_hi, _p(bn.dgamma),
                                         _p(bn.dbeta), eng.dt, _st()), "bn backward sums from the weight-gradient GEMM")
        bn._s1 = None

    def launch_q(self, d, gm, a_in, ws, wgs):
        check(self.eng.lib.mvf_conv2d_nhwc_wgrad_wgs(C.byref(d), _p(gm), _p(a_in), None, self.kw, self.cin, self.kw, self.cin, _p(self.dw), _p(ws), ws.numel(), wgs, _st()),
              "conv wgrad (launch stream)")

    def gram_ok(self):
        return (self.eng.tdtype == torch.bfloat16 and self.kh == 1 and self.kw == 1 and self.stride == 1 and not self.stem and
                self.cin % 32 == 0 and self.cout % 32 == 0)

    def gram_stats(self, a_in, bn, n, h, w, eng, means_done=False):
        c, k, m = self.cout, self.cin, n * h * w
        gram = eng.buf((id(self), "gram"), (k, k), torch.float32)
        amean = eng.buf((id(self), "amean"), (4, k), torch.float32)
        d = ConvDesc(n, h, w, k, k, 1, 1, 1, 0, h, w, k, eng.dt, 0, 0, 0, 0)
        ws = eng.workspace(max(self.eng.lib.mvf_conv2d_wgrad_workspace_bytes(C.byref(d)), self.eng.lib.mvf_bn_workspace_bytes(m, k), (eng.gram_stats_wgs + 8) * k * k * 4))
        if k not in eng._ones:
            eng._ones[k] = (torch.ones(k, device=a_in.device), torch.zeros(k, device=a_in.device))
        one, zero = eng._ones[k]
        self.launch_gram(d, a_in, gram, ws, eng.gram_stats_wgs)
        if not means_done:
            check(self.eng.lib.mvf_bn_train_stats(_p(a_in), m, k, _p(one), _p(zero), C.c_float(1e-5), C.c_float(0.1), None, None, _p(amean[0]), _p(amean[1]),
                                         _p(amean[2]), _p(amean[3]), _p(ws), ws.numel(), eng.dt, _st()), "column means")
        check(self.eng.lib.mvf_bn_train_stats_gram(_p(gram), _p(amean[0]), _p(self.wp), m, c, k, _p(bn.gamma), _p(bn.beta), C.c_float(bn.eps), C.c_float(bn.momentum),
                                          _p(bn.mod.running_mean), _p(bn.mod.running_var), _p(bn.mean), _p(bn.invstd), _p(bn.scale), _p(bn.shift), eng.dt,
                                          _st()), "bn statistics from the Gram matrix")
        bn._count()

    def launch_gram(self, d, a_in, gram, ws, wgs):
        k = self.cin
        check(self.eng.lib.mvf_conv2d_nhwc_wgrad_wgs(C.byref(d), _p(a_in), _p(a_in), None, 1, k, 1, k, _p(gram), _p(ws), ws.numel(), wgs, _st()), "gram (launch stream)")

    def dzfree_wgrad(self, gm, a_in, bn, n, h, w, eng, frozen_zero=None, q_done=False, gram_done=False):
        c, k, m = self.cout, self.cin, n * h * w
        if not q_done:
            self.wgrad(gm, a_in, n, h, w, h, w, eng)
        gram = eng.buf((id(self), "gram"), (k, k), torch.float32)
        amean = eng.buf((id(self), "amean"), (4, k), torch.float32)
        d = ConvDesc(n, h, w, k, k, 1, 1, 1, 0, h, w, k, eng.dt, 0, 0, 0, 0)
        nbytes = max(self.eng.lib.mvf_conv2d_wgrad_workspace_bytes(C.byref(d)), self.eng.lib.mvf_bn_workspace_bytes(m, k))
        if k not in eng._ones:
            eng._ones[k] = (torch.ones(k, device=gm.device), torch.zeros(k, device=gm.device))
        one, zero = eng._ones[k]
        sg, sb = (frozen_zero, frozen_zero) if frozen_zero is not None else (bn.dgamma, bn.dbeta)
        side = eng.side_stream()
        ws = eng.workspace(nbytes, side=side is not None)

        def launch():
            if not gram_done:
                check(self.eng.lib.mvf_conv2d_nhwc_wgrad(C.byref(d), _p(a_in), _p(a_in), None, 1, k, 1, k, _p(gram), _p(ws), ws.numel(), _st()), "gram")
                check(self.eng.lib.mvf_bn_train_stats(_p(a_in), m, k, _p(one), _p(zero), C.c_float(1e-5), C.c_float(0.1), None, None, _p(amean[0]), _p(amean[1]),
                                             _p(amean[2]), _p(amean[3]), _p(ws), ws.numel(), eng.dt, _st()), "column means")
            check(self.eng.lib.mvf_bn_bwd_dzfree_wgrad(_p(self.dw), _p(self.wp), _p(gram), _p(amean[0]), _p(bn.gamma), _p(bn.mean), _p(bn.invstd), _p(sg), _p(sb),
                                              m, c, k, eng.dt, _st()), "weight gradient without dz: correction")
        if side is None:
            launch()
        else:
            eng.on_side(launch)


class _TMvf(object):
    def __init__(self, mvf, eng):
        self.eng = eng
        self.cs, self.T = mvf.num_shift_channel, mvf.n_segment
        self.mode = _lib.MODE_BITS[mvf.mode]
        self.share, self.use_hs = mvf.share, mvf.use_hs
        cs = self.cs
        self.wt = mvf.shift_conv.weight
        self.wh = mvf.shift_conv.weight if mvf.share else (mvf.h_conv.weight if self.mode & 2 else None)
        self.ww = mvf.shift_conv.weight if mvf.share else (mvf.w_conv.weight if self.mode & 4 else None)
        self.dwt = eng.grad_of(mvf.shift_conv.weight)
        self.dwh = None if mvf.share or not (self.mode & 2) else eng.grad_of(mvf.h_conv.weight)
        self.dww = None if mvf.share or not (self.mode & 4) else eng.grad_of(mvf.w_conv.weight)
        self.bn = _BN(mvf.bn, eng, "mvf.bn") if self.use_hs else None
        dev = mvf.shift_conv.weight.device
        self.tmp_h = torch.empty(cs, 3, device=dev) if self.dwh is None else None
        self.tmp_w = torch.empty(cs, 3, device=dev) if self.dww is None else None

    def desc(self, nt, h, w, c):
        return MvfDesc(nt, c, h, w, self.T, self.cs, self.mode, _lib.MVF_NHWC, self.eng.dt)

    def forward(self, x, nt, h, w, c, eng):
        m = nt * h * w
        d = self.desc(nt, h, w, c)
        y = self.eng.buf((id(self), "y"), (m, self.cs))
        if self.use_hs and eng.fuse_mvf_stats and eng.fuse_stats and not self.bn.frozen and self.cs % 4 == 0:
            rows = self.eng.lib.mvf_nhwc_stencil_stats_rows(C.byref(d), c, self.cs)
            part = self.eng.buf((id(self), "part"), (self.cs, rows, 2), torch.float32)
            self.launch_stencil_stats(d, x, c, y, part)
            self.bn.finalize(part, rows, m)
            return y, self.bn.apply(y, m, 2)
        self.launch_stencil(d, x, c, y, self.cs, 0, None, 0, None)
        if not self.use_hs:
            return y, y
        self.bn.stats(y, m, eng)
        return y, self.bn.apply(y, m, 2)

    def launch_stencil_stats(self, d, x, c, y, part):
        check(self.eng.lib.mvf_nhwc_stencil_stats(C.byref(d), _p(x), c, _p(y), self.cs, _p(self.wt), _p(self.wh), _p(self.ww), _p(part), _p(self.bn.mod.running_mean),
                                         _st()), "mvf stencil + statistics")

    def backward(self, dxp, x, y, nt, h, w, c, eng, addend=None, addend_bits=None, out_gate=None, gsum=None):
        m = nt * h * w
        d = self.desc(nt, h, w, c)
        if self.use_hs:
            dy = self.bn.backward(dxp, c, y, m, eng, 3)
        else:
            dy = dxp[:, : self.cs].contiguous()
        nbytes = self.eng.lib.mvf_nhwc_tapgrad_workspace_bytes(C.byref(d))
        dwh = self.dwh if self.dwh is not None else self.tmp_h
        dww = self.dww if self.dww is not None else self.tmp_w
        side = eng.side_stream() if (self.use_hs and not self.share) else None
        if side is None:
            ws = eng.workspace(nbytes)
            check(self.eng.lib.mvf_nhwc_tapgrad(C.byref(d), _p(x), c, _p(dy), self.cs, _p(self.dwt), _p(dwh), _p(dww), _p(ws), ws.numel(), _st()), "mvf tapgrad")
            if self.share:
                self.dwt.view(self.cs, 3).add_(dwh.view(self.cs, 3) if self.mode & 2 else 0).add_(dww.view(self.cs, 3) if self.mode & 4 else 0)
        else:
            ws = eng.workspace(nbytes, side=True)

            def launch():
                check(self.eng.lib.mvf_nhwc_tapgrad(C.byref(d), _p(x), c, _p(dy), self.cs, _p(self.dwt), _p(dwh), _p(dww), _p(ws), ws.numel(), _st()), "mvf tapgrad")
            eng.on_side(launch)
        self.launch_stencil(d, dy, self.cs, dxp, c, 1, addend, c if addend is not None else 0, addend_bits, out_gate, gsum)

    def launch_stencil(self, d, src, src_c, dst, dst_c, flip, addend, addend_c, addend_bits, out_gate=None, gsum=None):
        if out_gate is not None and gsum is not None:
            bn = gsum["bn"]
            rows = self.eng.lib.mvf_nhwc_stencil_stats_rows(C.byref(d), src_c, dst_c)
            part = self.eng.buf((id(bn), "gsum_mvf"), (self.cs, rows, 2), torch.float32)
            check(self.eng.lib.mvf_nhwc_stencil_gate_colsums(C.byref(d), _p(src), src_c, _p(dst), dst_c, _p(self.wt), _p(self.wh), _p(self.ww), flip, _p(addend), addend_c,
                                                    _p(addend_bits), _p(out_gate), _p(part), _st()), "mvf stencil (gated output + column sums)")
            bn._s1[0], bn._s1[1] = part, rows
            return
        if out_gate is not None:
            check(self.eng.lib.mvf_nhwc_stencil_gate(C.byref(d), _p(src), src_c, _p(dst), dst_c, _p(self.wt), _p(self.wh), _p(self.ww), None, None, flip,
                                            _p(addend), addend_c, _p(addend_bits), _p(out_gate), _st()), "mvf stencil (gated output)")
            return
        check(self.eng.lib.mvf_nhwc_stencil(C.byref(d), _p(src), src_c, _p(dst), dst_c, _p(self.wt), _p(self.wh), _p(self.ww), None, None, flip,
                                   _p(addend), addend_c, _p(addend_bits), _st()), "mvf stencil")


class _TBlock(object):
    def __init__(self, blk, eng):
        from .modules.MVF import MVF
        c1 = blk.conv1
        self.mvf = None
        if isinstance(c1, MVF):
            if c1.num_shift_channel:
                self.mvf = _TMvf(c1, eng)
            c1 = c1.net
        self.c1, self.b1 = _TConv(c1, eng), _BN(blk.bn1, eng, "bn1")
        self.c2, self.b2 = _TConv(blk.conv2, eng), _BN(blk.bn2, eng, "bn2")
        self.c3, self.b3 = _TConv(blk.conv3, eng), _BN(blk.bn3, eng, "bn3")
        self.cd = self.bd = None
        if blk.downsample is not None:
            self.cd, self.bd = _TConv(blk.downsample[0], eng), _BN(blk.downsample[1], eng, "down")
        self.split_ok = self.mvf is not None and self.mvf.cs % (32 if eng.tdtype == torch.float32 else 64) == 0

    def convs(self):
        return [c for c in (self.c1, self.c2, self.c3, self.cd) if c is not None]

    def fuse_apply(self, eng):
        if self.drop is not None:
            return False
        f = eng.fuse_bn3_apply
        return f == 2 or (f == 1 and self.c3.cin <= 128)

    def z3_free(self, eng, m2=None):
        m2 = m2 or (1 << 16)
        if self.cd is not None:
            return self.z3_free_ds(eng, m2)
        if not (eng.z3_free and self.fuse_apply(eng) and eng.fuse_stats and not self.b3.frozen):
            return False
        if self.q_z3_free(eng, m2):
            return True
        if (eng.fuse_bnwg & 8) and eng.tdtype == torch.bfloat16 and eng.lib.mvf_bn_bwd_wgrad_splits(m2, self.c3.cout, self.c3.cin, 1, 4) > 0:
            return False
        return eng.z3_free == 2 or self.c3.cin <= 64

    def z3_free_ds(self, eng, m2=1 << 16):
        if not (eng.z3_free_ds and eng.z3_free and eng.fuse_c3_bwd and eng.fuse_bn_bwd_sums and eng.fuse_stats and self.fuse_apply(eng) and eng.tdtype == torch.bfloat16):
            return False
        if self.b3.frozen or self.bd.frozen or self.cd.stride != 1 or self.cd.kh != 1 or self.cd.kw != 1 or self.cd.cin != self.c3.cin or self.cd.cout != self.c3.cout:
            return False
        return eng.lib.mvf_conv1x1_bwd_fused_splits(m2, self.c3.cout, self.c3.cin) > 0

    above = None
    drop = None

    def q_policy(self, eng, m2):
        return eng.dzfree_q == 2 or (eng.dzfree_q == 1 and eng.dzfree_q_mink <= self.c3.cin <= eng.dzfree_q_maxk and m2 * self.c3.cout * 4 >= 160e6)

    def _dzfree_base(self, eng, m2):
        if not eng.dzfree or self.cd is not None or not eng.fuse_bn_bwd_sums or not self.c3.dzfree_ok(m2 or (1 << 16)):
            return False
        return eng.dzfree == 2 or self.c3.cin >= 256

    def gram_fwd(self, eng, m2):
        if not (eng.gram_stats and eng.tdtype == torch.bfloat16 and self.cd is None and self.c3.gram_ok() and self.fuse_apply(eng) and eng.fuse_stats and
                not self.b3.frozen and eng.z3_free):
            return False
        return self.z3_free(eng, m2)

    def q_z3_free(self, eng, m2):
        return bool(eng.gram_stats and self.c3.gram_ok() and eng.gate_producer and self.above is not None and
                    not self.b3.frozen and self.fuse_apply(eng) and self._dzfree_base(eng, m2) and self.q_policy(eng, m2))

    def dzfree(self, eng, m2=None):
        if self.drop is not None or self.cd is not None or (self.z3_free(eng, m2) and not self.q_z3_free(eng, m2 or (1 << 16))):
            return False
        return self._dzfree_base(eng, m2)

    def wants_gated_gradient(self, eng):
        s = self.saved
        if s is None or not eng.gate_producer or not self.dzfree(eng, s["out"].shape[0]):
            return None
        q = self.q_policy(eng, s["out"].shape[0])
        sums = "s1" if (q and not self.b3.frozen) else False
        if s["z3"] is None and sums != "s1":
            return None
        return dict(bits=s["bits"], z3=s["z3"], bn=self.b3, sums=sums)

    def launch_sums_pair(self, a2, x, x_pitch, g, bits, m, eng):
        c3, cd = self.c3, self.cd
        ns = eng.lib.mvf_conv1x1_bwd_fused_splits(m, c3.cout, c3.cin)
        pa = eng.buf((id(c3), "bwpart_pair"), (c3.cout, 2 * ns, 2), torch.float32)
        pb = eng.buf((id(cd), "bwpart_pair"), (c3.cout, 2 * ns, 2), torch.float32)
        check(eng.lib.mvf_conv1x1_bnbwd_sums_pair(_p(a2), c3.cin, _p(c3.wp), _p(x), x_pitch, _p(cd.wp), _p(g), c3.cout, _p(bits), m, c3.cout, c3.cin, _p(self.b3.mean),
                                              _p(self.b3.invstd), _p(self.bd.mean), _p(self.bd.invstd), _p(pa), _p(pb), 2 * ns, eng.dt, _st()), "bn backward sums (pair)")
        check(eng.lib.mvf_bn_bwd_finalize(_p(pa), 2 * ns, c3.cout, _p(self.b3.dgamma), _p(self.b3.dbeta), _st()), "mvf_bn_bwd_finalize")
        check(eng.lib.mvf_bn_bwd_finalize(_p(pb), 2 * ns, c3.cout, _p(self.bd.dgamma), _p(self.bd.dbeta), _st()), "mvf_bn_bwd_finalize")

    def forward(self, x, nt, h, w, c, eng):
        m = nt * h * w
        s = dict(x=x, h=h, w=w, c=c)
        if self.drop is not None and (self.drop.numel() != nt or self.drop.dtype != torch.float32):
            raise ValueError("drop path: a float32 scale per image is expected (%d images, got %d %s)" % (nt, self.drop.numel(), self.drop.dtype))
        side = eng.side_stream() if (self.cd is not None and eng.overlap_downsample and eng.fuse_stats) else None
        if side is not None:
            eng._wait(side, eng.main_stream())
            with _on_stream(side):
                zd, _, _ = self.cd.forward(x, nt, h, w, bn=self.bd)
        if self.mvf is not None:
            s["y"], o = self.mvf.forward(x, nt, h, w, c, eng)
            if self.split_ok:
                s["o"] = o
                z1, _, _ = self.c1.forward(x, nt, h, w, c, x2=o, split_c=self.mvf.cs, bn=self.b1)
            else:
                xin = x.clone()
                xin[:, : self.mvf.cs] = o
                s["xin"] = xin
                z1, _, _ = self.c1.forward(xin, nt, h, w, c, bn=self.b1)
        else:
            z1, _, _ = self.c1.forward(x, nt, h, w, c, bn=self.b1)
        a1 = self.b1.apply(z1, m, 1)
        z2, ho, wo = self.c2.forward(a1, nt, h, w, bn=self.b2)
        m2 = nt * ho * wo
        gram = self.gram_fwd(eng, m2)
        cs = gram and eng.gram_colsums and self.b2.c % 8 == 0
        if cs:
            amean = eng.buf((id(self.c3), "amean"), (4, self.c3.cin), torch.float32)
            a2 = self.b2.apply_colmeans(z2, m2, 1, amean[0])
        else:
            a2 = self.b2.apply(z2, m2, 1)
        if gram:
            self.c3.gram_stats(a2, self.b3, nt, ho, wo, eng, means_done=cs)
            z3 = None
        else:
            z3, _, _ = self.c3.forward(a2, nt, ho, wo, bn=self.b3, store=not self.z3_free(eng, m2))
        if self.cd is not None:
            if side is not None:
                eng._wait(eng.main_stream(), side)
            else:
                zd, _, _ = self.cd.forward(x, nt, h, w, bn=self.bd)
            if self.drop is not None:
                out, bits = self.b3.apply_rowscale(z3, m2, 1, zd, self.drop, ho * wo, rbn=self.bd)
            elif self.fuse_apply(eng):
                out, bits = self.c3.forward_apply(a2, nt, ho, wo, self.b3, zd, self.bd)
            else:
                out, bits = self.b3.apply(z3, m2, 1, residual=zd, rbn=self.bd, bits=True)
            s["zd"] = zd
        elif self.drop is not None:
            out, bits = self.b3.apply_rowscale(z3, m2, 1, x, self.drop, ho * wo)
        elif self.fuse_apply(eng):
            out, bits = self.c3.forward_apply(a2, nt, ho, wo, self.b3, x)
        else:
            out, bits = self.b3.apply(z3, m2, 1, residual=x, bits=True)
        s.update(z1=z1, a1=a1, z2=z2, a2=a2, z3=z3, out=out, bits=bits, ho=ho, wo=wo, gram=gram, drop=self.drop)
        self.saved = s
        return out, ho, wo, self.c3.cout

    def backward(self, g, nt, eng, g_gated=False, gate=None, sums_done=False):
        out_gate = gate["bits"] if gate is not None else None
        gsum = gate if (gate is not None and gate["sums"]) else None
        s = self.saved
        h, w, c, ho, wo = s["h"], s["w"], s["c"], s["ho"], s["wo"]
        m, m2 = nt * h * w, nt * ho * wo
        bits = s["bits"]
        self.gated_out = self.sums_out = False
        if g_gated:
            assert self.dzfree(eng, m2), "a gated gradient was produced for a block that does not take it"
        dzd = resid_ds = None
        w3_done = wd_done = False
        q_first = s["z3"] is None and g_gated and sums_done == "s1"
        if s["drop"] is not None:
            assert not g_gated and s["z3"] is not None
            gm = self.b3.gate_rowscale(g, self.c3.cout, bits, m2, s["drop"], ho * wo)
            dz3 = self.b3.backward(gm, self.c3.cout, s["z3"], m2, eng, 0)
            del gm
        elif self.cd is not None and s["z3"] is None:
            pair = bool(eng.pair_ds_sums & 1)
            if pair:
                self.launch_sums_pair(s["a2"], s["x"], c, g, bits, m2, eng)
            da2 = self.c3.bwd_fused(s["a2"], g, bits, nt, ho, wo, self.b3, self.b2, s["z2"], sums_done=pair)
            resid_ds = self.cd.bwd_fused(s["x"], g, bits, nt, h, w, self.bd, a_pitch=c, sums_done=pair)
            dz3, w3_done, wd_done = None, True, True
        elif self.cd is not None and eng.pair_bn_bwd and not (self.b3.frozen or self.bd.frozen):
            if (eng.fuse_bnwg & 2) and self.c3.fuses_wgrad(eng, m2, self.c3.cout, 4, 2):
                both = self.cd.stride == 1 and self.cd.cin == self.c3.cin and self.cd.kh == 1 and self.c3.cin == 64
                dz3, dzd = _BN.backward_pair_wgrad(self.b3, self.bd, g, self.c3.cout, s["z3"], s["zd"], m2, eng, bits, self.c3, s["a2"], self.c3.cin,
                                                   self.cd, s["x"] if both else None, c)
                w3_done, wd_done = True, both
            else:
                dz3, dzd = _BN.backward_pair(self.b3, self.bd, g, self.c3.cout, s["z3"], s["zd"], m2, eng, bits)
        elif s["z3"] is None and not q_first and eng.fuse_c3_bwd and eng.fuse_bn_bwd_sums and self.c3.bwd_fused_ok(m2):
            da2 = self.c3.bwd_fused(s["a2"], g, bits, nt, ho, wo, self.b3, self.b2, s["z2"])
            dz3, w3_done = None, True
        elif s["z3"] is None and not q_first:
            dz3 = self.c3.bwd_recompute(s["a2"], g, bits, nt, ho, wo, self.b3)
        elif self.dzfree(eng, m2):
            b3 = self.b3
            q_done = False
            if g_gated:
                gm = g
                if sums_done == "s1":
                    self.c3.dzfree_q_sums(gm, s["a2"], b3, nt, ho, wo, eng)
                    q_done = True
                elif not sums_done:
                    b3._reduce(gm, self.c3.cout, s["z3"], m2, eng, 0, None, None)
            else:
                assert s["z3"] is not None
                gm = eng.buf((id(b3), "gm"), s["z3"].shape, s["z3"].dtype)
                b3._reduce(g, self.c3.cout, s["z3"], m2, eng, 4, bits, gm)
            fz = b3._zero if b3.frozen else None
            da2 = self.c3.dzfree_dgrad(gm, s["a2"], b3, nt, ho, wo, self.b2, s["z2"], frozen_zero=fz)
            self.c3.dzfree_wgrad(gm, s["a2"], b3, nt, ho, wo, eng, frozen_zero=fz, q_done=q_done, gram_done=bool(s.get("gram")))
            dz3, w3_done = None, True
            del gm
        elif (eng.fuse_bnwg & 1) and self.c3.fuses_wgrad(eng, m2, self.c3.cout, 4):
            dz3 = self.b3.backward_wgrad(g, self.c3.cout, s["z3"], m2, eng, 4, bits, self.c3, s["a2"], self.c3.cin)
            w3_done = True
        else:
            dz3 = self.b3.backward(g, self.c3.cout, s["z3"], m2, eng, 4, ymask=bits)
        eng.issue_marked()
        fuse = eng.fuse_bn_bwd_sums
        if dz3 is None:
            pass
        elif fuse:
            da2 = self.c3.dgrad_bnsums(dz3, nt, ho, wo, ho, wo, self.b2, s["z2"])
        else:
            da2 = self.c3.dgrad(dz3, nt, ho, wo, ho, wo)
        if not w3_done:
            self.c3.wgrad(dz3, s["a2"], nt, ho, wo, ho, wo, eng)
        del dz3
        dz2 = self.b2.backward(da2, self.c2.cout, s["z2"], m2, eng, 2, sums_done=fuse)
        del da2
        fuse1 = fuse and (self.c2.stride == 1 or eng.fuse_bn_bwd_strided)
        if fuse1:
            da1 = self.c2.dgrad_bnsums(dz2, nt, ho, wo, h, w, self.b1, s["z1"])
        else:
            da1 = self.c2.dgrad(dz2, nt, ho, wo, h, w)
        self.c2.wgrad(dz2, s["a1"], nt, h, w, ho, wo, eng)
        del dz2
        w1_done = (eng.fuse_bnwg & 4) and self.mvf is None and self.c1.fuses_wgrad(eng, m, self.c1.cout, 2)
        if w1_done:
            dz1 = self.b1.backward_wgrad(da1, self.c1.cout, s["z1"], m, eng, 2, None, self.c1, s["x"], c, sums_done=fuse1)
        else:
            dz1 = self.b1.backward(da1, self.c1.cout, s["z1"], m, eng, 2, sums_done=fuse1)
        del da1
        resid, rbits = (g, None) if g_gated else (g, bits)
        if resid_ds is not None:
            resid, rbits = resid_ds, None
        elif self.cd is not None:
            if dzd is None:
                dzd = self.bd.backward(g, self.cd.cout, s["zd"], m2, eng, 4, ymask=bits)
            resid, rbits = self.cd.dgrad(dzd, nt, ho, wo, h, w), None
            if not wd_done:
                self.cd.wgrad(dzd, s["x"], nt, h, w, ho, wo, eng, x_pitch=c)
            del dzd
        if self.mvf is None:
            dx = self.c1.dgrad(dz1, nt, h, w, h, w, residual=resid, res_bits=rbits, out_gate=out_gate, gsum=gsum)
            self.gated_out, self.sums_out = out_gate is not None, (gsum["sums"] if gsum is not None else False)
            if not w1_done:
                self.c1.wgrad(dz1, s["x"], nt, h, w, h, w, eng, x_pitch=c)
        else:
            fuse = self.mvf.cs % 4 == 0
            og = out_gate if fuse else None
            gs = gsum if fuse else None
            dxp = self.c1.dgrad(dz1, nt, h, w, h, w, residual=resid if fuse else None, res_c0=self.mvf.cs, res_bits=rbits if fuse else None, out_gate=og, gsum=gs)
            self.gated_out, self.sums_out = og is not None, (gs["sums"] if gs is not None else False)
            if self.split_ok:
                self.c1.wgrad(dz1, s["x"], nt, h, w, h, w, eng, x_pitch=c, x2=s["o"], split_c=self.mvf.cs)
            else:
                self.c1.wgrad(dz1, s["xin"], nt, h, w, h, w, eng, x_pitch=c)
            self.mvf.backward(dxp, s["x"], s["y"], nt, h, w, c, eng, addend=resid if fuse else None, addend_bits=rbits if fuse else None, out_gate=og, gsum=gs)
            if not fuse:
                if rbits is not None:
                    resid = resid * (s["out"] > 0).to(resid.dtype)
                dx = eng.add(dxp, resid, key=id(self))
            else:
                dx = dxp
        if eng.keep_io:
            self.io = dict(x=s["x"], out=s["out"], g=g, dx=dx, h=h, w=w, c=c, ho=ho, wo=wo, g_gated=g_gated, dx_gated=self.gated_out)
        self.saved = None
        eng.flush_side(late=True)
        return dx


class _StatTable(object):

    def __init__(self, eng, bns):
        self.eng = eng
        names = {id(m_): n_ for n_, m_ in eng.model.named_modules()}
        segs, self.keys, self.slices, first = [], [], [], 0
        for bn in bns:
            for attr in ("running_mean", "running_var"):
                t = getattr(bn.mod, attr)
                segs.append(_lib.StatSegment(t.data_ptr(), first))
                self.keys.append("%s.%s" % (names[id(bn.mod)], attr))
                self.slices.append((first, t.numel(), tuple(t.shape)))
                first += t.numel()
        self.bns, self.nseg, self.n = list(bns), len(segs), first
        arr = (_lib.StatSegment * len(segs))(*segs)
        self.dev = torch.frombuffer(bytearray(bytes(arr)), dtype=torch.uint8).to(eng.device)
        self.acc = torch.zeros(first, dtype=torch.float64, device=eng.device)
        self.shadow = torch.empty(first, dtype=torch.float32, device=eng.device)

    def accumulate(self):
        check(self.eng.lib.mvf_bn_stats_accumulate(_p(self.dev), self.nseg, self.n, _p(self.acc), _st()), "bn stats accumulate")

    def finalize(self, count, dst=None):
        check(self.eng.lib.mvf_bn_stats_finalize(_p(self.dev), self.nseg, self.n, _p(self.acc), count, _p(dst), _st()), "bn stats finalize")

    def exchange(self, flat, mode):
        check(self.eng.lib.mvf_bn_stats_exchange(_p(self.dev), self.nseg, self.n, _p(flat), mode, _st()), "bn stats exchange")


class _ParamStore(object):

    lib = _lib.lib

    def _init_store(self, model, dtype=torch.float32, rehome=True):
        if dtype not in (torch.float32, torch.bfloat16):
            raise TypeError("training dtype must be float32 or bfloat16 (activation storage; weights/statistics/gradients stay fp32)")
        self.tdtype = dtype
        self.dt = _lib.MVF_F32 if dtype == torch.float32 else _lib.MVF_BF16
        dev = next(model.parameters()).device
        if dev.type != "cuda":
            raise RuntimeError("the HIP training engine needs the model on an MI355X device; no CPU fallback")
        self.model, self.device = model, dev
        self._side_pending = []
        self._side_keep = []
        params = [p for p in model.parameters()]
        n = sum(p.numel() for p in params)
        pad = lambda k: (k + 3) // 4 * 4
        total = sum(pad(p.numel()) for p in params)
        self.rehomed = bool(rehome)
        self.flat_params = torch.zeros(total, device=dev) if rehome else None
        self.flat_grads = torch.zeros(total, device=dev)
        self.flat_mom = torch.zeros(total, device=dev) if rehome else None
        self._grad_view = {}
        off = 0
        with torch.no_grad():
            for p in params:
                k = p.numel()
                if rehome:
                    v = self.flat_params[off:off + k].view(p.shape)
                    v.copy_(p.data.float())
                    p.data = v
                elif p.dtype != torch.float32 or not p.is_contiguous() or p.device != dev:
                    raise TypeError("stand-alone block: parameters must be contiguous float32 tensors on %s" % dev)
                gv = self.flat_grads[off:off + k].view(p.shape)
                self._grad_view[id(p)] = gv
                off += pad(k)
        self.n_params = n
        if rehome:
            for m_ in model.modules():
                if hasattr(m_, "invalidate_engine"):
                    m_.invalidate_engine()
        self._ws = None
        self.norm_out = torch.zeros(2, device=dev)
        self.steps = 0
        self.ema_momentum, self.ema_warmup_steps, self.ema_updates = None, 0, 0
        self._ones = {}
        self._bufs = {}
        self._caps = {}
        self._last_shape = {}

    def grad_of(self, p):
        return self._grad_view[id(p)]

    def buf(self, key, shape, dtype=None):
        dt = dtype or self.tdtype
        shape = tuple(shape)
        k = (key, shape, dt)
        step = getattr(self, "forward_count", None)
        if step is not None:
            last = self._last_shape.get((key, dt))
            if last is not None and last[0] == step and last[1] != shape:
                raise RuntimeError("engine buffer %r requested with shapes %s and %s inside one step: they would share storage" % (key, last[1], shape))
            self._last_shape[(key, dt)] = (step, shape)
        t = self._bufs.get(k)
        if t is None:
            n = 1
            for v in shape:
                n *= int(v)
            ck = (key, dt)
            flat = self._caps.get(ck)
            if flat is None or flat.numel() < n:
                if flat is not None:
                    self._side_keep.append(flat)
                    self._storage_epoch += 1
                    for kk in [kk for kk in self._bufs if kk[0] == key and kk[2] == dt]:
                        del self._bufs[kk]
                flat = torch.empty(max(n, 1), device=self.device, dtype=dt)
                self._caps[ck] = flat
            t = flat[:n].view(shape)
            self._bufs[k] = t
        return t

    def workspace(self, nbytes, side=False):
        key = "_ws_side" if side else "_ws"
        ws = getattr(self, key, None)
        if ws is None or ws.numel() < nbytes:
            if ws is not None:
                self._storage_epoch += 1
            ws = torch.empty(max(int(nbytes), 1 << 20), dtype=torch.uint8, device=self.device)
            setattr(self, key, ws)
        return ws

    _storage_epoch = 0

    overlap_wgrad = True
    keep_io = False
    fuse_stats = True
    overlap_downsample = _policy("side_downsample", 1) != 0
    z3_free = _policy("z3_free", 1)
    fuse_bn3_apply = _policy("fuse_bn3_apply", 1)
    fuse_bn_bwd_sums = _policy("fuse_bn_bwd", 1) != 0
    fuse_bn_bwd_strided = _policy("fuse_bn_bwd_strided", 1) != 0
    pair_bn_bwd = _policy("pair_bn_bwd", 1) != 0
    fuse_bnwg = _policy("fuse_bnwg", 7)
    pair_ds_sums = _policy("pair_ds_sums", 3)
    z3_free_ds = _policy("z3_free_ds", 1)
    fuse_c3_bwd = _policy("fuse_c3_bwd", 1)
    fuse_mvf_stats = _policy("fuse_mvf_stats", 1) != 0
    dzfree = _policy("dzfree", 2)
    gate_producer = _policy("gate_producer", 1) != 0
    dzfree_q = _policy("dzfree_q", 1)
    dzfree_q_wgs = _policy("dzfree_q_wgs", 256)
    dzfree_q_maxk = _policy("dzfree_q_maxk", 256)
    dzfree_q_mink = _policy("dzfree_q_mink", 0)
    gram_stats = _policy("gram_stats", 1) != 0
    gram_stats_wgs = _policy("gram_stats_wgs", 256)
    gram_colsums = _policy("gram_colsums", 1) != 0

    def side_stream(self):
        if not self.overlap_wgrad:
            return None
        if getattr(self, "_side", None) is None:
            from .streams import concurrent_stream
            self._side = concurrent_stream(self.main_stream())
        return self._side

    def main_stream(self):
        ms = getattr(self, "_main", None)
        return ms if ms is not None else torch.cuda.current_stream()

    _rec = None

    def _wait(self, dst, src):
        if self._rec is not None:
            self._rec.wait(dst, src)
        else:
            dst.wait_stream(src)

    def _mark(self, stream):
        if self._rec is not None:
            return self._rec.mark(stream)
        ev = torch.cuda.Event()
        ev.record(stream)
        return ev

    def _wait_mark(self, stream, ev):
        if self._rec is not None:
            self._rec.wait_mark(stream, ev)
        else:
            stream.wait_event(ev)

    def on_side(self, launch):
        self._side_keep.append(launch)
        self._side_pending.append(launch)


    def flush_side(self, late=False):
        pend = getattr(self, "_side_pending", None)
        marked = getattr(self, "_side_marked", None)
        if late and pend:
            ev = self._mark(self.main_stream())
            if marked is None:
                marked = self._side_marked = []
            marked.append((ev, list(pend)))
            del pend[:]
            return
        self.issue_marked()
        if pend:
            self._wait(self._side, self.main_stream())
            with _on_stream(self._side):
                for launch in pend:
                    launch()
            del pend[:]

    def issue_marked(self):
        marked = getattr(self, "_side_marked", None)
        if marked:
            for ev, launches in marked:
                self._wait_mark(self._side, ev)
                with _on_stream(self._side):
                    for launch in launches:
                        launch()
            del marked[:]

    def join_side(self):
        self.flush_side()
        if getattr(self, "_side", None) is not None:
            self._wait(self.main_stream(), self._side)
        del self._side_keep[:]

    def add(self, a, b, key=None):
        m, c = a.shape
        if c not in self._ones:
            self._ones[c] = (torch.ones(c, device=a.device), torch.zeros(c, device=a.device))
        one, zero = self._ones[c]
        out = self.buf((key or id(a), "add"), a.shape, a.dtype) if key is not None else torch.empty_like(a)
        check(self.lib.mvf_bn_apply(_p(a), m, c, _p(one), _p(zero), _p(b), None, None, 0, _p(out), self.dt, _st()), "add")
        return out

    lr, momentum, weight_decay, max_norm = 0.015, 0.9, 1e-4, 40.0

    def trainable_offset(self):
        params = list(self.model.parameters())
        flags = [p.requires_grad for p in params]
        k = flags.index(True) if True in flags else len(flags)
        self._scattered_frozen = not all(flags[k:])
        return self._grad_view[id(params[k])].storage_offset() if k < len(params) else self.flat_grads.numel()

    nesterov = True
    param_options = None

    def set_param_options(self, options):
        self.param_options = {id(p): (float(a), float(b)) for p, (a, b) in options.items()} if options else None
        self._seg_tables = {}

    def _segment_table(self, off, merge):
        opts = self.param_options or {}
        segs, names, last = [], [], None
        for name, p in self.model.named_parameters():
            first = self._grad_view[id(p)].storage_offset()
            if first + p.numel() <= off:
                continue
            mult = opts.get(id(p), (1.0, 1.0)) if p.requires_grad else (-1.0, 0.0)
            if merge and mult == last:
                continue
            start = max(first - off, 0) if segs else 0
            if not merge and segs and start <= segs[-1].first:
                raise RuntimeError("lamb: parameter %s does not lie behind its predecessor in the flat buffer" % name)
            segs.append(_lib.SgdSegment(start, mult[0], mult[1]))
            names.append(name)
            last = mult
        arr = (_lib.SgdSegment * len(segs))(*segs)
        return torch.frombuffer(bytearray(bytes(arr)), dtype=torch.uint8).to(self.device), len(segs), names

    def _segments(self, off):
        tabs = self.__dict__.setdefault("_seg_tables", {})
        key = (off, tuple(p.requires_grad for p in self.model.parameters()))
        if key not in tabs:
            tabs[key] = self._segment_table(off, merge=True)[:2]
        return tabs[key]

    def apply_sgd(self, lr=None, world=1):
        return self._apply_optimizer(self.flat_grads, 1.0 / world, lr)

    def _apply_optimizer(self, grads, grad_scale, lr=None):
        ls = self._lstats
        if ls is not None:
            ls["grads"], ls["scale"] = grads, float(grad_scale)
            measured = self._layer_stats_before(grads)
        if self._adam is not None:
            out = self._apply_lamb(grads, grad_scale, lr) if self._adam.get("lamb") is not None else self._apply_adamw(grads, grad_scale, lr)
        else:
            out = self._apply_sgd(grads, grad_scale, lr)
        if ls is not None:
            ls["grads"] = None
            if measured and out is not None:
                self._layer_stats_after()
        return out

    _lstats = None

    def _flat_stats(self, x, y, out, guard=None, step_out=None):
        ls = self._lstats
        check(self.lib.mvf_flat_segment_stats(_p(x), _p(y), x.numel(), _p(ls["first"]), ls["nseg"], _p(out), _p(guard), _p(step_out), _p(ls["ws"]), ls["ws"].numel(),
                                         _st()), "flat segment stats")

    def _layer_stats_before(self, grads):
        ls = self._lstats
        if not ls["armed"] or not self.rehomed:
            return False
# ... 1386 lines not shown
```

Before: 1794 clips/s.

## Compute Gram matrix once per tile with fused column sums for BN stats

Adds a symmetric Gram kernel (A^T A) for 64/128-channel pointwise convs. It reads the activation tile once into LDS and uses it as both operands, and it also computes column sums through an MFMA against a ones vector, accumulating them in double. A new BN-stats kernel derives the column means from those sums, which removes the separate colmeans pass in the forward pass, and it uses a block-wide reduction over K in a split-bf16 MFMA. The wgrad path also routes the dz==x case through this kernel. The cost is extra workspace and more complex reduction code, and it relies on the compensated split for accuracy.

```diff
diff --git a/include/mvfnet_hip.h b/include/mvfnet_hip.h
--- a/include/mvfnet_hip.h
+++ b/include/mvfnet_hip.h
@@ -182,6 +182,9 @@
 int mvf_bn_train_stats_gram(const float* gram, const float* a_mean, const void* w_packed, long m, int c, int k, const float* gamma, const float* beta,
                             float eps, float momentum, float* running_mean, float* running_var, float* save_mean, float* save_invstd, float* scale,
                             float* shift, int dtype, void* stream);
+int mvf_bn_train_stats_gram_colsums(const float* gram, const float* col_sums, const void* w_packed, long m, int c, int k, const float* gamma,
+                                    const float* beta, float eps, float momentum, float* running_mean, float* running_var, float* save_mean,
+                                    float* save_invstd, float* scale, float* shift, float* a_mean_out, int dtype, void* stream);
 int mvf_bn_apply_colmeans(const void* z, long m, int c, const float* scale, const float* shift, int act, void* out, float* mean_out, void* ws,
                           size_t ws_bytes, int dtype, void* stream);
 int mvf_bn_apply(const void* z, long m, int c, const float* scale, const float* shift, const void* residual,
@@ -366,6 +369,7 @@
     int32_t launches;
 } mvf_wgrad_launch_info_t;
 int mvf_conv2d_wgrad_last_launch(mvf_wgrad_launch_info_t* out);
+int mvf_conv2d_nhwc_gram_colsums(const mvf_conv_desc_t* d, const void* a, float* gram_colsums, void* ws, size_t ws_bytes, int wgs, void* stream);
 typedef struct {
     const float* w;
     void* out;
diff --git a/mvfnet_amd/_lib.py b/mvfnet_amd/_lib.py
--- a/mvfnet_amd/_lib.py
+++ b/mvfnet_amd/_lib.py
@@ -247,6 +247,8 @@
     lib.mvf_bn_train_finalize.argtypes = [fp, i32, i64, i32, fp, fp, f32, f32, fp, fp, fp, fp, fp, fp, vp]
     lib.mvf_bn_train_stats_gram.restype = i32
     lib.mvf_bn_train_stats_gram.argtypes = [fp, fp, vp, i64, i32, i32, fp, fp, f32, f32, fp, fp, fp, fp, fp, fp, i32, vp]
+    lib.mvf_bn_train_stats_gram_colsums.restype = i32
+    lib.mvf_bn_train_stats_gram_colsums.argtypes = [fp, fp, vp, i64, i32, i32, fp, fp, f32, f32, fp, fp, fp, fp, fp, fp, fp, i32, vp]
     lib.mvf_bn_apply_colmeans.restype = i32
     lib.mvf_bn_apply_colmeans.argtypes = [vp, i64, i32, fp, fp, i32, vp, fp, vp, sz, i32, vp]
     lib.mvf_bn_apply.restype = i32
@@ -348,6 +350,8 @@
     lib.mvf_conv2d_nhwc_wgrad.argtypes = [cp, vp, vp, vp, i32, i32, i32, i32, fp, vp, sz, vp]
     lib.mvf_conv2d_nhwc_wgrad_wgs.restype = i32
     lib.mvf_conv2d_nhwc_wgrad_wgs.argtypes = [cp, vp, vp, vp, i32, i32, i32, i32, fp, vp, sz, i32, vp]
+    lib.mvf_conv2d_nhwc_gram_colsums.restype = i32
+    lib.mvf_conv2d_nhwc_gram_colsums.argtypes = [cp, vp, fp, vp, sz, i32, vp]
     lib.mvf_conv2d_wgrad_last_launch.restype = i32
     lib.mvf_conv2d_wgrad_last_launch.argtypes = [C.POINTER(WgradLaunchInfo)]
     lib.mvf_pack_conv_weight_dgrad.restype = i32
diff --git a/mvfnet_amd/csrc/bn_dzfree.hip b/mvfnet_amd/csrc/bn_dzfree.hip
--- a/mvfnet_amd/csrc/bn_dzfree.hip
+++ b/mvfnet_amd/csrc/bn_dzfree.hip
@@ -274,6 +274,86 @@
     }
 }
 
+__global__ __launch_bounds__(1024) void gram_stats_blocks_kernel(GramStatsArgs p, const float* col_sums, float* a_mean_out, float m_f) {
+    extern __shared__ __attribute__((aligned(16))) float gs_lds[];
+    const int tid = threadIdx.x, lane = tid & 63, kb = tid >> 6, K = p.K, nkb = K / 32;
+    float* am = gs_lds;
+    float* redq = gs_lds + K;
+    float* redm = redq + nkb * 32;
+    for (int k = tid; k < K; k += blockDim.x) {
+        const float a = col_sums[k] / m_f;
+        am[k] = a;
+        if (blockIdx.x == 0) a_mean_out[k] = a;
+    }
+    __syncthreads();
+    const int c0 = blockIdx.x * 32, row = lane & 31, half = lane >> 5;
+    const uint16_t* pw = p.w + (long)(c0 + row) * K + half * 8;
+    const int k = kb * 32 + row;
+    const float* pg = p.gram + (long)k * K + half * 8;
+    const float* pa = am + half * 8;
+    const float ak = am[k];
+    f32x16 acc;
+#pragma unroll
+    for (int r = 0; r < 16; ++r) acc[r] = 0.f;
+    for (int j = 0; j < K; j += 16) {
+        const uint4 vw = *reinterpret_cast<const uint4*>(pw + j);
+        const float4 g0 = *reinterpret_cast<const float4*>(pg + j), g1 = *reinterpret_cast<const float4*>(pg + j + 4);
+        const float4 a0 = *reinterpret_cast<const float4*>(pa + j), a1 = *reinterpret_cast<const float4*>(pa + j + 4);
+        float gc[8] = {g0.x * p.inv_m - ak * a0.x, g0.y * p.inv_m - ak * a0.y, g0.z * p.inv_m - ak * a0.z, g0.w * p.inv_m - ak * a0.w,
+                       g1.x * p.inv_m - ak * a1.x, g1.y * p.inv_m - ak * a1.y, g1.z * p.inv_m - ak * a1.z, g1.w * p.inv_m - ak * a1.w};
+        unsigned hi[4], mid[4], lo[4];
+#pragma unroll
+        for (int q = 0; q < 4; ++q) {
+            const float x0 = gc[2 * q], x1 = gc[2 * q + 1];
+            hi[q] = pack_bf16x2(x0, x1);
+            const float r0 = x0 - bf16lo(hi[q]), r1 = x1 - bf16hi(hi[q]);
+            mid[q] = pack_bf16x2(r0, r1);
+            lo[q] = pack_bf16x2(r0 - bf16lo(mid[q]), r1 - bf16hi(mid[q]));
+        }
+        bf16x8 fw, fh, fm, fl;
+        __builtin_memcpy(&fw, &vw, 16);
+        __builtin_memcpy(&fh, hi, 16);
+        __builtin_memcpy(&fm, mid, 16);
+        __builtin_memcpy(&fl, lo, 16);
+        acc = __builtin_amdgcn_mfma_f32_32x32x16_bf16(fw, fh, acc, 0, 0, 0);
+        acc = __builtin_amdgcn_mfma_f32_32x32x16_bf16(fw, fm, acc, 0, 0, 0);
+        acc = __builtin_amdgcn_mfma_f32_32x32x16_bf16(fw, fl, acc, 0, 0, 0);
+    }
+#pragma unroll
+    for (int r = 0; r < 16; ++r) {
+        const int cl = 8 * (r >> 2) + 4 * half + (r & 3);
+        const float wv = __uint_as_float((unsigned)p.w[(long)(c0 + cl) * K + k] << 16);
+        float q = acc[r] * wv, mu = wv * ak;
+#pragma unroll
+        for (int o = 1; o < 32; o <<= 1) {
+            q += __shfl_xor(q, o, 64);
+            mu += __shfl_xor(mu, o, 64);
+        }
+        if (row == 0) {
+            redq[kb * 32 + cl] = q;
+            redm[kb * 32 + cl] = mu;
+        }
+    }
+    __syncthreads();
+    if (tid < 32) {
+        float q = 0.f, mean = 0.f;
+        for (int b = 0; b < nkb; ++b) {
+            q += redq[b * 32 + tid];
+            mean += redm[b * 32 + tid];
+        }
+        const int c = c0 + tid;
+        const float var = fmaxf(q, 0.f);
+        const float invstd = 1.0f / sqrtf(var + p.eps);
+        p.save_mean[c] = mean;
+        p.save_invstd[c] = invstd;
+        const float s = p.gamma[c] * invstd;
+        p.scale[c] = s;
+        p.shift[c] = p.beta[c] - mean * s;
+        if (p.running_mean) p.running_mean[c] = (1.f - p.momentum) * p.running_mean[c] + p.momentum * mean;
+        if (p.running_var) p.running_var[c] = (1.f - p.momentum) * p.running_var[c] + p.momentum * (var * p.unbias);
+    }
+}
+
 constexpr long GRAM_F64_MAX_ROWS = 16;
 __global__ __launch_bounds__(256) void gram_stats_f64_kernel(GramStatsArgs p, double inv_m, double unbias) {
     const int lane = threadIdx.x & 63, c = blockIdx.x * 4 + (threadIdx.x >> 6), K = p.K;
@@ -323,6 +403,24 @@
         hipLaunchKernelGGL(gram_stats_f64_kernel, dim3((c + 3) / 4), dim3(256), 0, (hipStream_t)stream, p, 1.0 / (double)m, (double)m / (double)(m > 1 ? m - 1 : 1));
     else
         hipLaunchKernelGGL(gram_stats_kernel, dim3((c / 32 + 3) / 4), dim3(256), 0, (hipStream_t)stream, p);
+    MVF_LAUNCH_CHECK();
+    return MVF_OK;
+}
+
+int mvf_bn_train_stats_gram_colsums(const float* gram, const float* col_sums, const void* w_packed, long m, int c, int k, const float* gamma, const float* beta,
+                                    float eps, float momentum, float* running_mean, float* running_var, float* save_mean, float* save_invstd, float* scale,
+                                    float* shift, float* a_mean_out, int dtype, void* stream) {
+    MVF_REQUIRE(gram && col_sums && w_packed && gamma && beta && save_mean && save_invstd && scale && shift && a_mean_out && m > 0, MVF_EINVAL,
+                "bn_train_stats_gram_colsums: NULL argument");
+    MVF_REQUIRE(dtype == MVF_BF16, MVF_EUNSUPPORTED, "bn_train_stats_gram_colsums: bf16 storage only");
+    MVF_REQUIRE(c > 0 && k > 0 && c % 32 == 0 && k % 32 == 0 && k <= 512, MVF_ESHAPE, "bn_train_stats_gram_colsums: c=%d and k=%d (<= 512) must be multiples of 32", c, k);
+    MVF_REQUIRE(((uintptr_t)gram | (uintptr_t)w_packed) % 16 == 0, MVF_EINVAL, "bn_train_stats_gram_colsums: gram / w_packed must be 16-byte aligned");
+    MVF_REQUIRE(m > GRAM_F64_MAX_ROWS, MVF_EUNSUPPORTED, "bn_train_stats_gram_colsums: m=%ld rows: up to %ld take mvf_bn_train_stats_gram (fp64)", m, GRAM_F64_MAX_ROWS);
+    GramStatsArgs p = {gram, nullptr, (const uint16_t*)w_packed, gamma, beta, running_mean, running_var, save_mean, save_invstd, scale, shift,
+                       c, k, 1.0f / (float)m, eps, momentum, (float)((double)m / (double)(m - 1))};
+    const int nkb = k / 32;
+    hipLaunchKernelGGL(gram_stats_blocks_kernel, dim3(c / 32), dim3(64 * nkb), (size_t)(k + 64 * nkb) * sizeof(float), (hipStream_t)stream, p, col_sums, a_mean_out,
+                       (float)m);
     MVF_LAUNCH_CHECK();
     return MVF_OK;
 }
diff --git a/mvfnet_amd/csrc/wgrad_nhwc.hip b/mvfnet_amd/csrc/wgrad_nhwc.hip
--- a/mvfnet_amd/csrc/wgrad_nhwc.hip
+++ b/mvfnet_amd/csrc/wgrad_nhwc.hip
@@ -538,6 +538,134 @@
     }
 }
 
+struct GramArgs {
+    const void* a;
+    float* part;
+    int M, rows_per_split;
+};
+template <int TM, int NS>
+__global__ __launch_bounds__(256) void gram_once_kernel(GramArgs g) {
+    constexpr int kThreads = 256;
+    constexpr int K = 2 * TM * 32;
+    constexpr int PA = K * 2;
+    constexpr int UA = K / 8;
+    constexpr int NA = BMR16 * UA / kThreads;
+    static_assert(NS >= 3 && (NS - 2) * NA < 64, "ring depth");
+    extern __shared__ __attribute__((aligned(16))) char smem16[];
+    char* As = smem16;
+    const int split = blockIdx.x;
+    const int tid = threadIdx.x, lane = tid & 63, wave = tid >> 6;
+    const int wm = wave >> 1, wn = wave & 1;
+    const int ra0 = tid / UA;
+    const int qa = (tid % UA) ^ swz16<UA>(ra0);
+    const long m_begin = (long)split * g.rows_per_split;
+    const int rows = (int)max(0L, min((long)g.M - m_begin, (long)g.rows_per_split));
+    const int nchunks = (rows + BMR16 - 1) / BMR16;
+    const bf16_t* ap = reinterpret_cast<const bf16_t*>(g.a);
+    const i32x4 gs_a = rsrc_words(ap + (rows > 0 ? m_begin : 0) * K, (unsigned)((long)rows * K * 2));
+    const unsigned lds_a0 = (unsigned)__builtin_amdgcn_readfirstlane((int)(unsigned)(size_t)(__attribute__((address_space(3))) char*)As + (wave * 64 / UA) * PA);
+    const unsigned a_col = (unsigned)(qa * 8) * 2u;
+    auto dma_chunk = [&](int c, int buf) {
+#pragma unroll
+        for (int i = 0; i < NA; ++i) {
+            const int r = c * BMR16 + ra0 + (kThreads / UA) * i;
+            glds16(gs_a, lds_a0 + (unsigned)((buf * BMR16 + (kThreads / UA) * i) * PA), (unsigned)(r * K) * 2u + a_col);
+        }
+    };
+    const int tg = lane >> 4, ti = lane & 15;
+    const int trow = (ti >> 2) + 8 * (tg >> 1);
+    const int tunit = 2 * (tg & 1) + ((ti & 3) >> 1), thalf = ti & 1;
+    int offA[TM], offB[TM];
+#pragma unroll
+    for (int i = 0; i < TM; ++i) {
+        offA[i] = trow * PA + ((((wm * TM + i) * 4 + tunit) ^ swz16<UA>(trow)) * 16) + thalf * 8;
+        offB[i] = trow * PA + ((((wn * TM + i) * 4 + tunit) ^ swz16<UA>(trow)) * 16) + thalf * 8;
+    }
+    auto gather = [&](const char* p) {
+        typedef short v4s __attribute__((ext_vector_type(4)));
+        typedef __attribute__((address_space(3))) v4s* lds_v4s;
+        const v4s lo = __builtin_amdgcn_ds_read_tr16_b64_v4i16((lds_v4s)(p));
+        const v4s hi = __builtin_amdgcn_ds_read_tr16_b64_v4i16((lds_v4s)(p + 4 * PA));
+        bf16x8_t v;
+        v[0] = lo[0]; v[1] = lo[1]; v[2] = lo[2]; v[3] = lo[3];
+        v[4] = hi[0]; v[5] = hi[1]; v[6] = hi[2]; v[7] = hi[3];
+        return v;
+    };
+    bf16x8_t ones;
+#pragma unroll
+    for (int e = 0; e < 8; ++e) ones[e] = (short)0x3f80;
+    f32x16 acc[TM][TM];
+    double dsum[TM][16];
+#pragma unroll
+    for (int i = 0; i < TM; ++i) {
+#pragma unroll
+        for (int r = 0; r < 16; ++r) dsum[i][r] = 0.0;
+#pragma unroll
+        for (int j = 0; j < TM; ++j)
+#pragma unroll
+            for (int r = 0; r < 16; ++r) acc[i][j][r] = 0.f;
+    }
+    auto compute = [&](int buf) {
+        f32x16 accs[TM];
+#pragma unroll
+        for (int i = 0; i < TM; ++i)
+#pragma unroll
+            for (int r = 0; r < 16; ++r) accs[i][r] = 0.f;
+#pragma unroll
+        for (int ks = 0; ks < BMR16 / 16; ++ks) {
+            const int r0 = buf * BMR16 + ks * 16;
+            bf16x8_t fa[TM], fb[TM];
+#pragma unroll
+            for (int i = 0; i < TM; ++i) fa[i] = gather(As + r0 * PA + offA[i]);
+#pragma unroll
+            for (int j = 0; j < TM; ++j) fb[j] = gather(As + r0 * PA + offB[j]);
+#pragma unroll
+            for (int i = 0; i < TM; ++i)
+#pragma unroll
+                for (int j = 0; j < TM; ++j) acc[i][j] = __builtin_amdgcn_mfma_f32_32x32x16_bf16(fa[i], fb[j], acc[i][j], 0, 0, 0);
+            if (wn == 0) {
+#pragma unroll
+                for (int i = 0; i < TM; ++i) accs[i] = __builtin_amdgcn_mfma_f32_32x32x16_bf16(fa[i], ones, accs[i], 0, 0, 0);
+            }
+        }
+        if (wn == 0) {
+#pragma unroll
+            for (int i = 0; i < TM; ++i)
+#pragma unroll
+                for (int r = 0; r < 16; ++r) dsum[i][r] += (double)accs[i][r];
+        }
+    };
+#pragma unroll
+    for (int s_ = 0; s_ < NS - 1; ++s_) dma_chunk(s_, s_);
+    for (int cc = 0; cc < nchunks; cc += NS) {
+#pragma unroll
+        for (int s_ = 0; s_ < NS; ++s_) {
+            if (cc + s_ < nchunks) {
+                wg_wait_vmcnt<(NS - 2) * NA>();
+                __builtin_amdgcn_s_barrier();
+                dma_chunk(cc + s_ + NS - 1, (s_ + NS - 1) % NS);
+                compute(s_);
+            }
+        }
+    }
+    asm volatile("s_waitcnt vmcnt(0)" ::: "memory");
+    float* outp = g.part + (long)split * (K + 2) * K;
+    const int lr = lane >> 5, lc = lane & 31;
+#pragma unroll
+    for (int i = 0; i < TM; ++i)
+#pragma unroll
+        for (int r = 0; r < 16; ++r) {
+            const int row = (wm * TM + i) * 32 + (r & 3) + 8 * (r >> 2) + 4 * lr;
+#pragma unroll
+            for (int j = 0; j < TM; ++j) outp[row * K + (wn * TM + j) * 32 + lc] = acc[i][j][r];
+            if (wn == 0 && lc == 0) {
+                const float hi = (float)dsum[i][r];
+                outp[K * K + row] = hi;
+                outp[(K + 1) * K + row] = (float)(dsum[i][r] - (double)hi);
+            }
+        }
+}
+
 constexpr int BMRX = 32;
 template <int TM, int TN>
 __global__ __launch_bounds__(256, 3) void wgrad_x3_kernel(WgArgs a) {
@@ -1010,7 +1138,7 @@
 }
 
 __global__ __launch_bounds__(256) void wgrad_reduce1_kernel(const float* part, int nsplit, int cout, int cin, int kh, int kw, int kwp, int cinp,
-                                    float* dw) {
+                                    float* dw, long slab) {
     __shared__ float red[4][64];
     const long K = (long)kh * kwp * cinp;
     const long total = (long)cout * K;
@@ -1020,12 +1148,12 @@
     if (i < total) {
         int k = sl;
         for (; k + 12 < nsplit; k += 16) {
-            s0 += part[(long)k * total + i];
-            s1 += part[(long)(k + 4) * total + i];
-            s2 += part[(long)(k + 8) * total + i];
-            s3 += part[(long)(k + 12) * total + i];
-        }
-        for (; k < nsplit; k += 4) s0 += part[(long)k * total + i];
+            s0 += part[(long)k * slab + i];
+            s1 += part[(long)(k + 4) * slab + i];
+            s2 += part[(long)(k + 8) * slab + i];
+            s3 += part[(long)(k + 12) * slab + i];
+        }
+        for (; k < nsplit; k += 4) s0 += part[(long)k * slab + i];
     }
     red[sl][e] = (s0 + s1) + (s2 + s3);
     __syncthreads();
@@ -1038,9 +1166,37 @@
         if (ci < cin && x < kw) dw[(((long)co * cin + ci) * kh + y) * kw + x] = (red[0][e] + red[1][e]) + (red[2][e] + red[3][e]);
     }
 }
-int launch_wgrad_reduce(const float* part, int nsplit, int cout, int cin, int kh, int kw, int kwp, int cinp, float* dw, hipStream_t st) {
+__global__ __launch_bounds__(256) void gram_reduce_kernel(const float* part, int nsplit, int k, float* out) {
+    __shared__ float red[4][64];
+    __shared__ double redd[4][64];
+    const long kk = (long)k * k, slab = kk + 2 * k;
+    const int e = threadIdx.x & 63, sl = threadIdx.x >> 6;
+    const long i = (long)blockIdx.x * 64 + e;
+    if (i < kk) {
+        float s0 = 0.f, s1 = 0.f, s2 = 0.f, s3 = 0.f;
+        int s = sl;
+        for (; s + 12 < nsplit; s += 16) {
+            s0 += part[(long)s * slab + i];
+            s1 += part[(long)(s + 4) * slab + i];
+            s2 += part[(long)(s + 8) * slab + i];
+            s3 += part[(long)(s + 12) * slab + i];
+        }
+        for (; s < nsplit; s += 4) s0 += part[(long)s * slab + i];
+        red[sl][e] = (s0 + s1) + (s2 + s3);
+        __syncthreads();
+        if (sl == 0) out[i] = (red[0][e] + red[1][e]) + (red[2][e] + red[3][e]);
+    } else {
+        double t = 0.0;
+        if (i < kk + k)
+            for (int s = sl; s < nsplit; s += 4) t += (double)part[(long)s * slab + i] + (double)part[(long)s * slab + i + k];
+        redd[sl][e] = t;
+        __syncthreads();
+        if (sl == 0 && i < kk + k) out[i] = (float)((redd[0][e] + redd[1][e]) + (redd[2][e] + redd[3][e]));
+    }
+}
+int launch_wgrad_reduce(const float* part, int nsplit, int cout, int cin, int kh, int kw, int kwp, int cinp, float* dw, hipStream_t st, long slab = 0) {
     const long total = (long)cout * kh * kwp * cinp;
-    hipLaunchKernelGGL(wgrad_reduce1_kernel, dim3((int)((total + 63) / 64)), dim3(256), 0, st, part, nsplit, cout, cin, kh, kw, kwp, cinp, dw);
+    hipLaunchKernelGGL(wgrad_reduce1_kernel, dim3((int)((total + 63) / 64)), dim3(256), 0, st, part, nsplit, cout, cin, kh, kw, kwp, cinp, dw, slab > 0 ? slab : total);
     MVF_LAUNCH_CHECK();
     return MVF_OK;
 }
@@ -1169,6 +1325,41 @@
            d->x_pix_stride == 4 && mvf_internal::wgrad_stem_ok(d->n, d->h, d->w, d->ho, d->wo);
 }
 
+constexpr int GRAM_ONCE_MIN_ROWS = 17;
+static bool gram_once_shape(const mvf_conv_desc_t* d) {
+    return d->dtype == MVF_BF16 && d->kh == 1 && d->kw == 1 && d->stride == 1 && d->pad == 0 && d->cin == d->cout && (d->cin == 64 || d->cin == 128) &&
+           d->x_pix_stride == d->cin && d->split_c == 0 && d->x_c0 == 0 && d->ho == d->h && d->wo == d->w && (long)d->n * d->h * d->w >= GRAM_ONCE_MIN_ROWS &&
+           (long)d->n * d->h * d->w < 0x7fffffffL;
+}
+static int gram_once_launch(const mvf_conv_desc_t* d, const void* a, void* ws, size_t ws_bytes, int wgs, hipStream_t st, int* nsplit_out) {
+    const int K = d->cin, M = d->n * d->h * d->w;
+    const size_t slab = (size_t)(K + 2) * K * sizeof(float);
+    const long fit = (long)(std::min(ws_bytes, mvf_conv2d_wgrad_workspace_bytes(d)) / slab);
+    MVF_REQUIRE(fit >= 1, MVF_EWS, "gram: workspace too small");
+    int target_used = 0;
+    int rows = plan_split(M, 1, wgs, &target_used);
+    if ((M + rows - 1) / rows > fit) rows = std::max(rows, (int)(((M + fit - 1) / fit + 63) / 64 * 64));
+    const int nsplit = (M + rows - 1) / rows;
+    constexpr int NS64 = 8, NS128 = 6;
+    MVF_REQUIRE(((long)rows + (NS64 + 1) * 64) * K * 2 < 0x7ffffff0L, MVF_ESHAPE, "gram: %d rows per split exceed 32-bit offsets", rows);
+    GramArgs g = {a, (float*)ws, M, rows};
+    auto k64 = gram_once_kernel<1, NS64>;
+    auto k128 = gram_once_kernel<2, NS128>;
+    constexpr int lds64 = NS64 * BMR16 * 64 * 2, lds128 = NS128 * BMR16 * 128 * 2;
+    static bool attr = false;
+    if (!attr) {
+        MVF_HIP_OK(hipFuncSetAttribute((const void*)k64, hipFuncAttributeMaxDynamicSharedMemorySize, lds64));
+        MVF_HIP_OK(hipFuncSetAttribute((const void*)k128, hipFuncAttributeMaxDynamicSharedMemorySize, lds128));
+        attr = true;
+    }
+    if (K == 64) hipLaunchKernelGGL(k64, dim3(nsplit), dim3(256), lds64, st, g);
+    else hipLaunchKernelGGL(k128, dim3(nsplit), dim3(256), lds128, st, g);
+    MVF_LAUNCH_CHECK();
+    t_last_wgrad = mvf_wgrad_launch_info_t{MVF_WGRAD_FAM_BF16_PIPE, K == 64 ? NS64 : NS128, K, K, MVF_BF16, nsplit, rows, 0, 0, 1, target_used, 1};
+    *nsplit_out = nsplit;
+    return MVF_OK;
+}
+
 size_t mvf_conv2d_wgrad_workspace_bytes(const mvf_conv_desc_t* d) {
     if (!d || d->cout <= 0 || d->cin <= 0) return 0;
     const int M = d->n * d->ho * d->wo, K = d->kh * d->kw * d->cin;
@@ -1179,7 +1370,7 @@
     if (wg_big_shape(d)) nsplit = std::max(nsplit, (M + wg_big_rows(d) - 1) / wg_big_rows(d));
     if (wg_direct3x3(d)) nsplit = std::max(nsplit, mvf_internal::wgrad3x3_c64_wgs(d->n, d->h));
     if (wg_direct_stem(d)) nsplit = std::max(nsplit, mvf_internal::wgrad_stem_wgs(d->n, d->ho));
-    return align_up((size_t)nsplit * d->cout * K * sizeof(float), 256);
+    return align_up((size_t)nsplit * (d->cout + (gram_once_shape(d) ? 2 : 0)) * K * sizeof(float), 256);
 }
 
 }
@@ -1208,6 +1399,16 @@
         if (rc != MVF_OK) return rc;
         t_last_wgrad = mvf_wgrad_launch_info_t{MVF_WGRAD_FAM_STEM, 0, 64, 224, MVF_BF16, w.nwg, 0, 0, 0, 0, 0, 1};
         const int rr = launch_wgrad_reduce((const float*)ws, w.nwg, 64, 3, 7, 7, 8, 4, dw_oihw, st0);
+        if (rr == MVF_OK) t_last_wgrad.launches = 2;
+        return rr;
+    }
+    static const int gram_once_env = mvf_policy_int("gram_once", 1);
+    if (gram_once_env && wgs_target > 0 && dz == x && !x2 && gram_once_shape(d) && kw_real == 1 && kw_packed == 1 && cin_real == d->cin && cin_packed == d->cin &&
+        (uintptr_t)x % 16 == 0) {
+        int nsplit = 0;
+        const int rc = gram_once_launch(d, x, ws, ws_bytes, wgs_target, st0, &nsplit);
+        if (rc != MVF_OK) return rc;
+        const int rr = launch_wgrad_reduce((const float*)ws, nsplit, d->cin, d->cin, 1, 1, 1, d->cin, dw_oihw, st0, (long)(d->cin + 2) * d->cin);
         if (rr == MVF_OK) t_last_wgrad.launches = 2;
         return rr;
     }
@@ -1311,6 +1512,23 @@
     return wgrad_impl(d, dz, x, x2, kw_real, cin_real, kw_packed, cin_packed, dw_oihw, ws, ws_bytes, stream, wgs);
 }
 
+int mvf_conv2d_nhwc_gram_colsums(const mvf_conv_desc_t* d, const void* a, float* gram_colsums, void* ws, size_t ws_bytes, int wgs, void* stream) {
+    t_last_wgrad = mvf_wgrad_launch_info_t{};
+    MVF_REQUIRE(d && a && gram_colsums && ws, MVF_EINVAL, "gram_colsums: NULL argument");
+    MVF_REQUIRE(wgs >= 1 && wgs <= 4096, MVF_EINVAL, "gram_colsums: wgs=%d outside 1 .. 4096", wgs);
+    MVF_REQUIRE(d->dtype == MVF_BF16, MVF_EUNSUPPORTED, "gram_colsums: bf16 storage only");
+    MVF_REQUIRE(gram_once_shape(d), MVF_ESHAPE, "gram_colsums: a compact pointwise descriptor with cin = cout = 64 | 128 and >= %d rows", GRAM_ONCE_MIN_ROWS);
+    MVF_REQUIRE((uintptr_t)a % 16 == 0, MVF_EINVAL, "gram_colsums: a must be 16-byte aligned");
+    int nsplit = 0;
+    const int rc = gram_once_launch(d, a, ws, ws_bytes, wgs, (hipStream_t)stream, &nsplit);
+    if (rc != MVF_OK) return rc;
+    const int k = d->cin;
+    hipLaunchKernelGGL(gram_reduce_kernel, dim3((k + 1) * k / 64), dim3(256), 0, (hipStream_t)stream, (const float*)ws, nsplit, k, gram_colsums);
+    MVF_LAUNCH_CHECK();
+    t_last_wgrad.launches = 2;
+    return MVF_OK;
+}
+
 int mvf_conv2d_wgrad_last_launch(mvf_wgrad_launch_info_t* out) {
     MVF_REQUIRE(out, MVF_EINVAL, "conv2d_wgrad_last_launch: NULL argument");
     *out = t_last_wgrad;
diff --git a/mvfnet_amd/train_engine.py b/mvfnet_amd/train_engine.py
--- a/mvfnet_amd/train_engine.py
+++ b/mvfnet_amd/train_engine.py
@@ -482,31 +482,48 @@
 
     def gram_stats(self, a_in, bn, n, h, w, eng, means_done=False):
         c, k, m = self.cout, self.cin, n * h * w
-        gram = eng.buf((id(self), "gram"), (k, k), torch.float32)
+        gram = self.gram_buf(eng)
         amean = eng.buf((id(self), "amean"), (4, k), torch.float32)
         d = ConvDesc(n, h, w, k, k, 1, 1, 1, 0, h, w, k, eng.dt, 0, 0, 0, 0)
-        ws = eng.workspace(max(self.eng.lib.mvf_conv2d_wgrad_workspace_bytes(C.byref(d)), self.eng.lib.mvf_bn_workspace_bytes(m, k), (eng.gram_stats_wgs + 8) * k * k * 4))
+        ws = eng.workspace(max(self.eng.lib.mvf_conv2d_wgrad_workspace_bytes(C.byref(d)), self.eng.lib.mvf_bn_workspace_bytes(m, k), (eng.gram_stats_wgs + 8) * (k + 2) * k * 4))
+        if self.gram_colsums_ok(eng, m):
+            assert not means_done, "the column means come from the Gram kernel's column sums"
+            self.launch_gram(d, a_in, gram, ws, eng.gram_stats_wgs)
+            check(self.eng.lib.mvf_bn_train_stats_gram_colsums(_p(gram), _p(gram[k]), _p(self.wp), m, c, k, _p(bn.gamma), _p(bn.beta), C.c_float(bn.eps),
+                                                               C.c_float(bn.momentum), _p(bn.mod.running_mean), _p(bn.mod.running_var), _p(bn.mean), _p(bn.invstd),
+                                                               _p(bn.scale), _p(bn.shift), _p(amean[0]), eng.dt, _st()), "bn statistics from the Gram matrix and column sums")
+            bn._count()
+            return
         if k not in eng._ones:
             eng._ones[k] = (torch.ones(k, device=a_in.device), torch.zeros(k, device=a_in.device))
         one, zero = eng._ones[k]
-        self.launch_gram(d, a_in, gram, ws, eng.gram_stats_wgs)
+        self.launch_gram(d, a_in, gram[:k], ws, eng.gram_stats_wgs)
         if not means_done:
             check(self.eng.lib.mvf_bn_train_stats(_p(a_in), m, k, _p(one), _p(zero), C.c_float(1e-5), C.c_float(0.1), None, None, _p(amean[0]), _p(amean[1]),
                                          _p(amean[2]), _p(amean[3]), _p(ws), ws.numel(), eng.dt, _st()), "column means")
-        check(self.eng.lib.mvf_bn_train_stats_gram(_p(gram), _p(amean[0]), _p(self.wp), m, c, k, _p(bn.gamma), _p(bn.beta), C.c_float(bn.eps), C.c_float(bn.momentum),
+        check(self.eng.lib.mvf_bn_train_stats_gram(_p(gram[:k]), _p(amean[0]), _p(self.wp), m, c, k, _p(bn.gamma), _p(bn.beta), C.c_float(bn.eps), C.c_float(bn.momentum),
                                           _p(bn.mod.running_mean), _p(bn.mod.running_var), _p(bn.mean), _p(bn.invstd), _p(bn.scale), _p(bn.shift), eng.dt,
                                           _st()), "bn statistics from the Gram matrix")
         bn._count()
 
+    def gram_buf(self, eng):
+        return eng.buf((id(self), "gram"), (self.cin + 1, self.cin), torch.float32)
+
+    def gram_colsums_ok(self, eng, m):
+        return bool(eng.gram_stats_blocks and eng.gram_once and self.gram_ok() and self.cin in (64, 128) and m >= 17)
+
     def launch_gram(self, d, a_in, gram, ws, wgs):
         k = self.cin
+        if gram.shape[0] == k + 1:
+            check(self.eng.lib.mvf_conv2d_nhwc_gram_colsums(C.byref(d), _p(a_in), _p(gram), _p(ws), ws.numel(), wgs, _st()), "gram + column sums (launch stream)")
+            return
         check(self.eng.lib.mvf_conv2d_nhwc_wgrad_wgs(C.byref(d), _p(a_in), _p(a_in), None, 1, k, 1, k, _p(gram), _p(ws), ws.numel(), wgs, _st()), "gram (launch stream)")
 
     def dzfree_wgrad(self, gm, a_in, bn, n, h, w, eng, frozen_zero=None, q_done=False, gram_done=False):
         c, k, m = self.cout, self.cin, n * h * w
         if not q_done:
             self.wgrad(gm, a_in, n, h, w, h, w, eng)
-        gram = eng.buf((id(self), "gram"), (k, k), torch.float32)
+        gram = self.gram_buf(eng)[:k]
         amean = eng.buf((id(self), "amean"), (4, k), torch.float32)
         d = ConvDesc(n, h, w, k, k, 1, 1, 1, 0, h, w, k, eng.dt, 0, 0, 0, 0)
         nbytes = max(self.eng.lib.mvf_conv2d_wgrad_workspace_bytes(C.byref(d)), self.eng.lib.mvf_bn_workspace_bytes(m, k))
@@ -729,7 +746,7 @@
         z2, ho, wo = self.c2.forward(a1, nt, h, w, bn=self.b2)
         m2 = nt * ho * wo
         gram = self.gram_fwd(eng, m2)
-        cs = gram and eng.gram_colsums and self.b2.c % 8 == 0
+        cs = gram and eng.gram_colsums and self.b2.c % 8 == 0 and not self.c3.gram_colsums_ok(eng, m2)
         if cs:
             amean = eng.buf((id(self.c3), "amean"), (4, self.c3.cin), torch.float32)
             a2 = self.b2.apply_colmeans(z2, m2, 1, amean[0])
@@ -1036,6 +1053,8 @@
     gram_stats = _policy("gram_stats", 1) != 0
     gram_stats_wgs = _policy("gram_stats_wgs", 256)
     gram_colsums = _policy("gram_colsums", 1) != 0
+    gram_once = _policy("gram_once", 1) != 0
+    gram_stats_blocks = _policy("gram_stats_blocks", 1) != 0
 
     def side_stream(self):
         if not self.overlap_wgrad:
```

After: 1804 clips/s, median of 6. No clear change (+0.6%).
